# chaitjo/efficient-gnns

Measured on AMD Instinct MI355X. Metric: training epochs/sec, ogbn-arxiv 3-layer GCN student + G-CRD, 1/2/4/8 MI355X, higher is better.
Workload: dtype f32

## Files before the change

### efficient-gnns_amd/_lib.py

```python
from __future__ import annotations

import ctypes as C
import os

import torch

_HERE = os.path.dirname(os.path.abspath(__file__))
LIB_PATH = os.path.join(_HERE, "lib", "libegnn_hip.so")

_p, _i64, _i32, _f32, _sz, _u64 = C.c_void_p, C.c_int64, C.c_int, C.c_float, C.c_size_t, C.c_uint64


class BnAct(C.Structure):
    _fields_ = [("x", _p), ("ld", _i64), ("n", _i64), ("C", _i64),
                ("mean", _p), ("var", _p), ("eps", _f32),
                ("gamma", _p), ("beta", _p),
                ("relu", _i32), ("p", _f32), ("seed", _u64), ("seed_dev", _p),
                ("pick", _p), ("n_pick", _i64)]


class GatLayer(C.Structure):
    _fields_ = [("rowptr", _p), ("col", _p),
                ("colptr", _p), ("t_col", _p), ("perm", _p),
                ("n", _i64), ("nnz", _i64), ("H", _i32), ("C", _i32),
                ("xl", _p), ("ld_xl", _i64),
                ("el", _p), ("er", _p),
                ("attn_l", _p), ("attn_r", _p),
                ("keep", _p), ("mult", _p), ("src_scale", _p), ("dst_scale", _p),
                ("negative_slope", _f32)]


class Spmm(C.Structure):
    _fields_ = [("n_rows", _i64), ("n_src", _i64), ("K", _i64),
                ("rowptr", _p), ("col", _p), ("index_bits", _i32),
                ("val", _p), ("src_scale", _p), ("bias", _p),
                ("X", _p), ("ldx", _i64), ("Y", _p), ("ldy", _i64), ("reduce", _i32),
                ("addend", _p), ("ld_addend", _i64), ("stat_part", _p), ("stat_shift", _p), ("flags", _i32)]


class SignSeg(C.Structure):
    _fields_ = [("B", _i64), ("Cs", _i64), ("H", _i32),
                ("p", _f32), ("seed", _p), ("seed_dev", _p),
                ("slope", _p),
                ("src", _p), ("ld_src", _p), ("n_src", _i64),
                ("batch", _p)]


ADAM_MAX_LAG = 64


class AdamRows(C.Structure):
    _fields_ = [("p", _p), ("m", _p), ("v", _p), ("last", _p),
                ("n_rows", _i64), ("D", _i64), ("ld", _i64),
                ("beta1", _f32), ("beta2", _f32), ("eps", _f32),
                ("one_minus_beta1", _f32), ("one_minus_beta2", _f32),
                ("step", _i32), ("flushed", _i32),
                ("step_size", _f32 * ADAM_MAX_LAG), ("bc2_sqrt", _f32 * ADAM_MAX_LAG),
                ("dup_count", _p)]


SIGNATURES = {
    "egnn_abi_version": (_i32, []),
    "egnn_error_string": (C.c_char_p, [_i32]),
    "egnn_build_info": (_i32, [C.c_char_p, _sz]),
    "egnn_spmm_csr_f32": (_i32, [_p, _p, _p, _i64, _p, _i64, _p, _i64, _p]),
    "egnn_spmm_csr_seg_f32": (_i32, [_p, _p, _i64, _p, _p, _i64, _p, _i64, _p]),
    "egnn_spmm_csr_blk_f32": (_i32, [_p, _i32, _i32, _p, _i64, _p, _p, _i64, _p, _p]),
    "egnn_spmm_blk_stat_rows": (_i64, [_i64, _i32, _i32]),
    "egnn_spmm_blk_window_i32": (_i32, [_p, _p, _i64, _i32, _p, _i64, _p, _p]),
    "egnn_bn_stats_merge_ws_floats": (_sz, [_i64]),
    "egnn_bn_stats_merge_f32": (_i32, [_p, _i64, _i64, _p, _i64, _p, _i64, _p, _i64, _p, _p, _p, _sz, _p]),
    "egnn_spmm_combine_f32": (_i32, [_p, _p, _p, _i64, _p, _i64, _p]),
    "egnn_spmm_csr_max_bwd_f32": (_i32, [_i64, _i64, _p, _i32, _p, _p, _p, _i64, _p, _i64, _p]),
    "egnn_spmm_csr_max_piece_f32": (_i32, [_p, _p, _i32, _p, _p]),
    "egnn_spmm_csr_max_bwd_rows_f32": (_i32, [_i64, _i64, _i64, _p, _p, _i32, _p, _p, _p, _p, _i64, _p, _i64, _p, _i64, _p]),
    "egnn_spmm_algorithmic_bytes": (_i64, [_i64, _i64, _i64, _i64, _i32, _i32]),
    "egnn_csr_from_coo_ws_bytes": (_sz, [_i64, _i64, _i32]),
    "egnn_csr_from_coo_i64": (_i32, [_p, _p, _i64, _i64, _i32, _p, _p, _p, _p, _sz, _p]),
    "egnn_csr_transpose_ws_bytes": (_sz, [_i64, _i64]),
    "egnn_csr_transpose_i64": (_i32, [_p, _p, _i64, _i64, _i64, _p, _p, _p, _p, _sz, _p]),
    "egnn_rowptr_from_sorted_rows_i64": (_i32, [_p, _i64, _i64, _p, _p]),
    "egnn_narrow_i64_to_i32": (_i32, [_p, _i64, _p, _p, _p]),
    "egnn_gcn_norm_count_i64": (_i32, [_p, _p, _i64, _p, _p]),
    "egnn_gcn_norm_fill_i64": (_i32, [_p, _p, _i64, _p, _p, _p, _p]),
    "egnn_gcn_norm_values_i64": (_i32, [_p, _p, _i64, _p, _p, _p]),
    "egnn_gemm_ws_floats": (_sz, [_i32, _i32, _i64, _i64, _i64, _i32]),
    "egnn_gemm_f32": (_i32, [_i32, _i32, _i64, _i64, _i64, _f32, _p, _i64, _p, _i64, _p, _p, _i64, _i32, _p, _sz, _p]),
    "egnn_gemm_ex_f32": (_i32, [_i32, _i32, _i64, _i64, _i64, _f32, _p, _i64, _p, _i64, _p, _p, _i64, _i32, _p, _sz, _i32, _p]),
    "egnn_gemm_add_f32": (_i32, [_i32, _i32, _i64, _i64, _i64, _f32, _p, _i64, _p, _i64, _p, _p, _i64, _p, _i64, _i32, _p, _sz, _p]),
    "egnn_bn_fold_f32": (_i32, [_p, _i64, _i64, _i64, _p, _p, _p, _p, _p, _f32, _p, _i64, _p, _p]),
    "egnn_gemm_rows_f32": (_i32, [_i32, _i32, _i64, _i64, _i64, _f32, _p, _i64, _p, _p, _i64, _p, _p, _p, _i64, _i32, _p, _sz, _p]),
    "egnn_gemm_tn_planes_bytes": (_sz, [_i64, _i64]),
    "egnn_gemm_tn_planes_pack_f32": (_i32, [_p, _i64, _p, _i64, _i64, _p, _sz, _p]),
    "egnn_gemm_tn_planes_ws_floats": (_sz, [_i64, _i64, _i64]),
    "egnn_gemm_tn_planes_f32": (_i32, [_i64, _i64, _i64, _f32, _p, _i64, _p, _p, _i64, _p, _sz, _p]),
    "egnn_gemm_rows_planes_bytes": (_sz, [_i64, _i64]),
    "egnn_gemm_rows_planes_pack_f32": (_i32, [_p, _i64, _p, _i64, _i64, _p, _sz, _p]),
    "egnn_gemm_rows_planes_ws_bytes": (_sz, [_i64, _i64]),
    "egnn_gemm_rows_planes_f32": (_i32, [_i64, _i64, _i64, _f32, _p, _p, _i64, _p, _p, _i64, _p, _sz, _p]),
    "egnn_ce_kd_ws_floats": (_sz, [_i64]),
    "egnn_ce_kd_fwd_f32": (_i32, [_p, _i64, _p, _i64, _p, _p, _i64, _i64, _f32, _p, _p, _p]),
    "egnn_ce_kd_bwd_f32": (_i32, [_p, _i64, _p, _i64, _p, _p, _i64, _i64, _i64, _f32, _p, _p, _p, _p, _i64, _p]),
    "egnn_gather_normalize_rows_f32": (_i32, [_p, _i64, _p, _i64, _i64, _f32, _p, _i64, _p, _p]),
    "egnn_normalize_rows_bwd_f32": (_i32, [_p, _i64, _p, _i64, _p, _p, _i64, _i64, _f32, _p, _i64, _i32, _p]),
    "egnn_nce_ws_floats": (_sz, [_i64]),
    "egnn_nce_fwd_f32": (_i32, [_p, _p, _i64, _i64, _i64, _f32, _i32, _p, _p, _p, _p, _sz, _p]),
    "egnn_nce_saves_exp": (_i32, [_f32, _i32]),
    "egnn_nce_bwd_ws_floats": (_sz, [_i64, _i64, _i64]),
    "egnn_nce_bwd_f32": (_i32, [_p, _p, _i64, _i64, _i64, _f32, _i32, _p, _p, _p, _p, _p, _p, _sz, _p]),
    "egnn_nce_block_fwd_f32": (_i32, [_p, _i64, _p, _i64, _i64, _i64, _i64, _i64, _f32, _f32, _i32, _p, _p, _p, _p, _sz, _p]),
    "egnn_nce_block_bwd_f32": (_i32, [_p, _i64, _p, _i64, _i64, _i64, _i64, _i64, _f32, _f32, _i32, _p, _p, _p, _p, _i64, _p, _i64, _p, _sz, _p]),
    "egnn_gsp_ws_floats": (_sz, [_i64]),
    "egnn_gsp_fwd_f32": (_i32, [_p, _i64, _i64, _p, _i64, _i64, _i64, _i32, _p, _p, _p, _p, _sz, _p]),
    "egnn_rowsum_f32": (_i32, [_p, _i64, _i64, _i64, _p, _p]),
    "egnn_scale_rowcorr_f32": (_i32, [_p, _i64, _p, _i64, _p, _p, _i64, _i64, _p, _i64, _p]),
    "egnn_bce_pair_ws_floats": (_sz, []),
    "egnn_bce_pair_fwd_f32": (_i32, [_p, _p, _p, _i64, _p, _p, _p]),
    "egnn_bce_pair_bwd_f32": (_i32, [_p, _p, _p, _i64, _p, _p, _p, _p]),
    "egnn_edge_sim_f32": (_i32, [_p, _i64, _i64, _p, _p, _i64, _i32, _p, _p, _p]),
    "egnn_edge_sim_coef_f32": (_i32, [_p, _p, _p, _i64, _i32, _p, _p, _p, _p]),
    "egnn_gat_attention_fwd_f32": (_i32, [_p, _p, _p, _p, _i64, _i64, _i32, _f32, _p, _p]),
    "egnn_gat_layer_fwd_f32": (_i32, [_p, _p, _p, _i64, _p]),
    "egnn_gat_layer_bwd_ws_floats": (_sz, [_i64, _i32, _i32]),
    "egnn_gat_layer_bwd_f32": (_i32, [_p, _p, _p, _i64, _i32, _p, _p, _p, _i64, _p, _p, _sz, _p]),
    "egnn_segment_softmax_fwd_f32": (_i32, [_p, _p, _i64, _p, _p]),
    "egnn_segment_softmax_bwd_f32": (_i32, [_p, _p, _p, _i64, _p, _p]),
    "egnn_segment_sum_f32": (_i32, [_p, _p, _i64, _p, _p]),
    "egnn_lsp_loss_ws_floats": (_sz, []),
    "egnn_lsp_loss_fwd_f32": (_i32, [_p, _p, _p, _i64, _i64, _i32, _p, _p, _p, _p, _p]),
    "egnn_lsp_loss_bwd_f32": (_i32, [_p, _p, _p, _i64, _i64, _i32, _p, _p, _p, _p]),
    "egnn_colsum_ws_floats": (_sz, [_i64]),
    "egnn_colsum_f32": (_i32, [_p, _i64, _i64, _i64, _p, _p, _p]),
    "egnn_bn_ws_floats": (_sz, [_i64]),
    "egnn_bn_stats_f32": (_i32, [_p, _i64, _i64, _i64, _p, _p, _p, _sz, _p]),
    "egnn_bn_act_fwd_f32": (_i32, [_p, _p, _i64, _p]),
    "egnn_bn_act_bwd_f32": (_i32, [_p, _p, _i64, _i32, _p, _p, _p, _i64, _p, _p, _sz, _p]),
    "egnn_bn_act_bwd_reduce_f32": (_i32, [_p, _p, _i64, _p, _p, _p, _sz, _p]),
    "egnn_bn_act_bwd_apply_f32": (_i32, [_p, _p, _i64, _p, _p, _f32, _p, _p, _i64, _p, _p, _sz, _p]),
    "egnn_bn_merge_shards_f32": (_i32, [_p, _i32, _i64, _p, _p, _p, _p]),
    "egnn_bn_act_linear_fwd_f32": (_i32, [_p, _p, _i64, _i32, _i64, _p, _i64, _p, _i64, _p]),
    "egnn_skinny_dx_bn_ws_floats": (_sz, [_i64, _i64]),
    "egnn_skinny_dx_bn_bwd_reduce_f32": (_i32, [_p, _i64, _p, _i64, _i32, _i64, _f32, _p, _i64, _p, _i64, _p, _p, _p, _p, _p, _i64, _p, _sz, _p]),
    "egnn_bn_bwd_apply_stored_f32": (_i32, [_p, _p, _p, _f32, _p, _i64, _p, _p, _sz, _p]),
    "egnn_bn_running_update_dev_f32": (_i32, [_p, _p, _i64, _p, _f32, _p, _p, _p, _p]),
    "egnn_bn_running_update_f32": (_i32, [_p, _p, _i64, _i64, _f32, _p, _p, _p, _p]),
    "egnn_split_accuracy_ws_ints": (_sz, []),
    "egnn_split_accuracy_f32": (_i32, [_p, _i64, _i64, _i64, _p, _p, _p, _p, _sz, _p]),
    "egnn_split_counts_f32": (_i32, [_p, _i64, _i64, _i64, _p, _p, _p, _p, _sz, _p]),
    "egnn_rows_add_f32": (_i32, [_p, _i64, _p, _p, _i64, _i64, _i64, _p]),
    "egnn_feature_loss_ws_floats": (_sz, [_i64]),
    "egnn_fitnet_fwd_f32": (_i32, [_p, _i64, _p, _i64, _i64, _i64, _f32, _p, _p, _sz, _p]),
    "egnn_fitnet_bwd_f32": (_i32, [_p, _i64, _p, _i64, _i64, _i64, _f32, _p, _p, _i64, _p, _i64, _p]),
    "egnn_at_fwd_f32": (_i32, [_p, _i64, _i64, _p, _i64, _i64, _i64, _f32, _p, _p, _sz, _p]),
    "egnn_at_bwd_f32": (_i32, [_p, _i64, _i64, _p, _i64, _i64, _i64, _f32, _p, _p, _p, _i64, _p, _i64, _p]),
    "egnn_at_energy_f32": (_i32, [_p, _i64, _i64, _p, _i64, _i64, _i64, _p, _p, _p, _p, _sz, _p]),
    "egnn_at_partial_f32": (_i32, [_p, _p, _i64, _p, _f32, _p, _p, _p, _sz, _p]),
    "egnn_at_bwd_rows_f32": (_i32, [_p, _i64, _i64, _p, _i64, _i64, _i64, _i64, _p, _p, _p, _p, _f32, _p, _p, _i64, _p, _i64, _p]),
    "egnn_saint_induced_geometry": (_i64, [_i32]),
    "egnn_saint_random_walk_i64": (_i32, [_p, _p, _i64, _i64, _i64, _i64, _p, _p, _u64, _p, _p, _p, _p]),
    "egnn_saint_scan_ws_bytes": (_sz, [_i64]),
    "egnn_saint_select_i64": (_i32, [_p, _i64, _p, _p, _i64, _p, _sz, _p]),
    "egnn_saint_induced_count_i64": (_i32, [_p, _p, _p, _i64, _p, _i64, _i64, _i64, _p, _p, _p, _p, _sz, _p]),
    "egnn_saint_induced_fill_i64": (_i32, [_p, _p, _p, _p, _i64, _p, _i64, _i64, _i64, _p, _p, _p, _i64, _p, _p, _p, _p]),
    "egnn_saint_gather_i64": (_i32, [_p, _i64, _p, _p, _p, _p, _p, _p, _p, _p, _p, _i64, _p, _p, _p]),
    "egnn_sign_gather_drop_f32": (_i32, [_p, _p, _i64, _p]),
    "egnn_prelu_drop_fwd_f32": (_i32, [_p, _p, _i64, _p, _i64, _p]),
    "egnn_prelu_drop_ws_floats": (_sz, [_i64, _i64, _i32]),
    "egnn_prelu_drop_bwd_f32": (_i32, [_p, _p, _i64, _p, _i64, _p, _i64, _p, _p, _p, _sz, _p]),
    "egnn_pair_moments_ws_bytes": (_sz, [_i64]),
    "egnn_pair_moments_f32": (_i32, [_p, _i64, _i64, _p, _i64, _i64, _i64, _p, _p, _sz, _p]),
    "egnn_pearson_moments_ws_bytes": (_sz, [_i64]),
    "egnn_pearson_moments_f32": (_i32, [_p, _p, _i64, _p, _p, _sz, _p]),
    "egnn_sqdist_median_ws_bytes": (_sz, [_i64]),
    "egnn_sqdist_median_f32": (_i32, [_p, _i64, _i64, _i64, _p, _p, _sz, _p]),
    "egnn_rbf_cka_ws_bytes": (_sz, [_i64]),
    "egnn_rbf_cka_f32": (_i32, [_p, _i64, _i64, _p, _i64, _i64, _i64, _p, _p, _p, _sz, _p]),
    "egnn_group_input_f32": (_i32, [_p, _p, _i32, _p, _p, _i64, _i64, _p, _i64, _p, _p]),
    "egnn_adam_rows_catchup_f32": (_i32, [_p, _i32, _p, _p, _i64, _p]),
    "egnn_adam_rows_flush_f32": (_i32, [_p, _p]),
    "egnn_adam_rows_step_f32": (_i32, [_p, _i32, _p, _p, _i64, _p, _i64, _p]),
    "egnn_probe_gather_lines_f32":(_i32, [_p, _i64, _i64, _i64, _p, _i64, _i32, _i32, _p, _p]),
}

_lib = None


class HipExtensionError(RuntimeError):
    pass


def load() -> C.CDLL:
    global _lib
    if _lib is not None:
        return _lib
    if not os.path.exists(LIB_PATH):
        raise HipExtensionError(
            f"{LIB_PATH} is missing: build it with `python efficient-gnns_amd/build.py` "
            "(__graft_entry__.build()); there is no CPU fallback")
    lib = C.CDLL(LIB_PATH)
    for name, (res, args) in SIGNATURES.items():
        fn = getattr(lib, name)
        fn.restype, fn.argtypes = res, args
    if lib.egnn_abi_version() != 9:
        raise HipExtensionError("libegnn_hip.so ABI version mismatch")
    _lib = lib
    return lib


EGNN_EALIGN = -4


def check(rc: int, what: str) -> None:
    if rc != 0:
        msg = load().egnn_error_string(rc).decode()
        raise HipExtensionError(f"{what} failed: {msg} ({rc})")


# ... 28 lines not shown
```

### efficient-gnns_amd/criterion.py

```python
from __future__ import annotations

import numpy as np
import torch

from . import ops

__all__ = ["distill", "kd_criterion", "fitnet_criterion", "at_criterion", "gpw_criterion", "lpw_criterion", "nce_criterion",
           "loss_kd_only", "ppi_kd_criterion", "ppi_fitnet_criterion", "ppi_at_criterion", "ppi_gpw_criterion", "ppi_lpw_criterion",
           "ppi_nce_criterion"]


_ROW_SAMPLER = None


def _sample_rows(n: int, max_samples: int, device):
    if _ROW_SAMPLER is not None:
        return _ROW_SAMPLER(n, max_samples, device)
    if max_samples < n:
        pick = np.random.choice(n, max_samples, replace=False)
        return torch.from_numpy(pick).to(device=device, dtype=torch.int64, non_blocking=True)
    return None


def _rows_of(x, idx):
# ... 24 lines not shown
    if rows is not None:
        logits, labels = logits[rows], labels[rows]
    return bce_with_logits_pair(logits, labels, logits.detach())[0]




def kd_criterion(logits, labels, teacher_logits, alpha=0.9, T=4):
    return rows_kd_criterion(logits, labels, teacher_logits, alpha, T, rows=None)


def rows_kd_criterion(logits, labels, teacher_logits, alpha=0.9, T=4, rows=None):
    loss_cls, loss_kd = ops.ce_and_kd(_plain(logits), _plain(labels), _plain(teacher_logits), T, rows)
    loss = loss_kd * (alpha * T * T) + loss_cls * (1 - alpha)
    return loss, loss_cls, loss_kd


def loss_kd_only(logits, labels, teacher_logits, alpha=0.9, T=4):
    return kd_criterion(logits, labels, teacher_logits, alpha, T)[2]


def fitnet_criterion(logits, labels, feat, teacher_feat, beta=1000):
    return rows_fitnet_criterion(logits, labels, feat, teacher_feat, beta, rows=None)


@_plain_args
def rows_fitnet_criterion(logits, labels, feat, teacher_feat, beta=1000, rows=None, *, _cls=None):
    loss_cls = (_cls or _ce_term)(logits, labels, rows)
    loss_aux = ops.fitnet_loss(_plain(feat), _plain(teacher_feat))
    return torch.add(loss_cls, loss_aux, alpha=beta), loss_cls, loss_aux


def at_criterion(logits, labels, feat, teacher_feat, beta=1000):
    return rows_at_criterion(logits, labels, feat, teacher_feat, beta, rows=None)


@_plain_args
def rows_at_criterion(logits, labels, feat, teacher_feat, beta=1000, rows=None, *, _cls=None):
    loss_cls = (_cls or _ce_term)(logits, labels, rows)
    loss_aux = ops.at_loss(_plain(feat), _plain(teacher_feat))
    return torch.add(loss_cls, loss_aux, alpha=beta), loss_cls, loss_aux


def gpw_criterion(logits, labels, feat, teacher_feat, kernel="cosine", beta=1, max_samples=8192):
    return rows_gpw_criterion(logits, labels, feat, teacher_feat, kernel, beta, max_samples, rows=None)


@_plain_args
def rows_gpw_criterion(logits, labels, feat, teacher_feat, kernel="cosine", beta=1, max_samples=8192, rows=None, presampled=False, *, _cls=None):
    from .ops_pairwise import gsp_loss
    if kernel not in ("cosine", "poly", "l2", "rbf"):
        raise NotImplementedError
    loss_cls = (_cls or _ce_term)(logits, labels, rows)
    idx = None if presampled else _sample_rows(feat.shape[0], max_samples, feat.device)
    if hasattr(feat, "_egnn_materialise") or hasattr(teacher_feat, "_egnn_materialise"):
        from .lazy import materialise
        feat, teacher_feat, idx = materialise(feat, idx), materialise(teacher_feat, idx), None
    loss_aux = gsp_loss(feat, teacher_feat, idx, kernel)
    return torch.add(loss_cls, loss_aux, alpha=beta), loss_cls, loss_aux


def lpw_criterion(logits, labels, feat, teacher_feat, edge_index, kernel="cosine", beta=100, criterion="kld"):
    return rows_lpw_criterion(logits, labels, feat, teacher_feat, edge_index, kernel, beta, criterion, rows=None)


@_plain_args
def rows_lpw_criterion(logits, labels, feat, teacher_feat, edge_index, kernel="cosine", beta=100, criterion="kld", rows=None, *, _cls=None):
    from .ops_edge import lsp_loss
    if kernel not in ("cosine", "poly", "l2", "rbf") or criterion not in ("kld", "mse"):
        raise NotImplementedError
    loss_cls = (_cls or _ce_term)(logits, labels, rows)
    loss_aux = lsp_loss(_plain(feat), _plain(teacher_feat), edge_index, kernel, criterion)
    return torch.add(loss_cls, loss_aux, alpha=beta), loss_cls, loss_aux


def nce_criterion(logits, labels, feat, teacher_feat, beta=0.5, nce_T=0.075, max_samples=8192):
    return rows_nce_criterion(logits, labels, feat, teacher_feat, beta, nce_T, max_samples, rows=None)


@_plain_args
def rows_nce_criterion(logits, labels, feat, teacher_feat, beta=0.5, nce_T=0.075, max_samples=8192, rows=None, presampled=False, *, _cls=None):
    loss_cls = (_cls or _ce_term)(logits, labels, rows)
    idx = None if presampled else _sample_rows(feat.shape[0], max_samples, feat.device)
    fhat = ops.gather_normalize(*_rows_of(feat, idx))
    that = ops.gather_normalize(*_rows_of(teacher_feat, idx))
    loss_aux = ops.nce_unit(fhat, that, nce_T)
    return torch.add(loss_cls, loss_aux, alpha=beta), loss_cls, loss_aux


def ppi_fitnet_criterion(logits, labels, feat, teacher_feat, beta=1000):
    return rows_fitnet_criterion(logits, labels, feat, teacher_feat, beta, _cls=_bce_term)


def ppi_at_criterion(logits, labels, feat, teacher_feat, beta=1000):
    return rows_at_criterion(logits, labels, feat, teacher_feat, beta, _cls=_bce_term)


def ppi_gpw_criterion(logits, labels, feat, teacher_feat, kernel="cosine", beta=1, max_samples=8192):
    return rows_gpw_criterion(logits, labels, feat, teacher_feat, kernel, beta, max_samples, _cls=_bce_term)


def ppi_lpw_criterion(logits, labels, feat, teacher_feat, edge_index, kernel="cosine", beta=100, criterion="kld"):
    return rows_lpw_criterion(logits, labels, feat, teacher_feat, edge_index, kernel, beta, criterion, _cls=_bce_term)


def ppi_nce_criterion(logits, labels, feat, teacher_feat, beta=0.5, nce_T=0.075, max_samples=8192):
    return rows_nce_criterion(logits, labels, feat, teacher_feat, beta, nce_T, max_samples, _cls=_bce_term)


def ppi_kd_criterion(logits, labels, teacher_logits, alpha=0.5, T=1):
    from .ops_pairwise import bce_with_logits_pair
    loss_cls, loss_kd = bce_with_logits_pair(_plain(logits), _plain(labels), _plain(teacher_logits))
    return loss_kd * (alpha * T * T) + loss_cls * (1 - alpha), loss_cls, loss_kd


def presample(mode, n, hp, device):
    return _sample_rows(n, hp["max_samples"], device) if mode in ("gpw", "nce") else None


def distill(mode, logits, labels, feat, teacher_feat, hp, *, teacher_logits=None, rows=None, edge_index=None, presampled=False,
            multilabel=False, kd_and_aux=False):
    cls = _bce_term if multilabel else None

    def kd():
        if not multilabel:
            return rows_kd_criterion(logits, labels, teacher_logits, hp["alpha"], hp["kd_T"], rows=rows)
        picked = (logits, labels, teacher_logits) if rows is None else (logits[rows], labels[rows], teacher_logits[rows])
        return ppi_kd_criterion(*picked, hp["alpha"], hp["kd_T"])
    if mode == "kd":
        return kd()
    if mode == "fitnet":
        res = rows_fitnet_criterion(logits, labels, feat, teacher_feat, hp["beta"], rows=rows, _cls=cls)
    elif mode == "at":
        res = rows_at_criterion(logits, labels, feat, teacher_feat, hp["beta"], rows=rows, _cls=cls)
    elif mode == "gpw":
        res = rows_gpw_criterion(logits, labels, feat, teacher_feat, hp["kernel"], hp["beta"], hp["max_samples"], rows=rows,
                                 presampled=presampled, _cls=cls)
    elif mode == "lpw":
        res = rows_lpw_criterion(logits, labels, feat, teacher_feat, edge_index, hp["kernel"], hp["beta"], rows=rows, _cls=cls)
    elif mode in ("nce", "gcd"):
        res = rows_nce_criterion(logits, labels, feat, teacher_feat, hp["beta"], hp["nce_T"], hp["max_samples"], rows=rows,
                                 presampled=presampled, _cls=cls)
    else:
        raise NotImplementedError(mode)
    if not kd_and_aux:
        return res
    loss, loss_cls, _ = kd()
    return loss + hp["beta"] * res[2], loss_cls, res[2]
```

### efficient-gnns_amd/csrc/fused_bn.hip

```cpp
#include "bn_common.h"

namespace {

constexpr int kMaxChunks = 4;
constexpr int kStatBlocks = 512;

using namespace egnn_bn;

__global__ __launch_bounds__(256) void bn_stats_partial_kernel(const float* __restrict__ x, int64_t ld, int64_t n, int64_t C,
                                                               float* __restrict__ part) {
  __shared__ float sh[4][2][kMaxChunks * 256];
  const int lane = egnn_lane();
  const int wave = egnn_wave_id();
  const int chunks = (int)((C + 255) / 256);
  float s1[kMaxChunks][4], s2[kMaxChunks][4], x0[kMaxChunks][4];
#pragma unroll
  for (int j = 0; j < kMaxChunks; ++j)
#pragma unroll
    for (int q = 0; q < 4; ++q) { s1[j][q] = 0.f; s2[j][q] = 0.f; x0[j][q] = 0.f; }
#pragma unroll
  for (int j = 0; j < kMaxChunks; ++j) {
    const int64_t c = j * 256 + lane * 4;
    if (j < chunks && c < C) {
      const float4 v = *reinterpret_cast<const float4*>(x + c);
      x0[j][0] = v.x; x0[j][1] = v.y; x0[j][2] = v.z; x0[j][3] = v.w;
    }
  }
  auto tally = [&](int j, const float4& v) {
    const float d0 = v.x - x0[j][0], d1 = v.y - x0[j][1], d2 = v.z - x0[j][2], d3 = v.w - x0[j][3];
    s1[j][0] += d0; s1[j][1] += d1; s1[j][2] += d2; s1[j][3] += d3;
    s2[j][0] = fmaf(d0, d0, s2[j][0]); s2[j][1] = fmaf(d1, d1, s2[j][1]);
    s2[j][2] = fmaf(d2, d2, s2[j][2]); s2[j][3] = fmaf(d3, d3, s2[j][3]);
  };
  const int64_t stride = (int64_t)gridDim.x * 4;
  int64_t row = blockIdx.x * 4LL + wave;
  if (chunks == 1) {
    const int64_t c = lane * 4;
    if (c < C) {
      for (; row + 3 * stride < n; row += 4 * stride) {
        float4 v[4];
#pragma unroll
        for (int u = 0; u < 4; ++u) v[u] = *reinterpret_cast<const float4*>(x + (row + u * stride) * ld + c);
#pragma unroll
        for (int u = 0; u < 4; ++u) tally(0, v[u]);
      }
    }
  }
  for (; row < n; row += stride) {
#pragma unroll
    for (int j = 0; j < kMaxChunks; ++j) {
      const int64_t c = j * 256 + lane * 4;
      if (j < chunks && c < C) tally(j, *reinterpret_cast<const float4*>(x + row * ld + c));
    }
  }
#pragma unroll
  for (int j = 0; j < kMaxChunks; ++j)
#pragma unroll
    for (int q = 0; q < 4; ++q) {
      sh[wave][0][j * 256 + lane * 4 + q] = s1[j][q];
      sh[wave][1][j * 256 + lane * 4 + q] = s2[j][q];
    }
  __syncthreads();
  for (int64_t c = threadIdx.x; c < C; c += 256) {
    float a = 0.f, b = 0.f;
    for (int w = 0; w < 4; ++w) { a += sh[w][0][c]; b += sh[w][1][c]; }
    part[((int64_t)blockIdx.x * 2) * C + c] = a;
    part[((int64_t)blockIdx.x * 2 + 1) * C + c] = b;
  }
}

constexpr int kMergeCols = 8;
constexpr int kMergeGroups = 256 / kMergeCols;
__device__ __forceinline__ void merge_partials(const float* __restrict__ part, int nblocks, int64_t C, float& a, float& b, bool& owner,
                                               int64_t& c) {
  __shared__ float sh[2][kMergeGroups][kMergeCols];
  const int col = threadIdx.x % kMergeCols, grp = threadIdx.x / kMergeCols;
  c = (int64_t)blockIdx.x * kMergeCols + col;
  float sa = 0.f, sb = 0.f;
  if (c < C)
    for (int i = grp; i < nblocks; i += kMergeGroups) { sa += part[((int64_t)i * 2) * C + c]; sb += part[((int64_t)i * 2 + 1) * C + c]; }
  sh[0][grp][col] = sa;
  sh[1][grp][col] = sb;
  __syncthreads();
  owner = grp == 0 && c < C;
  a = 0.f; b = 0.f;
  if (owner)
    for (int g = 0; g < kMergeGroups; ++g) { a += sh[0][g][col]; b += sh[1][g][col]; }
}

__global__ __launch_bounds__(256) void bn_stats_final_kernel(const float* __restrict__ part, int nblocks, const float* __restrict__ x,
                                                             int64_t n, int64_t C, float* __restrict__ mean, float* __restrict__ var) {
  float a, b; bool owner; int64_t c;
  merge_partials(part, nblocks, C, a, b, owner, c);
  if (!owner) return;
  const float inv = 1.f / (float)n;
  const float m1 = a * inv;
  mean[c] = x[c] + m1;
  var[c] = fmaxf(b * inv - m1 * m1, 0.f);
}

__global__ __launch_bounds__(256) void bn_act_fwd_kernel(const BnParams q, float* __restrict__ y, int64_t ldy) {
  const int lane = egnn_lane();
  const int wave = egnn_wave_id();
  const int chunks = (int)((q.C + 255) / 256);
  for (int j = 0; j < chunks; ++j) {
    const int64_t c = j * 256 + lane * 4;
    if (c >= q.C) continue;
    float mean[4], rstd[4], g[4], b[4];
#pragma unroll
    for (int k = 0; k < 4; ++k) {
      mean[k] = q.mean[c + k];
      rstd[k] = rsqrtf(q.var[c + k] + q.eps);
      g[k] = q.gamma ? q.gamma[c + k] : 1.f;
      b[k] = q.beta ? q.beta[c + k] : 0.f;
    }
    for (int64_t row = blockIdx.x * 4LL + wave; row < q.n; row += (int64_t)gridDim.x * 4) {
      const int64_t src = bn_row(q, row);
      const float4 v = *reinterpret_cast<const float4*>(q.x + src * q.ldx + c);
      const float xv[4] = {v.x, v.y, v.z, v.w};
      float o[4];
#pragma unroll
      for (int k = 0; k < 4; ++k) {
        float xhat, gate;
        bn_elem(q, xv[k], mean[k], rstd[k], g[k], b[k], src, c + k, xhat, gate);
        o[k] = (g[k] * xhat + b[k]) * gate;
      }
      *reinterpret_cast<float4*>(y + row * ldy + c) = make_float4(o[0], o[1], o[2], o[3]);
    }
  }
}

__global__ __launch_bounds__(256) void bn_act_bwd_reduce_kernel(const BnParams q, const float* __restrict__ dy, int64_t ldd,
                                                                float* __restrict__ part) {
  __shared__ float sh[4][2][kMaxChunks * 256];
  const int lane = egnn_lane();
  const int wave = egnn_wave_id();
  const int chunks = (int)((q.C + 255) / 256);
  for (int j = 0; j < chunks; ++j) {
    const int64_t c = j * 256 + lane * 4;
    float sd[4] = {0.f, 0.f, 0.f, 0.f}, sx[4] = {0.f, 0.f, 0.f, 0.f};
    if (c < q.C) {
      float mean[4], rstd[4], g[4], b[4];
#pragma unroll
      for (int k = 0; k < 4; ++k) {
        mean[k] = q.mean[c + k];
        rstd[k] = rsqrtf(q.var[c + k] + q.eps);
        g[k] = q.gamma ? q.gamma[c + k] : 1.f;
        b[k] = q.beta ? q.beta[c + k] : 0.f;
      }
      const int64_t stride = (int64_t)gridDim.x * 4;
      int64_t row = blockIdx.x * 4LL + wave;
      for (; row + 3 * stride < q.n; row += 4 * stride) {
        float4 v[4], gd[4];
        int64_t src[4];
#pragma unroll
        for (int u = 0; u < 4; ++u) {
          src[u] = bn_row(q, row + u * stride);
          v[u] = *reinterpret_cast<const float4*>(q.x + src[u] * q.ldx + c);
          gd[u] = *reinterpret_cast<const float4*>(dy + (row + u * stride) * ldd + c);
        }
#pragma unroll
        for (int u = 0; u < 4; ++u) {
          const float xv[4] = {v[u].x, v[u].y, v[u].z, v[u].w};
          const float gv[4] = {gd[u].x, gd[u].y, gd[u].z, gd[u].w};
#pragma unroll
          for (int k = 0; k < 4; ++k) {
            float xhat, gate;
            bn_elem(q, xv[k], mean[k], rstd[k], g[k], b[k], src[u], c + k, xhat, gate);
            const float d = gv[k] * gate;
            sd[k] += d;
            sx[k] = fmaf(d, xhat, sx[k]);
          }
        }
      }
      for (; row < q.n; row += stride) {
        const int64_t src = bn_row(q, row);
        const float4 v = *reinterpret_cast<const float4*>(q.x + src * q.ldx + c);
        const float4 gd = *reinterpret_cast<const float4*>(dy + row * ldd + c);
        const float xv[4] = {v.x, v.y, v.z, v.w};
        const float gv[4] = {gd.x, gd.y, gd.z, gd.w};
#pragma unroll
// ... 121 lines not shown
    rmean[c] = (1.f - m) * rmean[c] + m * mean[c];
    rvar[c] = (1.f - m) * rvar[c] + (m * unbias) * var[c];
  }
  __syncthreads();
  if (threadIdx.x == 0 && tracked) tracked[0] = t;
}

__global__ __launch_bounds__(256) void bn_running_update_dev_kernel(const float* __restrict__ mean, const float* __restrict__ var, int64_t C,
                                                                    const float* __restrict__ total, float momentum, float* __restrict__ rmean,
                                                                    float* __restrict__ rvar, long long* __restrict__ tracked) {
  const long long t = tracked ? tracked[0] + 1 : 1;
  const float m = momentum < 0.f ? 1.f / (float)t : momentum;
  const float n = total[0];
  const float unbias = n > 1.f ? n / (n - 1.f) : 1.f;
  for (int64_t c = threadIdx.x; c < C; c += 256) {
    rmean[c] = (1.f - m) * rmean[c] + m * mean[c];
    rvar[c] = (1.f - m) * rvar[c] + (m * unbias) * var[c];
  }
  __syncthreads();
  if (threadIdx.x == 0 && tracked) tracked[0] = t;
}

bool shape_ok(const void* p, int64_t ld, int64_t C) { return C > 0 && C % 4 == 0 && C <= kMaxChunks * 256 && ld % 4 == 0 && egnn_aligned16(p); }

int row_blocks(int64_t n) {
  const int64_t want = (n + 3) / 4;
  return (int)(want < 2048 ? (want < 1 ? 1 : want) : 2048);
}

int bn_unpack(const egnn_bn_act_t* b, BnParams& all, BnParams& out) {
  EGNN_CHECK_ARG(b && b->n > 0 && b->x && b->mean && b->var && b->ld >= b->C);
  EGNN_CHECK_ARG(!b->pick || (b->n_pick >= 0 && b->n_pick <= b->n));
  if (!shape_ok(b->x, b->ld, b->C)) return EGNN_EALIGN;
  all = BnParams{b->x, b->ld, b->n, b->C, b->mean, b->var, b->eps, b->gamma, b->beta, b->relu, b->p, (unsigned long long)b->seed,
                 (const unsigned long long*)b->seed_dev, nullptr};
  out = all;
  if (b->pick) { out.n = b->n_pick; out.pick = b->pick; }
  return EGNN_OK;
}

}

namespace {
__global__ void bn_merge_shards_kernel(const float* __restrict__ st, int world, int64_t C, float* __restrict__ mean,
                                       float* __restrict__ var, float* __restrict__ total) {
  const int64_t c = blockIdx.x * 256LL + threadIdx.x;
  if (c >= C) return;
  const int64_t ld = 2 * C + 1;
  float n = 0.f, m = 0.f, m2 = 0.f;
  for (int w = 0; w < world; ++w) {
    const float nb = st[w * ld + 2 * C];
    if (nb <= 0.f) continue;
    const float mb = st[w * ld + c], vb = st[w * ld + C + c];
    const float nt = n + nb, d = mb - m;
    m2 = m2 + vb * nb + d * d * (n * nb / nt);
    m = m + d * (nb / nt);
    n = nt;
  }
  mean[c] = m;
  var[c] = n > 0.f ? m2 / n : 0.f;
  if (c == 0) total[0] = n;
}
}

extern "C" int egnn_bn_merge_shards_f32(const float* stats, int world, int64_t C, float* mean, float* var, float* total,
                                        void* stream) {
  EGNN_CHECK_ARG(world > 0 && C > 0 && stats && mean && var && total);
  hipLaunchKernelGGL(bn_merge_shards_kernel, dim3((unsigned)((C + 255) / 256)), dim3(256), 0, (hipStream_t)stream, stats, world, C, mean,
                     var, total);
  return egnn_launch_status();
}

extern "C" size_t egnn_bn_ws_floats(int64_t C) { return (size_t)kStatBlocks * 2 * (size_t)C; }

extern "C" int egnn_bn_stats_f32(const float* x, int64_t ld, int64_t n, int64_t C, float* mean, float* var, float* ws,
                                 size_t ws_floats, void* stream) {
  EGNN_CHECK_ARG(n > 0 && x && mean && var && ws && ld >= C);
  if (!shape_ok(x, ld, C)) return EGNN_EALIGN;
  if (ws_floats < egnn_bn_ws_floats(C)) return EGNN_EWORKSPACE;
  hipStream_t st = (hipStream_t)stream;
  const int64_t want = (n + 3) / 4;
  const int nb = (int)(want < kStatBlocks ? want : kStatBlocks);
  hipLaunchKernelGGL(bn_stats_partial_kernel, dim3(nb), dim3(256), 0, st, x, ld, n, C, ws);
  hipLaunchKernelGGL(bn_stats_final_kernel, dim3((unsigned)((C + kMergeCols - 1) / kMergeCols)), dim3(256), 0, st, ws, nb, x, n, C, mean, var);
  return egnn_launch_status();
}

extern "C" int egnn_bn_act_fwd_f32(const egnn_bn_act_t* bn, float* y, int64_t ldy, void* stream) {
  BnParams qa, q;
  const int rc = bn_unpack(bn, qa, q);
  if (rc != EGNN_OK) return rc;
  EGNN_CHECK_ARG(q.n > 0 && y && ldy >= bn->C && bn->p >= 0.f && bn->p < 1.f);
  if (!shape_ok(y, ldy, bn->C)) return EGNN_EALIGN;
  hipLaunchKernelGGL(bn_act_fwd_kernel, dim3(row_blocks(q.n)), dim3(256), 0, (hipStream_t)stream, q, y, ldy);
  return egnn_launch_status();
}

extern "C" int egnn_bn_act_bwd_reduce_f32(const egnn_bn_act_t* bn, const float* dy, int64_t ld_dy, float* dgamma, float* dbeta, float* ws,
                                          size_t ws_floats, void* stream) {
  BnParams qa, q;
  const int rc = bn_unpack(bn, qa, q);
  if (rc != EGNN_OK) return rc;
  const int64_t C = bn->C;
  EGNN_CHECK_ARG(q.n > 0 && dy && dgamma && dbeta && ws && ld_dy >= C);
  if (!shape_ok(dy, ld_dy, C)) return EGNN_EALIGN;
  if (ws_floats < egnn_bn_ws_floats(C)) return EGNN_EWORKSPACE;
  hipStream_t st = (hipStream_t)stream;
  const int64_t want = (q.n + 3) / 4;
  const int nb = (int)(want < kStatBlocks ? want : kStatBlocks);
  hipLaunchKernelGGL(bn_act_bwd_reduce_kernel, dim3(nb), dim3(256), 0, st, q, dy, ld_dy, ws);
  hipLaunchKernelGGL(bn_bwd_final_kernel, dim3((unsigned)((C + kMergeCols - 1) / kMergeCols)), dim3(256), 0, st, ws, nb, C, dbeta, dgamma);
  return egnn_launch_status();
}

extern "C" int egnn_bn_act_bwd_apply_f32(const egnn_bn_act_t* bn, const float* dy, int64_t ld_dy, const float* sum_dbeta,
                                         const float* sum_dgamma, float inv_count, const float* local_dbeta, float* dx, int64_t ld_dx,
                                         float* dx_colsum, float* ws, size_t ws_floats, void* stream) {
  BnParams qa, qp;
  const int rc = bn_unpack(bn, qa, qp);
  if (rc != EGNN_OK) return rc;
  const int64_t C = bn->C;
  const bool rows = bn->pick != nullptr;
  EGNN_CHECK_ARG(sum_dbeta && sum_dgamma && dx && ld_dx >= C);
  EGNN_CHECK_ARG(qp.n == 0 || (dy && ld_dy >= C));
  EGNN_CHECK_ARG(!dx_colsum || !rows || qp.n == 0 || local_dbeta);
  if (!shape_ok(dx, ld_dx, C) || (qp.n > 0 && !shape_ok(dy, ld_dy, C))) return EGNN_EALIGN;
  if (dx_colsum && (ws == nullptr || ws_floats < egnn_bn_ws_floats(C))) return EGNN_EWORKSPACE;
  hipStream_t st = (hipStream_t)stream;
  int nb = row_blocks(bn->n);
  if (dx_colsum) {
    if (nb > 2 * kStatBlocks) nb = 2 * kStatBlocks;
    nb = (nb + 1) & ~1;
  }
  if (!rows) {
    if (dx_colsum)
      hipLaunchKernelGGL(bn_act_bwd_apply_kernel<true>, dim3(nb), dim3(256), 0, st, qa, dy, ld_dy, sum_dbeta, sum_dgamma, inv_count, dx, ld_dx, ws);
    else
      hipLaunchKernelGGL(bn_act_bwd_apply_kernel<false>, dim3(nb), dim3(256), 0, st, qa, dy, ld_dy, sum_dbeta, sum_dgamma, inv_count, dx, ld_dx,
                         (float*)nullptr);
  } else {
    if (dx_colsum)
      hipLaunchKernelGGL((bn_act_bwd_apply_kernel<true, 1>), dim3(nb), dim3(256), 0, st, qa, (const float*)nullptr, (int64_t)0, sum_dbeta, sum_dgamma,
                         inv_count, dx, ld_dx, ws);
    else
      hipLaunchKernelGGL((bn_act_bwd_apply_kernel<false, 1>), dim3(nb), dim3(256), 0, st, qa, (const float*)nullptr, (int64_t)0, sum_dbeta, sum_dgamma,
                         inv_count, dx, ld_dx, (float*)nullptr);
    if (qp.n > 0)
      hipLaunchKernelGGL((bn_act_bwd_apply_kernel<false, 2>), dim3(row_blocks(qp.n)), dim3(256), 0, st, qp, dy, ld_dy, sum_dbeta, sum_dgamma, inv_count,
                         dx, ld_dx, (float*)nullptr);
  }
  if (dx_colsum)
    hipLaunchKernelGGL(colsum_final_kernel, dim3((unsigned)((C + kMergeCols - 1) / kMergeCols)), dim3(256), 0, st, ws, nb / 2, C, dx_colsum,
                       rows ? bn->gamma : (const float*)nullptr, rows ? bn->var : (const float*)nullptr, rows ? bn->eps : 0.f,
                       rows && qp.n > 0 ? local_dbeta : (const float*)nullptr);
  return egnn_launch_status();
}

extern "C" int egnn_bn_act_bwd_f32(const egnn_bn_act_t* bn, const float* dy, int64_t ld_dy, int batch_stats, float* dgamma, float* dbeta,
                                   float* dx, int64_t ld_dx, float* dx_colsum, float* ws, size_t ws_floats, void* stream) {
  EGNN_CHECK_ARG(bn && dx && ld_dx >= bn->C);
  if (!shape_ok(dx, ld_dx, bn->C)) return EGNN_EALIGN;
  const int rc = egnn_bn_act_bwd_reduce_f32(bn, dy, ld_dy, dgamma, dbeta, ws, ws_floats, stream);
  if (rc != EGNN_OK) return rc;
  return egnn_bn_act_bwd_apply_f32(bn, dy, ld_dy, dbeta, dgamma, batch_stats ? 1.f / (float)bn->n : 0.f, dbeta, dx, ld_dx, dx_colsum, ws,
                                   ws_floats, stream);
}

// ... 504 lines not shown
```

### efficient-gnns_amd/csrc/nce.hip

```cpp
#include <stdlib.h>

#include "gemm3.h"

using namespace egnn_gemm;

namespace {

#ifndef EGNN_NCE_FWD_WAVES
#define EGNN_NCE_FWD_WAVES 2
#endif
constexpr int kMaxSplit = 8;
constexpr int FB = 128;

__device__ __forceinline__ float nce_shift(float inv_tau) { return inv_tau * 1.0001f; }
inline bool nce_unit_form(float tau, int unit_rows) { return unit_rows && (2.f / tau) <= 80.f; }

__device__ __forceinline__ float exp_bounded(float x) {
  const float kL2eHi = 1.44269502162933349609375f, kL2eLo = 1.925963033500011e-8f;
  const float n = __builtin_rintf(x * kL2eHi);
  float f = fmaf(x, kL2eHi, -n);
  f = fmaf(x, kL2eLo, f);
  return ldexpf(__builtin_amdgcn_exp2f(f), (int)n);
}

// ... 296 lines not shown
                                                      float coef, const float* __restrict__ g, float* __restrict__ C,
                                                      int64_t ldc, int64_t k_per_split, float* __restrict__ ws) {
  constexpr int BN = 128;
  using TS = typename TileSel<SPLIT, BM, BN>::type;
  extern __shared__ __attribute__((aligned(16))) float smem[];
  const int64_t tiles_n = (P + BN - 1) / BN;
  const int64_t tiles = (int64_t)gridDim.x;
  int64_t mt, nt;
  if (tiles_n > 1 && tiles % (8 * tiles_n) == 0) {
    nt = (blockIdx.x >> 3) % tiles_n;
    mt = (blockIdx.x & 7) + 8 * (blockIdx.x / (8 * tiles_n));
  } else {
    mt = blockIdx.x / tiles_n;
    nt = blockIdx.x % tiles_n;
  }
  const int64_t m0 = mt * BM, n0 = nt * BN;
  const int64_t kbeg = (int64_t)blockIdx.y * k_per_split;
  int64_t kend = kbeg + k_per_split;
  if (kend > Kd) kend = Kd;
  f32x16 acc[TS::TM][TS::TN];
  zero_acc(acc);
  IdentityXf id;
  const bool full = SPLIT && (kend - kbeg) % BK == 0;
  auto run = [&](auto fo, const auto& xa, const auto& xb) {
    mainloop_sel<SPLIT, BM, BN, AMAJ, MNMAJOR, VEC4, fo.value>(acc, Z, ldz, m0, M, Bm, ldb, n0, P, kbeg, kend, xa, xb, smem);
  };
  auto both = [&](const auto& xa, const auto& xb) {
    if constexpr (SPLIT) {
      if (full) run(std::true_type{}, xa, xb);
      else run(std::false_type{}, xa, xb);
    } else {
      run(std::false_type{}, xa, xb);
    }
  };
  if constexpr (!EXPZ) {
    NceGradXf xf{lse, AMAJ == MNMAJOR, diag_off};
    both(xf, id);
  } else if constexpr (AMAJ == KMAJOR) {
    both(id, id);
  } else if constexpr (BW) {
    RowWeightXf xw{lse, shift};
    both(id, xw);
  } else {
    both(id, id);
  }
  const int lane = egnn_lane();
  const int wave = egnn_wave_id();
  const int wm = wave >> 1, wn = wave & 1;
  const bool partial = gridDim.y > 1;
  const float scale = coef * (g ? g[0] : 1.f);
  float* out = partial ? ws + (int64_t)blockIdx.y * M * P : C;
  const int64_t ldo = partial ? P : ldc;
#pragma unroll
  for (int tn = 0; tn < TS::TN; ++tn) {
    const int64_t c = n0 + acc_col<BM, BN>(wn, tn, lane);
    if (c >= P) continue;
#pragma unroll
    for (int tm = 0; tm < TS::TM; ++tm)
#pragma unroll
      for (int r = 0; r < 16; ++r) {
        const int64_t row = m0 + acc_row<BM, BN>(wm, tm, r, lane);
        if (row >= M) continue;
        const float v = acc[tm][tn][r];
        out[row * ldo + c] = partial ? v : nce_bwd_finish<AMAJ, EXPZ>(v, row, c, Kd, diag_off, lse, shift, Im, ldi, scale);
      }
  }
}

template <int AMAJ, bool EXPZ>
__global__ __launch_bounds__(256) void nce_bwd_reduce_kernel(const float* __restrict__ ws, int nsplit, int64_t M, int64_t P, int64_t Kd,
                                                             int64_t diag_off, const float* __restrict__ lse, float shift,
                                                             const float* __restrict__ Im, int64_t ldi, float coef,
                                                             const float* __restrict__ g, float* __restrict__ C, int64_t ldc) {
  const int64_t total = M * P;
  const float scale = coef * (g ? g[0] : 1.f);
  for (int64_t t = blockIdx.x * 256LL + threadIdx.x; t < total; t += (int64_t)gridDim.x * 256) {
    float v = 0.f;
    for (int k = 0; k < nsplit; ++k) v += ws[(int64_t)k * total + t];
    const int64_t row = t / P, c = t % P;
    C[row * ldc + c] = nce_bwd_finish<AMAJ, EXPZ>(v, row, c, Kd, diag_off, lse, shift, Im, ldi, scale);
  }
}

__global__ __launch_bounds__(256) void nce_row_weight_kernel(const float* __restrict__ x, int64_t ldx, const float* __restrict__ lse,
                                                             float shift, int64_t n, int64_t P, float* __restrict__ out) {
  const int64_t total = n * P;
  for (int64_t t = blockIdx.x * 256LL + threadIdx.x; t < total; t += (int64_t)gridDim.x * 256) {
    const int64_t i = t / P, c = t % P;
    out[t] = x[i * ldx + c] * expf(shift - lse[i]);
  }
}

inline int nce_bwd_split(int64_t M, int64_t P, int64_t Kd) {
  const int64_t t128 = ((M + 127) / 128) * ((P + 127) / 128);
  int64_t n = (768 + t128 - 1) / t128;
  const int64_t ksteps = (Kd + BK - 1) / BK;
  if (n > ksteps / 8) n = ksteps / 8;
  if (n > kMaxSplit) n = kMaxSplit;
  return n < 1 ? 1 : (int)n;
}

template <int AMODE, int TM, int TN, int BKT, int NB, int OCC>
__global__ __launch_bounds__(256, OCC) void nce3_bwd_kernel(const float* __restrict__ E, int64_t lde, const char* __restrict__ planes, int64_t nks,
                                                            int64_t M, int64_t P, int64_t k_per_split, float* __restrict__ ws) {
  using T = egnn_gemm3::Tile<AMODE, egnn_gemm3::PLANES, TM, TN, BKT, NB>;
  extern __shared__ __attribute__((aligned(16))) float smem[];
  const int64_t tiles_n = P / T::BN;
  int64_t tile = blockIdx.x;
  if (tiles_n > 1 && tiles_n <= 8) {
    const int64_t tiles = gridDim.x, q = tiles >> 3, rem = tiles & 7, xcd = tile & 7, j = tile >> 3;
    tile = (xcd < rem ? xcd * (q + 1) : rem * (q + 1) + (xcd - rem) * q) + j;
  }
  const int64_t m0 = (tile / tiles_n) * T::BM, n0 = (tile % tiles_n) * T::BN;
  const int64_t kbeg = (int64_t)blockIdx.y * k_per_split, kend = kbeg + k_per_split;
  f32x16 acc[TM][TN];
#pragma unroll
  for (int i = 0; i < TM; ++i)
#pragma unroll
    for (int j = 0; j < TN; ++j)
#pragma unroll
      for (int r = 0; r < 16; ++r) acc[i][j][r] = 0.f;
  constexpr int SCHED = AMODE == egnn_gemm3::F32M ? egnn_gemm3::SCHED_IGLP0 : egnn_gemm3::SCHED_HAND;
  egnn_gemm3::mainloop<AMODE, egnn_gemm3::PLANES, TM, TN, BKT, NB, 1, SCHED>(acc, E, lde, m0, planes, nks, n0, kbeg, kend, reinterpret_cast<char*>(smem));
  const int lane = egnn_lane(), wave = egnn_wave_id();
  const int wm = wave >> 1, wn = wave & 1;
  float* out = ws + (int64_t)blockIdx.y * M * P;
#pragma unroll
  for (int tn = 0; tn < TN; ++tn) {
    const int64_t c = n0 + wn * 32 * TN + tn * 32 + (lane & 31);
#pragma unroll
    for (int tm = 0; tm < TM; ++tm)
#pragma unroll
      for (int r = 0; r < 16; ++r) {
        const int64_t row = m0 + wm * 32 * TM + tm * 32 + (r & 3) + 8 * (r >> 2) + 4 * (lane >> 5);
        out[row * P + c] = acc[tm][tn][r];
      }
  }
}

constexpr int kNce3SplitMax = 8;
static inline int nce3_split(int64_t M) {
  return (M / 256) * 4 >= 256 ? 4 : 8;
}

inline size_t nce3_ws_floats(int64_t M, int64_t P, int64_t Kd) {
  return (size_t)kNce3SplitMax * M * P + (egnn_gemm3::planes_bytes(P, Kd, 256, 32) + 1024) / 4;
}

template <int AMAJ>
inline bool nce3_takes(int64_t M, int64_t Kd, int64_t P, int64_t ldz, const float* Z, bool expz, bool vec4, const float* ws) {
  constexpr int BM = AMAJ == KMAJOR ? 128 : 256, BN = AMAJ == KMAJOR ? 128 : 256, BKT = AMAJ == KMAJOR ? 32 : 16;
  return egnn_split_pipe() && expz && vec4 && ws && M % BM == 0 && P % BN == 0 && Kd % (kNce3SplitMax * BKT) == 0 && ldz % 4 == 0 &&
         egnn_aligned16(Z) && Kd / kNce3SplitMax >= 4 * BKT;
}

template <int AMAJ>
int launch_bwd3(const float* Z, int64_t ldz, int64_t M, int64_t Kd, int64_t diag_off, const float* lse, float shift, const float* Bm, int64_t P,
                int64_t ldb, const float* Im, int64_t ldi, float coef, const float* g, float* C, int64_t ldc, float* ws, hipStream_t st) {
  using namespace egnn_gemm3;
  float* partial = ws;
  const int kNce3Split = nce3_split(M);
  char* planes = reinterpret_cast<char*>((reinterpret_cast<uintptr_t>(ws + (size_t)kNce3SplitMax * M * P) + 1023) & ~(uintptr_t)1023);
  const int64_t k_per_split = Kd / kNce3Split;
  int rc;
  if constexpr (AMAJ == KMAJOR) {
    constexpr int TM = 2, TN = 2, BKT = 32, NB = 2;
    pack_planes<64 * TN, BKT>(Bm, ldb, 0, P, Kd, nullptr, nullptr, nullptr, 0.f, planes, st);
    using T = Tile<F32K, PLANES, TM, TN, BKT, NB>;
    const dim3 grid((unsigned)((M / T::BM) * (P / T::BN)), (unsigned)kNce3Split);
    rc = launch_dyn_lds<nce3_bwd_kernel<F32K, TM, TN, BKT, NB, 2>>(grid, dim3(256), (size_t)T::SMEM_BYTES, st, Z, ldz, (const char*)planes, Kd / BKT, M, P,
                                                                   k_per_split, partial);
  } else {
    constexpr int TM = 4, TN = 4, BKT = 16, NB = 3;
    pack_planes<64 * TN, BKT>(Bm, ldb, 0, P, Kd, nullptr, nullptr, lse, shift, planes, st);
    using T = Tile<F32M, PLANES, TM, TN, BKT, NB>;
    const dim3 grid((unsigned)((M / T::BM) * (P / T::BN)), (unsigned)kNce3Split);
    rc = launch_dyn_lds<nce3_bwd_kernel<F32M, TM, TN, BKT, NB, 1>>(grid, dim3(256), (size_t)T::SMEM_BYTES, st, Z, ldz, (const char*)planes, Kd / BKT, M, P,
                                                                   k_per_split, partial);
  }
  if (rc != EGNN_OK) return rc;
  const int64_t rb = (M * P + 255) / 256;
  hipLaunchKernelGGL((nce_bwd_reduce_kernel<AMAJ, true>), dim3((unsigned)(rb < 4096 ? rb : 4096)), dim3(256), 0, st, partial, kNce3Split, M, P, Kd,
                     diag_off, lse, shift, Im, ldi, coef, g, C, ldc);
  return EGNN_OK;
}

template <int AMAJ>
int launch_bwd(const float* Z, int64_t ldz, int64_t M, int64_t Kd, int64_t diag_off, const float* lse, float shift, bool expz,
                const float* Bm, int64_t P, int64_t ldb, const float* Im, int64_t ldi, float coef, const float* g, float* C,
                int64_t ldc, bool vec4, float* ws, hipStream_t st) {
  if (nce3_takes<AMAJ>(M, Kd, P, ldz, Z, expz, vec4, ws)) {
    return launch_bwd3<AMAJ>(Z, ldz, M, Kd, diag_off, lse, shift, Bm, P, ldb, Im, ldi, coef, g, C, ldc, ws, st);
  }
  const int64_t tiles_n = (P + 127) / 128;
  const int64_t t128 = ((M + 127) / 128) * tiles_n;
  constexpr int64_t min_tiles = 600;
  const int nsplit = ws ? nce_bwd_split(M, P, Kd) : 1;
  const bool big = ws || t128 >= min_tiles;
  const int64_t ksteps = (Kd + BK - 1) / BK;
  const int64_t k_per_split = ((ksteps + nsplit - 1) / nsplit) * BK;
  const dim3 grid((unsigned)(big ? t128 : ((M + 63) / 64) * tiles_n), (unsigned)nsplit);
  const bool split = big && egnn_split_pipe();
  constexpr size_t shm_f32 = (size_t)TileShape<128, 128>::SMEM_FLOATS * 4, shm_split = (size_t)TileShapeS<128, 128>::SMEM_BYTES;
  int rc = EGNN_OK;
#define EGNN_NCE_BWD_ARGS(B_, LDB_) Z, ldz, M, Kd, diag_off, lse, shift, B_, P, LDB_, Im, ldi, coef, g, C, ldc, k_per_split, ws
  if (AMAJ == MNMAJOR && ws && expz && vec4 && big) {
    float* wx = ws + (size_t)nsplit * M * P;
    const int64_t blocks = (Kd * P + 255) / 256;
    hipLaunchKernelGGL(nce_row_weight_kernel, dim3((unsigned)(blocks < 4096 ? blocks : 4096)), dim3(256), 0, st, Bm, ldb, lse, shift, Kd, P, wx);
    if (split) rc = launch_dyn_lds<nce_bwd_kernel<128, AMAJ, true, true, false, true>>(grid, dim3(256), shm_split, st, EGNN_NCE_BWD_ARGS(wx, P));
    else rc = launch_dyn_lds<nce_bwd_kernel<128, AMAJ, true, true, false, false>>(grid, dim3(256), shm_f32, st, EGNN_NCE_BWD_ARGS(wx, P));
    if (rc != EGNN_OK) return rc;
    if (nsplit > 1) {
      const int64_t rb = (M * P + 255) / 256;
      hipLaunchKernelGGL((nce_bwd_reduce_kernel<AMAJ, true>), dim3((unsigned)(rb < 4096 ? rb : 4096)), dim3(256), 0, st, ws, nsplit, M, P, Kd,
                         diag_off, lse, shift, Im, ldi, coef, g, C, ldc);
    }
    return EGNN_OK;
  }
#define EGNN_NCE_BWD(BM_, V, E, S_) rc_main = launch_dyn_lds<nce_bwd_kernel<BM_, AMAJ, V, E, true, S_>>(grid, dim3(256), S_ ? shm_split : (size_t)TileShape<BM_, 128>::SMEM_FLOATS * 4, st, EGNN_NCE_BWD_ARGS(Bm, ldb))
  int rc_main = EGNN_OK;
  if (split) {
    if (vec4) { if (expz) EGNN_NCE_BWD(128, true, true, true); else EGNN_NCE_BWD(128, true, false, true); }
    else { if (expz) EGNN_NCE_BWD(128, false, true, true); else EGNN_NCE_BWD(128, false, false, true); }
  } else if (big) {
    if (vec4) { if (expz) EGNN_NCE_BWD(128, true, true, false); else EGNN_NCE_BWD(128, true, false, false); }
    else { if (expz) EGNN_NCE_BWD(128, false, true, false); else EGNN_NCE_BWD(128, false, false, false); }
  } else {
    if (vec4) { if (expz) EGNN_NCE_BWD(64, true, true, false); else EGNN_NCE_BWD(64, true, false, false); }
    else { if (expz) EGNN_NCE_BWD(64, false, true, false); else EGNN_NCE_BWD(64, false, false, false); }
  }
#undef EGNN_NCE_BWD
#undef EGNN_NCE_BWD_ARGS
  if (rc_main != EGNN_OK) return rc_main;
  if (nsplit > 1) {
    const int64_t blocks = (M * P + 255) / 256;
    const dim3 rgrid((unsigned)(blocks < 4096 ? blocks : 4096));
    if (expz) hipLaunchKernelGGL((nce_bwd_reduce_kernel<AMAJ, true>), rgrid, dim3(256), 0, st, ws, nsplit, M, P, Kd, diag_off, lse, shift, Im, ldi, coef, g, C, ldc);
    else hipLaunchKernelGGL((nce_bwd_reduce_kernel<AMAJ, false>), rgrid, dim3(256), 0, st, ws, nsplit, M, P, Kd, diag_off, lse, shift, Im, ldi, coef, g, C, ldc);
  }
  return EGNN_OK;
}

}

extern "C" size_t egnn_nce_ws_floats(int64_t S) { return (size_t)S * (1 + 2 * kMaxSplit) + kFinalBlocks; }

extern "C" size_t egnn_nce_bwd_ws_floats(int64_t Sr, int64_t Sc, int64_t P) {
  if (Sr <= 0 || Sc <= 0 || P <= 0) return 0;
  const size_t a = (size_t)nce_bwd_split(Sr, P, Sc) * Sr * P, b = (size_t)nce_bwd_split(Sc, P, Sr) * Sc * P;
  const size_t staged = (a > b ? a : b) + (size_t)Sr * P;
  const size_t a3 = nce3_ws_floats(Sr, P, Sc), b3 = nce3_ws_floats(Sc, P, Sr);
  const size_t dma = a3 > b3 ? a3 : b3;
  return staged > dma ? staged : dma;
}

extern "C" int egnn_nce_saves_exp(float tau, int unit_rows) { return tau > 0.f && nce_unit_form(tau, unit_rows) ? 1 : 0; }

extern "C" int egnn_nce_block_fwd_f32(const float* fhat, int64_t ld_f, const float* that, int64_t ld_t, int64_t Sr, int64_t Sc,
                                      int64_t diag_off, int64_t P, float tau, float inv_count, int unit_rows, float* Z,
                                      float* lse, float* loss, float* ws, size_t ws_floats, void* stream) {
  EGNN_CHECK_ARG(Sr > 0 && Sc > 0 && P > 0 && ld_f >= P && ld_t >= P && tau > 0.f && fhat && that && lse && loss && ws);
  EGNN_CHECK_ARG(diag_off >= 0 && diag_off + Sr <= Sc);
  if (ws_floats < egnn_nce_ws_floats(Sr)) return EGNN_EWORKSPACE;
  hipStream_t st = (hipStream_t)stream;
  const int64_t rb = (Sr + FB - 1) / FB;
  const int64_t ncb = (Sc + FB - 1) / FB;
  int nsplit = (int)((256 * EGNN_NCE_FWD_WAVES + rb - 1) / rb);
  if (nsplit > kMaxSplit) nsplit = kMaxSplit;
  if (nsplit > ncb) nsplit = (int)ncb;
  if (nsplit < 1) nsplit = 1;
  const int cb_per_split = (int)((ncb + nsplit - 1) / nsplit);
  nsplit = (int)((ncb + cb_per_split - 1) / cb_per_split);
  float* zdiag = ws;
  float* pm = ws + Sr;
  float* ps = pm + Sr * kMaxSplit;
  const bool vec4 = (ld_f % 4 == 0) && (ld_t % 4 == 0) && egnn_aligned16(fhat) && egnn_aligned16(that);
  dim3 grid((unsigned)rb, (unsigned)nsplit);
  const bool fixed = nce_unit_form(tau, unit_rows);
  const bool aligned = Z && vec4 && fixed && Sr % FB == 0 && Sc % FB == 0 && P % BK == 0 && Sc < (1LL << 28);
  const bool split = egnn_split_pipe() && (!aligned || P % (BK * PipelineS<FB, FB, KMAJOR, KMAJOR, true, true, IdentityXf, IdentityXf>::UNROLL) == 0);
  int rc_fwd = EGNN_OK;
#define EGNN_NCE_FWD(V, F, A)                                                                                                              \
  do {                                                                                                                                     \
    if (split) rc_fwd = launch_dyn_lds<nce_fwd_kernel<V, F, A, true>>(grid, dim3(256), (size_t)TileShapeS<FB, FB>::SMEM_BYTES, st, fhat, ld_f, that, ld_t, Sr, \
                                                             Sc, diag_off, P, 1.f / tau, Z, zdiag, pm, ps, nsplit, cb_per_split);           \
    else rc_fwd = launch_dyn_lds<nce_fwd_kernel<V, F, A, false>>(grid, dim3(256), (size_t)TileShape<FB, FB>::SMEM_FLOATS * 4, st, fhat, ld_f, that, ld_t, Sr,  \
                                                        Sc, diag_off, P, 1.f / tau, Z, zdiag, pm, ps, nsplit, cb_per_split);                \
  } while (0)
  if (aligned) EGNN_NCE_FWD(true, true, true);
  else if (vec4) { if (fixed) EGNN_NCE_FWD(true, true, false); else EGNN_NCE_FWD(true, false, false); }
  else { if (fixed) EGNN_NCE_FWD(false, true, false); else EGNN_NCE_FWD(false, false, false); }
#undef EGNN_NCE_FWD
  if (rc_fwd != EGNN_OK) return rc_fwd;
  float* block_part = ps + Sr * kMaxSplit;
  const int fb = (int)((Sr + 255) / 256 < kFinalBlocks ? (Sr + 255) / 256 : kFinalBlocks);
  hipLaunchKernelGGL(nce_finalize_rows_kernel, dim3(fb), dim3(256), 0, st, pm, ps, zdiag, Sr, nsplit, lse, block_part);
  hipLaunchKernelGGL(nce_finalize_sum_kernel, dim3(1), dim3(256), 0, st, block_part, fb, inv_count, loss);
  return egnn_launch_status();
}

extern "C" int egnn_nce_block_bwd_f32(const float* fhat, int64_t ld_f, const float* that, int64_t ld_t, int64_t Sr, int64_t Sc,
                                      int64_t diag_off, int64_t P, float tau, float scale, int unit_rows, const float* Z,
                                      const float* lse, const float* g, float* dfhat, int64_t ld_df, float* dthat, int64_t ld_dt,
                                      float* ws, size_t ws_floats, void* stream) {
  EGNN_CHECK_ARG(Sr > 0 && Sc > 0 && P > 0 && ld_f >= P && ld_t >= P && tau > 0.f && fhat && that && Z && lse);
  if (ws && ws_floats < egnn_nce_bwd_ws_floats(Sr, Sc, P)) return EGNN_EWORKSPACE;
  EGNN_CHECK_ARG(diag_off >= 0 && diag_off + Sr <= Sc);
  EGNN_CHECK_ARG((dfhat == nullptr || ld_df >= P) && (dthat == nullptr || ld_dt >= P));
  hipStream_t st = (hipStream_t)stream;
  const bool vec4 = (ld_f % 4 == 0) && (ld_t % 4 == 0) && (Sc % 4 == 0) && egnn_aligned16(fhat) && egnn_aligned16(that) && egnn_aligned16(Z);
  const bool expz = nce_unit_form(tau, unit_rows);
  const float shift = (1.f / tau) * 1.0001f;
  int rc = EGNN_OK;
  if (dfhat) rc = launch_bwd<KMAJOR>(Z, Sc, Sr, Sc, diag_off, lse, shift, expz, that, P, ld_t, that, ld_t, scale, g, dfhat, ld_df, vec4, ws, st);
  if (rc == EGNN_OK && dthat) rc = launch_bwd<MNMAJOR>(Z, Sc, Sc, Sr, diag_off, lse, shift, expz, fhat, P, ld_f, fhat, ld_f, scale, g, dthat, ld_dt, vec4, ws, st);
  if (rc != EGNN_OK) return rc;
  return egnn_launch_status();
}

extern "C" int egnn_nce_fwd_f32(const float* fhat, const float* that, int64_t S, int64_t P, int64_t ld, float tau, int unit_rows,
                                float* Z, float* lse, float* loss, float* ws, size_t ws_floats, void* stream) {
  return egnn_nce_block_fwd_f32(fhat, ld, that, ld, S, S, 0, P, tau, S > 0 ? 1.f / (float)S : 0.f, unit_rows, Z, lse, loss, ws, ws_floats, stream);
}

extern "C" int egnn_nce_bwd_f32(const float* fhat, const float* that, int64_t S, int64_t P, int64_t ld, float tau, int unit_rows,
                                const float* Z, const float* lse, const float* g, float* dfhat, float* dthat,
                                float* ws, size_t ws_floats, void* stream) {
  EGNN_CHECK_ARG(S > 0 && tau > 0.f);
  return egnn_nce_block_bwd_f32(fhat, ld, that, ld, S, S, 0, P, tau, 1.f / ((float)S * tau), unit_rows, Z, lse, g, dfhat, ld, dthat,
                                ld, ws, ws_floats, stream);
}
```

### efficient-gnns_amd/csrc/spmm_blk.hip

```cpp
#include "spmm_desc.h"

namespace {

typedef unsigned int v4u __attribute__((ext_vector_type(4)));
typedef float v4f __attribute__((ext_vector_type(4)));
typedef __amdgpu_buffer_rsrc_t rsrc_t;

struct BlkArgs {
  int64_t n_rows, K;
  const int32_t* rowptr;
  const int32_t* col;
  const float* val;
  const float* src_scale;
  const float* bias;
  const float* X;
  int64_t ldx;
  float* Y;
  int64_t ldy;
  int mean;
  int seg_max;
  int rows_per_blk;
  const int32_t* blk_ptr;
  int64_t n_blk;
  const int32_t* win;
// ... 269 lines not shown
#pragma unroll
      for (int o = 8; o < 64; o <<= 1) {
        st1[q] += __shfl_xor(st1[q], o);
        st2[q] += __shfl_xor(st2[q], o);
      }
    }
    if (lane < 8 && colok) {
      float* sp = a.stat_part + ((int64_t)(blk * WAVES + wave) * 2) * a.K + col0;
      *reinterpret_cast<float4*>(sp) = make_float4(st1[0], st1[1], st1[2], st1[3]);
      *reinterpret_cast<float4*>(sp + a.K) = make_float4(st2[0], st2[1], st2[2], st2[3]);
    }
  }
}

__global__ __launch_bounds__(256) void spmm_blk_window_kernel(const int32_t* __restrict__ rowptr, const int32_t* __restrict__ col,
                                                             int64_t n_rows, int rows_per_blk, const int32_t* __restrict__ blk_ptr,
                                                             int64_t n_blk, int32_t* __restrict__ win) {
  const int64_t row = blockIdx.x * 256LL + threadIdx.x;
  if (row >= n_rows) return;
  int64_t lo_id, hi_id;
  if (blk_ptr) {
    int64_t lo = 0, hi = n_blk;
    while (hi - lo > 1) {
      const int64_t mid = (lo + hi) >> 1;
      if (blk_ptr[mid] <= row) lo = mid; else hi = mid;
    }
    lo_id = blk_ptr[lo];
    hi_id = blk_ptr[lo + 1];
  } else {
    lo_id = row / rows_per_blk * rows_per_blk;
    hi_id = lo_id + rows_per_blk;
  }
  const int s = rowptr[row], e = rowptr[row + 1];
  auto lower = [&](int64_t key) {
    int l = s, h = e;
    while (l < h) {
      const int m = (l + h) >> 1;
      if (col[m] < key) l = m + 1; else h = m;
    }
    return l;
  };
  win[2 * row] = lower(lo_id);
  win[2 * row + 1] = lower(hi_id);
}

constexpr int kStatSplits = 512;
__global__ __launch_bounds__(256) void bn_stats_fold_kernel(const float* __restrict__ part, int64_t n_blk, int64_t C,
                                                            float* __restrict__ fold) {
  __shared__ float sh[2][8][32];
  const int c = threadIdx.x & 31, g = threadIdx.x >> 5;
  const int64_t col = (int64_t)blockIdx.x * 32 + c;
  const int s = blockIdx.y;
  const int64_t per = (n_blk + kStatSplits - 1) / kStatSplits;
  const int64_t b0 = s * per, b1 = b0 + per < n_blk ? b0 + per : n_blk;
  float sa = 0.f, sb = 0.f;
  if (col < C) {
    int64_t i = b0 + g;
    for (; i + 24 < b1; i += 32) {
      const float a0 = part[(i * 2) * C + col], a1 = part[((i + 8) * 2) * C + col], a2 = part[((i + 16) * 2) * C + col],
                  a3 = part[((i + 24) * 2) * C + col];
      const float c0 = part[(i * 2 + 1) * C + col], c1 = part[((i + 8) * 2 + 1) * C + col], c2 = part[((i + 16) * 2 + 1) * C + col],
                  c3 = part[((i + 24) * 2 + 1) * C + col];
      sa += a0; sa += a1; sa += a2; sa += a3;
      sb += c0; sb += c1; sb += c2; sb += c3;
    }
    for (; i < b1; i += 8) {
      sa += part[(i * 2) * C + col];
      sb += part[(i * 2 + 1) * C + col];
    }
  }
  sh[0][g][c] = sa;
  sh[1][g][c] = sb;
  __syncthreads();
  if (threadIdx.x < 64) {
    const int which = threadIdx.x >> 5;
    float t = 0.f;
    for (int q = 0; q < 8; ++q) t += sh[which][q][c];
    if (col < C) fold[((int64_t)s * 2 + which) * C + col] = t;
  }
}

__global__ __launch_bounds__(256) void bn_stats_merge_kernel(const float* __restrict__ part, int64_t n_part, int64_t C,
                                                             const float* __restrict__ Y, int64_t ldy, const int64_t* __restrict__ extra_rows,
                                                             int64_t n_extra, const float* __restrict__ shift, int64_t n_total,
                                                             float* __restrict__ mean, float* __restrict__ var) {
  __shared__ float sh[2][32][8];
  const int colo = threadIdx.x & 7, grp = threadIdx.x >> 3;
  const int64_t c = (int64_t)blockIdx.x * 8 + colo;
  float sa = 0.f, sb = 0.f;
  if (c < C) {
    const float sft = shift ? shift[c] : 0.f;
    for (int64_t i = grp; i < n_part; i += 32) {
      sa += part[(i * 2) * C + c];
      sb += part[(i * 2 + 1) * C + c];
    }
    for (int64_t i = grp; i < n_extra; i += 32) {
      const float d = Y[extra_rows[i] * ldy + c] - sft;
      sa += d;
      sb = fmaf(d, d, sb);
    }
  }
  sh[0][grp][colo] = sa;
  sh[1][grp][colo] = sb;
  __syncthreads();
  if (grp == 0 && c < C) {
    float a = 0.f, b = 0.f;
    for (int g = 0; g < 32; ++g) { a += sh[0][g][colo]; b += sh[1][g][colo]; }
    const float inv = 1.f / (float)n_total;
    const float m1 = a * inv;
    mean[c] = (shift ? shift[c] : 0.f) + m1;
    var[c] = fmaxf(b * inv - m1 * m1, 0.f);
  }
}

template <bool LDS, bool STATS, int WAVES, int ROWS>
int launch_blk(const BlkArgs& a, unsigned grid, size_t shm, hipStream_t st) {
  if (shm > 65536 && hipFuncSetAttribute((const void*)spmm_blk_kernel<LDS, STATS, WAVES, ROWS>,
                                         hipFuncAttributeMaxDynamicSharedMemorySize, (int)shm) != hipSuccess)
    return EGNN_ELAUNCH;
  hipLaunchKernelGGL((spmm_blk_kernel<LDS, STATS, WAVES, ROWS>), dim3(grid), dim3(WAVES * 64), shm, st, a);
  return egnn_launch_status();
}

}

extern "C" int64_t egnn_spmm_blk_stat_rows(int64_t n_rows, int rows_per_blk, int lds) {
  if (n_rows <= 0 || rows_per_blk <= 0) return 0;
  return (n_rows + rows_per_blk - 1) / rows_per_blk * (lds ? 16 : 4);
}

extern "C" int egnn_spmm_blk_window_i32(const int32_t* rowptr, const int32_t* col, int64_t n_rows, int rows_per_blk,
                                        const int32_t* blk_ptr, int64_t n_blk, int32_t* win, void* stream) {
  EGNN_CHECK_ARG(n_rows >= 0 && rows_per_blk > 0 && (blk_ptr == nullptr || n_blk > 0));
  if (n_rows == 0) return EGNN_OK;
  EGNN_CHECK_ARG(rowptr && win);
  hipLaunchKernelGGL(spmm_blk_window_kernel, dim3((unsigned)((n_rows + 255) / 256)), dim3(256), 0, (hipStream_t)stream, rowptr, col,
                     n_rows, rows_per_blk, blk_ptr, n_blk, win);
  return egnn_launch_status();
}

extern "C" int egnn_spmm_csr_blk_f32(const egnn_spmm_t* op, int seg_max, int rows_per_blk, const int32_t* blk_ptr, int64_t n_blk,
                                     const int32_t* win, const int32_t* hub_seg, int64_t n_hub_seg, float* partial, void* stream) {
  const int rc = spmm_check(op, kSpmmGather | kSpmmEpilogue);
  if (rc != EGNN_OK) return rc;
  EGNN_CHECK_ARG(rows_per_blk > 0 && rows_per_blk % 32 == 0 && seg_max > 0 && n_hub_seg >= 0);
  const int64_t n_rows = op->n_rows, K = op->K;
  if (n_rows == 0 || K == 0) return EGNN_OK;
  EGNN_CHECK_ARG(op->rowptr && op->col && op->X && op->Y && (n_hub_seg == 0 || (hub_seg && partial)));
  if (op->index_bits != 32) return EGNN_EALIGN;
  if (K % 4 != 0 || op->ldx % 4 != 0 || op->ldy % 4 != 0 || !egnn_aligned16(op->X) || !egnn_aligned16(op->Y) ||
      (op->bias && !egnn_aligned16(op->bias)) || (partial && !egnn_aligned16(partial)) ||
      (op->addend && (!egnn_aligned16(op->addend) || op->ld_addend % 4 != 0 || op->ld_addend < K)))
    return EGNN_EALIGN;
  const uint64_t xb = (uint64_t)op->n_src * (uint64_t)op->ldx * 4ull;
  if (xb > 0x7FFFFFFFull) return EGNN_EALIGN;
  if (blk_ptr == nullptr) n_blk = (n_rows + rows_per_blk - 1) / rows_per_blk;
  EGNN_CHECK_ARG(n_blk > 0);
  const bool lds = win != nullptr;
  EGNN_CHECK_ARG(!lds || (op->n_src == n_rows && rows_per_blk <= 512 && rows_per_blk % 128 == 0));
  BlkArgs a{};
  a.n_rows = n_rows; a.K = K; a.rowptr = (const int32_t*)op->rowptr; a.col = (const int32_t*)op->col;
  a.val = op->val; a.src_scale = op->src_scale; a.bias = op->bias;
  a.X = op->X; a.ldx = op->ldx; a.Y = op->Y; a.ldy = op->ldy; a.mean = op->reduce == EGNN_MEAN;
  a.seg_max = seg_max; a.rows_per_blk = rows_per_blk; a.blk_ptr = blk_ptr; a.n_blk = n_blk; a.win = win;
  a.hseg = hub_seg; a.n_hseg = n_hub_seg; a.P = partial;
  a.addend = op->addend; a.ld_add = op->ld_addend; a.stat_part = op->stat_part; a.stat_shift = op->stat_shift;
  a.x_bytes = (uint32_t)xb; a.flags = op->flags;
  a.NS = (int)((K + 31) / 32);
  a.map_mode = (a.NS <= 8 && 8 % a.NS == 0) ? 1 : (a.NS % 8 == 0 ? 2 : 0);
  const int nsub = lds ? 128 : 32;
  const int64_t n_items = (n_hub_seg + nsub - 1) / nsub + n_blk;
  int64_t grid;
  if (a.map_mode == 1) {
    const int r = 8 / a.NS;
    grid = (n_items + r - 1) / r * 8;
  } else {
    grid = n_items * a.NS;
  }
  if (grid > 0x7fffffffLL) return EGNN_EINVAL;
  hipStream_t st = (hipStream_t)stream;
  const bool stats = op->stat_part != nullptr;
  if (!lds) {
    if (rows_per_blk == 32)
      return stats ? launch_blk<false, true, 4, 1>(a, (unsigned)grid, 0, st) : launch_blk<false, false, 4, 1>(a, (unsigned)grid, 0, st);
    return stats ? launch_blk<false, true, 4, 0>(a, (unsigned)grid, 0, st) : launch_blk<false, false, 4, 0>(a, (unsigned)grid, 0, st);
  }
  const size_t shm = (size_t)(rows_per_blk + 1) * 128;
  return stats ? launch_blk<true, true, 16, 4>(a, (unsigned)grid, shm, st) : launch_blk<true, false, 16, 4>(a, (unsigned)grid, shm, st);
}

extern "C" size_t egnn_bn_stats_merge_ws_floats(int64_t C) { return (size_t)kStatSplits * 2 * (size_t)C; }

extern "C" int egnn_bn_stats_merge_f32(const float* part, int64_t n_blk, int64_t C, const float* Y, int64_t ldy,
                                       const int64_t* extra_rows, int64_t n_extra, const float* shift, int64_t n_total, float* mean,
                                       float* var, float* ws, size_t ws_floats, void* stream) {
  EGNN_CHECK_ARG(n_blk >= 0 && C > 0 && n_extra >= 0 && n_total > 0 && mean && var);
  EGNN_CHECK_ARG((n_blk == 0 || part) && (n_extra == 0 || (Y && extra_rows && ldy >= C)));
  hipStream_t st = (hipStream_t)stream;
  int64_t n_part = n_blk;
  if (n_blk > 2 * kStatSplits) {
    if (ws == nullptr || ws_floats < egnn_bn_stats_merge_ws_floats(C)) return EGNN_EWORKSPACE;
    hipLaunchKernelGGL(bn_stats_fold_kernel, dim3((unsigned)((C + 31) / 32), kStatSplits), dim3(256), 0, st, part, n_blk, C, ws);
    part = ws;
    n_part = kStatSplits;
  }
  hipLaunchKernelGGL(bn_stats_merge_kernel, dim3((unsigned)((C + 7) / 8)), dim3(256), 0, st, part, n_part, C, Y, ldy, extra_rows,
                     n_extra, shift, n_total, mean, var);
  return egnn_launch_status();
}
```

### efficient-gnns_amd/models.py

```python
from __future__ import annotations

import contextlib
import math
import os

import torch
import torch.nn.functional as F
from torch import nn

from . import _cache, _lib
from . import criterion as C
from . import ops
from .nn import DGLGATConv, GATConv, GCNConv, RGCNConv, SAGEConv
from .sparse import SparseTensor


_EVAL_BN_FOLD = True
_TRAIN_ROWS = True
_FUSED_TAIL = True


class _Student(nn.Module):
    def __init__(self, make_conv, in_channels, hidden_channels, out_channels, num_layers, dropout):
        super().__init__()
        dims = [in_channels] + [hidden_channels] * (num_layers - 1) + [out_channels]
        self.convs = nn.ModuleList(make_conv(a, b) for a, b in zip(dims[:-1], dims[1:]))
        self.bns = nn.ModuleList(nn.BatchNorm1d(hidden_channels) for _ in range(num_layers - 1))
        self.dropout = dropout
        self.out_feat = None

    def reset_parameters(self):
        for m in list(self.convs) + list(self.bns):
            m.reset_parameters()

    def _layer_form(self, li, x, adj_t):
        conv, bn, last = self.convs[li], self.bns[li], self.convs[-1]
        training, grad, gpu = self.training, torch.is_grad_enabled(), x.is_cuda
        plain_adj, sharded_adj = isinstance(adj_t, SparseTensor), hasattr(adj_t, "gcn_normalized")
        gcn, torch_bn, sync_bn = isinstance(conv, GCNConv), isinstance(bn, nn.BatchNorm1d), hasattr(bn, "fused_act")
        if (_EVAL_BN_FOLD and not training and not grad and gcn and gpu and not conv._uses_memoised_input(x)
                and ((type(bn) is nn.BatchNorm1d and bn.track_running_stats and plain_adj) or (sharded_adj and sync_bn))):
            return "fold", None
        conv_form = "stats" if (gcn and torch_bn and gpu and training and plain_adj) else "plain"
        act = "bn_act" if (torch_bn and gpu) else ("sync" if sync_bn else "torch")
        if (li == len(self.bns) - 1 and _FUSED_TAIL and training and grad and gpu and isinstance(last, GCNConv)
                and last.in_channels >= last.out_channels):
            if plain_adj and not sharded_adj and type(bn) is nn.BatchNorm1d and last.out_channels <= 64 and last.in_channels % 64 == 0:
                act = "tail"
            elif sharded_adj and hasattr(bn, "fused_act_linear"):
                act = "tail_sync"
        return conv_form, act

    def forward(self, x, adj_t):
        for li, (conv, bn) in enumerate(zip(self.convs[:-1], self.bns)):
            conv_form, act = self._layer_form(li, x, adj_t)
            if conv_form == "fold":
                x = self.out_feat = conv(x, adj_t, eval_bn=bn)
                continue
            x = conv(x, adj_t, bn_stats_shift=bn.running_mean, want_bn_stats=True) if conv_form == "stats" else conv(x, adj_t)
            if act in ("tail", "tail_sync"):
                both = (ops.bn_act_linear(x, bn, self.convs[-1].weight, relu=True, p=self.dropout, training=True) if act == "tail"
                        else bn.fused_act_linear(x, self.convs[-1].weight, True, self.dropout, True))
                if both is not None:
                    self.out_feat, xw = both
                    return self.convs[-1](self.out_feat, adj_t, xw=xw)
                act = "bn_act" if act == "tail" else "sync"
            if act == "bn_act":
                x = ops.bn_act(x, bn, relu=True, p=self.dropout, training=self.training)
            elif act == "sync":
                x = bn.fused_act(x, True, self.dropout, self.training)
            else:
                _lib.require_gpu(x)
                x = F.dropout(F.relu(bn(x)), p=self.dropout, training=self.training)
            self.out_feat = x
        if self.training and x.is_cuda:
            x = self.out_feat = ops.grad_tap(x)
        return self.convs[-1](x, adj_t)


class GCN(_Student):
    def __init__(self, in_channels, hidden_channels, out_channels, num_layers, dropout, cached=True):
        super().__init__(lambda a, b: GCNConv(a, b, cached=cached), in_channels, hidden_channels, out_channels,
                         num_layers, dropout)


class SAGE(_Student):
    def __init__(self, in_channels, hidden_channels, out_channels, num_layers, dropout, aggr="mean"):
        super().__init__(lambda a, b: SAGEConv(a, b, aggr=aggr), in_channels, hidden_channels, out_channels,
                         num_layers, dropout)


class ProjectionGCD(nn.Module):
    def __init__(self, hidden_channels, proj_dim):
        super().__init__()
        self.lin = nn.Linear(hidden_channels, proj_dim)
        self.conv = GCNConv(hidden_channels, proj_dim)
        self.bn = nn.BatchNorm1d(proj_dim)

    def forward(self, x, adj_t):
        return F.relu(self.bn(self.lin(x) + self.conv(x, adj_t)))


class ProjectionHead(nn.Sequential):

    def __init__(self, in_dim, proj_dim):
        super().__init__(nn.Linear(in_dim, proj_dim), nn.BatchNorm1d(proj_dim), nn.ReLU())

    def forward(self, x):
        lin, bn = self[0], self[1]
        if hasattr(bn, "fused_act"):
            return bn.fused_act(ops.linear(x, lin.weight, lin.bias), True, 0.0, self.training)
        _lib.require_gpu(x)
        if not isinstance(bn, nn.BatchNorm1d):
            return super().forward(x)
        return ops.bn_act(ops.linear(x, lin.weight, lin.bias), bn, relu=True, p=0.0, training=self.training)

    def forward_rows(self, x, idx, pick=None, const_input=False):
        lin, bn = self[0], self[1]
        y = ops.linear_rows(x, idx, lin.weight, lin.bias, const_input=const_input)
        if hasattr(bn, "fused_act"):
            return bn.fused_act(y, True, 0.0, self.training, pick=pick)
        if not isinstance(bn, nn.BatchNorm1d):
            y = self[2](bn(y))
            return y if pick is None else y[pick]
        return ops.bn_act(y, bn, relu=True, p=0.0, training=self.training, pick=pick)


def make_projection(in_dim, proj_dim):
    return ProjectionHead(in_dim, proj_dim)


_ROW_CACHE = _cache.TensorKeyedCache(capacity=8)
_CACHE_CONST_ROWS = os.environ.get("EGNN_CACHE_CONST_ROWS", "0") == "1"


def _const_rows(t, idx):
    if t.requires_grad or not _CACHE_CONST_ROWS:
        return t[idx]
    return _ROW_CACHE.get((t, idx), (), lambda: t[idx])


_GLOBAL_EDGES = _cache.TensorKeyedCache(capacity=8)
# ... 818 lines not shown
```

### efficient-gnns_amd/nn.py

```python
from __future__ import annotations

import math

import torch
from torch import Tensor, nn

from . import ops
import os

from . import _lib, ops_edge
from .sparse import SparseTensor, _ind2ptr, csr_from_coo, gcn_norm

_MEMOISE_AX = os.environ.get("EGNN_GCN_MEMOISE_AX", "0") == "1"
_SAGE_FUSED = True
_SAGE_NARROW_FIRST = True


def _adj_from_edge_index(edge_index: Tensor, n: int, value: Tensor | None = None) -> SparseTensor:
    src, dst = edge_index[0], edge_index[1]
    perm = torch.argsort(dst, stable=True)
    return SparseTensor(rowptr=_ind2ptr(dst[perm].contiguous(), n), col=src[perm],
                        value=None if value is None else value[perm], sparse_sizes=(n, n))


def _gcn_norm_edge_index(edge_index: Tensor, n: int) -> SparseTensor:
    src, dst = edge_index[0], edge_index[1]
    keep = src != dst
    loops = torch.arange(n, dtype=torch.int64, device=edge_index.device)
    src2, dst2 = torch.cat([src[keep], loops]), torch.cat([dst[keep], loops])
    w = torch.ones(src2.numel(), dtype=torch.float32, device=edge_index.device)
    deg = torch.zeros(n, dtype=torch.float32, device=edge_index.device).index_add_(0, dst2, w)
    dinv = deg.pow(-0.5)
    dinv.masked_fill_(dinv == float("inf"), 0.0)
    val = dinv[src2] * w * dinv[dst2]
    return _adj_from_edge_index(torch.stack([src2, dst2]), n, val)


from ._cache import TensorKeyedCache as _TensorKeyedCache


_GCN_NORM_CACHE = _TensorKeyedCache(capacity=64)


class GCNConv(nn.Module):

    def __init__(self, in_channels: int, out_channels: int, cached: bool = False, bias: bool = True, **_):
        super().__init__()
        self.in_channels, self.out_channels, self.cached = in_channels, out_channels, cached
        self.weight = nn.Parameter(torch.empty(in_channels, out_channels))
        self.bias = nn.Parameter(torch.empty(out_channels)) if bias else None
        self._cached_adj_t = None
        self._cached_ax = None
        self.reset_parameters()

    def reset_parameters(self):
        a = math.sqrt(6.0 / (self.in_channels + self.out_channels))
        with torch.no_grad():
            self.weight.uniform_(-a, a)
            if self.bias is not None:
                self.bias.zero_()
        self._cached_adj_t = None
        self._cached_ax = None

    def forward(self, x: Tensor, edge_index, edge_weight=None, bn_stats_shift: Tensor | None = None, want_bn_stats: bool = False,
                eval_bn=None, xw: Tensor | None = None) -> Tensor:
        if edge_weight is not None:
            raise NotImplementedError("GCNConv with edge_weight is not used by the reference")
        agg_first = self.in_channels < self.out_channels
        if eval_bn is not None:
            sharded = hasattr(edge_index, "gcn_normalized")
            if torch.is_grad_enabled() or eval_bn.training or not (isinstance(edge_index, SparseTensor) or sharded) or not x.is_cuda:
                raise ValueError("eval_bn: inference only (no_grad, BatchNorm in eval mode, SparseTensor / sharded adjacency on the GPU)")
            if sharded:
                w, b = ops.bn_fold(self.weight, self.bias, eval_bn)
                if agg_first:
                    return ops.gemm_raw(edge_index.gcn_normalized().aggregate(x, "sum"), w, False, False, b, relu=True)
                return edge_index.gcn_normalized().aggregate(ops.gemm_raw(x, w), "sum", bias=b, relu=True)
            norm = self._cached_adj_t
            if norm is None:
                norm = gcn_norm(edge_index)
                if self.cached:
                    self._cached_adj_t = norm
            w, b = ops.bn_fold(self.weight, self.bias, eval_bn)
            if agg_first:
                return ops.gemm_raw(ops.spmm_raw(norm, x, "sum")[0], w, False, False, b, relu=True)
            return ops.spmm_raw(norm, ops.gemm_raw(x, w), "sum", bias=b, relu=True)[0]
        if hasattr(edge_index, "gcn_normalized"):
            if agg_first:
                return ops.matmul(edge_index.gcn_normalized().aggregate(x, "sum"), self.weight, self.bias)
            return edge_index.gcn_normalized().aggregate(ops.matmul(x, self.weight) if xw is None else xw, "sum", bias=self.bias)
        norm = self._cached_adj_t
        if norm is None:
            if isinstance(edge_index, SparseTensor):
                norm = gcn_norm(edge_index)
            else:
                n_nodes = x.shape[0]
                norm = _GCN_NORM_CACHE.get((edge_index,), (n_nodes,), lambda: _gcn_norm_edge_index(edge_index, n_nodes))
            if self.cached:
                self._cached_adj_t = norm
        if (self.cached and _MEMOISE_AX and not x.requires_grad and self.in_channels <= self.out_channels
                and isinstance(edge_index, SparseTensor)):
            key = (x.data_ptr(), x._version, tuple(x.shape), id(norm))
            if self._cached_ax is None or self._cached_ax[0] != key:
                with torch.no_grad():
                    self._cached_ax = (key, ops.spmm_raw(norm, x, "sum")[0], x)
            out = ops.matmul(self._cached_ax[1], self.weight)
            return ops.add_bias(out, self.bias)
        if agg_first:
            return ops.matmul(ops.spmm(norm, x, "sum"), self.weight, self.bias)
        return ops.spmm(norm, ops.matmul(x, self.weight) if xw is None else xw, "sum", bias=self.bias,
                        bn_stats_shift=bn_stats_shift, want_bn_stats=want_bn_stats)

    def _uses_memoised_input(self, x: Tensor) -> bool:
        return bool(self.cached and _MEMOISE_AX and not x.requires_grad and self.in_channels <= self.out_channels)

    def __repr__(self):
        return f"GCNConv({self.in_channels}, {self.out_channels})"


class SAGEConv(nn.Module):

    def __init__(self, in_channels: int, out_channels: int, aggr: str = "mean", **_):
        super().__init__()
        if aggr == "add":
            aggr = "sum"
        if aggr not in ("mean", "sum", "max"):
            raise ValueError(f"unsupported aggregation '{aggr}'")
        self.in_channels, self.out_channels, self.aggr = in_channels, out_channels, aggr
        self.lin_l = nn.Linear(in_channels, out_channels, bias=True)
        self.lin_r = nn.Linear(in_channels, out_channels, bias=False)

    def reset_parameters(self):
        self.lin_l.reset_parameters()
        self.lin_r.reset_parameters()

    def forward(self, x: Tensor, edge_index) -> Tensor:
        if hasattr(edge_index, "aggregate"):
            if _SAGE_FUSED and hasattr(edge_index, "sage_layer"):
                out = edge_index.sage_layer(x, self.lin_l, self.lin_r, self.aggr, _SAGE_NARROW_FIRST and self.out_channels < self.in_channels)
                if out is not None:
                    return out
            agg = edge_index.aggregate(x, self.aggr, valueless=True)
            return ops.linear_add(agg, self.lin_l.weight, self.lin_l.bias, ops.linear(x, self.lin_r.weight, None))
        adj = edge_index if isinstance(edge_index, SparseTensor) else _adj_from_edge_index(edge_index, x.shape[0])
        if (_SAGE_FUSED and self.aggr in ("mean", "sum") and x.is_cuda and x.dim() == 2 and self.lin_r.bias is None
                and adj.nnz() > 0 and adj.sparse_size(0) == adj.sparse_size(1)):
            narrow = _SAGE_NARROW_FIRST and self.out_channels < self.in_channels
            return ops.sage_layer(x, adj.set_value(None), self.lin_l, self.lin_r, self.aggr, narrow)
        if _SAGE_NARROW_FIRST and self.out_channels < self.in_channels and self.aggr in ("mean", "sum") and x.is_cuda:
            return ops.spmm(adj.set_value(None), ops.linear(x, self.lin_l.weight, None), self.aggr, bias=self.lin_l.bias) \
                + ops.linear(x, self.lin_r.weight, None)
        agg = ops.spmm(adj.set_value(None), x, self.aggr)
        return ops.linear(agg, self.lin_l.weight, self.lin_l.bias) + ops.linear(x, self.lin_r.weight, None)

    def __repr__(self):
        return f"SAGEConv({self.in_channels}, {self.out_channels}, aggr={self.aggr})"


_GAT_STRUCT_CACHE = _TensorKeyedCache(capacity=64)


class GATConv(nn.Module):

    def __init__(self, in_channels: int, out_channels: int, heads: int = 1, concat: bool = True, negative_slope: float = 0.2,
                 dropout: float = 0.0, add_self_loops: bool = True, bias: bool = True, **_):
        super().__init__()
        self.in_channels, self.out_channels, self.heads, self.concat = in_channels, out_channels, heads, concat
        self.negative_slope, self.dropout, self.add_self_loops = negative_slope, dropout, add_self_loops
        self.lin_l = nn.Linear(in_channels, heads * out_channels, bias=False)
        self.lin_r = self.lin_l
        self.att_l = nn.Parameter(torch.empty(1, heads, out_channels))
        self.att_r = nn.Parameter(torch.empty(1, heads, out_channels))
        self.bias = nn.Parameter(torch.empty(heads * out_channels if concat else out_channels)) if bias else None
        self.reset_parameters()

    def reset_parameters(self):
        with torch.no_grad():
            for t in (self.lin_l.weight, self.att_l, self.att_r):
                a = math.sqrt(6.0 / (t.size(-2) + t.size(-1)))
                t.uniform_(-a, a)
            if self.bias is not None:
                self.bias.zero_()

    def _structure(self, adj, n: int) -> SparseTensor:
        keys = (adj._col, adj._rowptr) if isinstance(adj, SparseTensor) else (adj,)
        return _GAT_STRUCT_CACHE.get(keys, (n, self.add_self_loops), lambda: self._build_structure(adj, n))

    def _build_structure(self, adj, n: int) -> SparseTensor:
        if isinstance(adj, SparseTensor):
            src, dst = adj._col, adj._row()
        else:
            src, dst = adj[0], adj[1]
        if self.add_self_loops:
            keep = src != dst
# ... 200 lines not shown
```

### efficient-gnns_amd/ops.py

```python
from __future__ import annotations

import ctypes
import os

import torch
from torch import Tensor

from . import _cache, _lib

_REDUCE = {"sum": 0, "add": 0, "mean": 1, "max": 2}
_OVERLAP_HEAVY_ROWS = True
_SIDE_STREAMS: dict = {}


def _side_stream(device) -> "torch.cuda.Stream":
    key = torch.device(device).index
    if key not in _SIDE_STREAMS:
        _SIDE_STREAMS[key] = torch.cuda.Stream(device=device)
    return _SIDE_STREAMS[key]



def _rowmajor(x: Tensor) -> Tensor:
    if x.dtype != torch.float32:
        raise TypeError(f"expected float32, got {x.dtype}")
    if x.dim() != 2:
        raise ValueError("expected a 2-D tensor")
    if x.stride(1) != 1 or x.stride(0) < x.shape[1]:
        x = x.contiguous()
    return x


_SPMM_SCHEDULE = "blocks"


class HipStatsUnavailable(RuntimeError):
    """spmm_raw(want_stats=True) on a shape / schedule whose kernel has no statistics epilogue (callers fall back to the
    separate egnn_bn_stats_f32 pass)."""


def _spmm_desc(adj, rowptr, col, bits, x, y, red, src_scale, bias) -> ctypes.Structure:
    n_rows, n_src = adj.sparse_sizes()
    return _lib.Spmm(n_rows, n_src, x.shape[1], _lib.ptr(rowptr), _lib.ptr(col), bits, _lib.ptr(adj._value), _lib.ptr(src_scale),
                     _lib.ptr(bias), _lib.ptr(x), x.stride(0), _lib.ptr(y), y.stride(0), red)


def spmm_raw(adj, x: Tensor, reduce: str = "sum", src_scale: Tensor | None = None, use_plan: bool = True,
             bias: Tensor | None = None, out: Tensor | None = None, stat_shift: Tensor | None = None, want_stats: bool = False,
             addend: Tensor | None = None, relu: bool = False):
    fused = []
    res = _spmm_raw(adj, x, reduce, src_scale, use_plan, bias, out, stat_shift, want_stats, addend, relu, fused)
    if relu and not fused:
        res[0].clamp_(min=0)
    return res


def _spmm_raw(adj, x: Tensor, reduce: str = "sum", src_scale: Tensor | None = None, use_plan: bool = True,
              bias: Tensor | None = None, out: Tensor | None = None, stat_shift: Tensor | None = None, want_stats: bool = False,
              addend: Tensor | None = None, relu: bool = False, relu_fused: list | None = None):
    _lib.require_gpu(x, adj._col)
    x = _rowmajor(x)
    n_rows, n_src = adj.sparse_sizes()
    if x.shape[0] != n_src:
        raise ValueError(f"matmul: adjacency has {n_src} columns, x has {x.shape[0]} rows")
    K = x.shape[1]
    red = _REDUCE[reduce]
    if out is not None:
        if tuple(out.shape) != (n_rows, K) or out.stride(1) != 1 or out.dtype != torch.float32 or out.device != x.device:
            raise ValueError("spmm_raw: `out` must be a float32 [n_rows, K] view with unit column stride on x's device")
        y = out
    else:
        y = torch.empty(n_rows, K, dtype=torch.float32, device=x.device)
    arg = torch.empty(n_rows, K, dtype=torch.int64, device=x.device) if red == 2 else None
    if addend is not None:
        if red == 2 or tuple(addend.shape) != (n_rows, K) or addend.dtype != torch.float32:
            raise ValueError("spmm_raw: `addend` is a float32 [n_rows, K] matrix (sum / mean only)")
        addend = _rowmajor(addend)
    if adj.nnz() == 0:
        y.zero_()
        if bias is not None:
            y.add_(bias)
        if addend is not None:
            y.add_(addend)
        if arg is not None:
            arg.fill_(-1)
        if want_stats:
            raise HipStatsUnavailable()
        return y, arg
    rowptr, col, bits = adj._index_arrays()
    lib = _lib.load()
    op = _spmm_desc(adj, rowptr, col, bits, x, y, red, src_scale, bias)
    op_ref = ctypes.byref(op)
    float4_ok = (use_plan and red != 2 and K % 4 == 0 and x.stride(0) % 4 == 0 and x.data_ptr() % 16 == 0
                 and y.stride(0) % 4 == 0 and y.data_ptr() % 16 == 0 and (bias is None or bias.data_ptr() % 16 == 0))
    add_fused = addend is not None and addend.stride(0) % 4 == 0 and addend.data_ptr() % 16 == 0
    if (float4_ok and _SPMM_SCHEDULE == "blocks" and bits == 32 and K >= 64 and n_src * x.stride(0) * 4 < 2 ** 31 and n_rows > 0
            and (addend is None or add_fused)):
        from .sparse import BLK_ROWS, SEG_MAX
        hseg, crow, cptr, slots = adj._blk_plan()
        partial = adj._scratch("partial", (max(slots, 1), K))
        loc = adj._struct.get("locality")
        use_lds = loc is not None and n_rows == n_src and K % 32 == 0
        rows_blk = loc[0] if use_lds else BLK_ROWS
        n_blk = (n_rows + rows_blk - 1) // rows_blk
        flags = 4 | (8 if (relu and not want_stats) else 0)
        n_stat = lib.egnn_spmm_blk_stat_rows(n_rows, rows_blk, int(use_lds)) if want_stats else 0
        n_hub = crow.numel()
        stat_part = adj._scratch("stat", (n_stat + n_hub, 2, K)) if want_stats else None
        if stat_shift is not None:
            stat_shift = stat_shift.detach().contiguous()
        op.addend, op.ld_addend = _lib.ptr(addend), 0 if addend is None else addend.stride(0)
        op.stat_part, op.stat_shift, op.flags = _lib.ptr(stat_part), _lib.ptr(stat_shift) if want_stats else None, flags
        rc = lib.egnn_spmm_csr_blk_f32(op_ref, SEG_MAX, rows_blk, None, 0, _lib.ptr(loc[1]) if use_lds else None, _lib.ptr(hseg),
                                       hseg.shape[0], _lib.ptr(partial), _lib.stream())
        if rc == 0:
            if n_hub > 0:
                _lib.check(lib.egnn_spmm_combine_f32(op_ref, _lib.ptr(crow), _lib.ptr(cptr), n_hub, _lib.ptr(partial), n_stat, _lib.stream()),
                           "egnn_spmm_combine_f32")
            if not want_stats:
                if flags & 8 and relu_fused is not None:
                    relu_fused.append(True)
                return y, None
            mean = torch.empty(K, dtype=torch.float32, device=x.device)
            var = torch.empty(K, dtype=torch.float32, device=x.device)
            nws = lib.egnn_bn_stats_merge_ws_floats(K)
            ws = adj._scratch("statfold", (nws,))
            _lib.check(lib.egnn_bn_stats_merge_f32(_lib.ptr(stat_part), n_stat + n_hub, K, None, 0, None, 0,
                                                   _lib.ptr(stat_shift), n_rows, _lib.ptr(mean), _lib.ptr(var), _lib.ptr(ws), nws,
                                                   _lib.stream()), "egnn_bn_stats_merge_f32")
            return y, None, (mean, var)
        if rc != -4:
            _lib.check(rc, "egnn_spmm_csr_blk_f32")
        op.addend = op.stat_part = op.stat_shift = None
        op.ld_addend = op.flags = 0
    if want_stats:
        raise HipStatsUnavailable()
    if float4_ok and _SPMM_SCHEDULE in ("blocks", "segments"):
        seg, crow, cptr, slots = adj._seg_plan()
        partial = adj._scratch("partial", (max(slots, 1), K))
        rc = lib.egnn_spmm_csr_seg_f32(op_ref, _lib.ptr(seg), seg.shape[0], _lib.ptr(crow), _lib.ptr(cptr), crow.numel(), _lib.ptr(partial),
                                       slots, _lib.stream())
        if rc == 0:
            if addend is not None:
                y.add_(addend)
            return y, None
        if rc != -4:
            _lib.check(rc, "egnn_spmm_csr_seg_f32")
    short, mid, long_ = adj._row_plan() if use_plan else (None, None, None)

    def lst(t):
        return (None, 0) if t is None or t.numel() == 0 else (_lib.ptr(t), t.numel())

    def launch(s, m, l, stream):
        return lib.egnn_spmm_csr_f32(op_ref, _lib.ptr(arg), *lst(s), *lst(m), *lst(l), stream)

    heavy = use_plan and short is not None and short.numel() > 0 and (mid.numel() + long_.numel()) > 0
    if heavy and _OVERLAP_HEAVY_ROWS:
        main = torch.cuda.current_stream()
        side = _side_stream(x.device)
        fork = torch.cuda.Event()
        fork.record(main)
        side.wait_event(fork)
        rc = launch(None, mid, long_, side.cuda_stream)
        _lib.check(rc, "egnn_spmm_csr_f32")
        rc = launch(short, None, None, main.cuda_stream)
        join = torch.cuda.Event()
        join.record(side)
        main.wait_event(join)
        for t in (x, y, arg, adj._value, src_scale, bias):
            if t is not None:
                t.record_stream(side)
    else:
        rc = launch(short, mid, long_, _lib.stream())
    _lib.check(rc, "egnn_spmm_csr_f32")
    if addend is not None:
        y.add_(addend)
    return y, arg


class _SpMM(torch.autograd.Function):
    @staticmethod
    def forward(ctx, x, adj, reduce, bias=None, stat_shift=None, want_stats=False):
        b = None if bias is None else bias.detach().contiguous()
        stats = None
        if want_stats:
            try:
                y, arg, stats = spmm_raw(adj, x, reduce, bias=b, stat_shift=stat_shift, want_stats=True)
            except HipStatsUnavailable:
                y, arg = spmm_raw(adj, x, reduce, bias=b)
        else:
            y, arg = spmm_raw(adj, x, reduce, bias=b)
        ctx.adj, ctx.reduce, ctx.has_bias = adj, reduce, bias is not None
        ctx.tap_box = getattr(x, "_egnn_tap", None)
        if arg is not None:
            ctx.save_for_backward(arg)
        if stats is None:
            return y, None, None
        ctx.mark_non_differentiable(*stats)
        return y, stats[0], stats[1]

    @staticmethod
    def backward(ctx, gy, _gm=None, _gv=None):
        adj, reduce = ctx.adj, ctx.reduce
        gy = _rowmajor(gy)
        if reduce in ("sum", "add"):
            gx, _ = spmm_raw(adj.t(), gy, "sum")
        elif reduce == "mean":
            gx, _ = spmm_raw(adj.t(), gy, "sum", src_scale=adj._inv_rowcount())
        else:
            (arg,) = ctx.saved_tensors
            n_rows, n_src = adj.sparse_sizes()
            K = gy.shape[1]
            gx = torch.zeros(n_src, K, dtype=torch.float32, device=gy.device)
            if adj.nnz() == 0:
                return gx, None, None, (colsum(gy) if ctx.has_bias and ctx.needs_input_grad[3] else None), None, None
            _, col, bits = adj._index_arrays()
            rc = _lib.load().egnn_spmm_csr_max_bwd_f32(n_rows, K, _lib.ptr(col), bits, _lib.ptr(adj._value), _lib.ptr(arg),
                                                       _lib.ptr(gy), gy.stride(0), _lib.ptr(gx), gx.stride(0), _lib.stream())
            _lib.check(rc, "egnn_spmm_csr_max_bwd_f32")
        gb = colsum(gy) if ctx.has_bias and ctx.needs_input_grad[3] else None
        return _fresh(gx, ctx.tap_box), None, None, gb, None, None


def _fresh(g, tap_box):
    if g is not None and tap_box is not None:
        g._egnn_fresh_for = tap_box
    return g


def colsum(g: Tensor) -> Tensor:
    tag = getattr(g, "_egnn_colsum", None)
    if tag is not None and tag[1] == g._version and tag[0].shape[0] == g.shape[1]:
        return tag[0]
    _lib.require_gpu(g)
    if g.dim() != 2 or g.dtype != torch.float32 or g.shape[0] == 0:
        return g.sum(0)
    g = _rowmajor(g)
    n, C = g.shape
    lib = _lib.load()
    out = torch.empty(C, dtype=torch.float32, device=g.device)
    ws = torch.empty(lib.egnn_colsum_ws_floats(C), dtype=torch.float32, device=g.device)
    _lib.check(lib.egnn_colsum_f32(_lib.ptr(g), g.stride(0), n, C, _lib.ptr(out), _lib.ptr(ws), _lib.stream()), "egnn_colsum_f32")
    return out


class _AddBias(torch.autograd.Function):

    @staticmethod
    def forward(ctx, x, bias):
        return x + bias

    @staticmethod
    def backward(ctx, g):
        return g, (colsum(g) if ctx.needs_input_grad[1] else None)


def add_bias(x: Tensor, bias: Tensor | None) -> Tensor:
    if bias is None:
        return x
    _lib.require_gpu(x)
    return _AddBias.apply(x, bias)


def spmm(adj, x: Tensor, reduce: str = "sum", bias: Tensor | None = None, bn_stats_shift: Tensor | None = None,
         want_bn_stats: bool = False, addend: Tensor | None = None) -> Tensor:
    if reduce not in _REDUCE:
        raise ValueError(f"unknown reduce '{reduce}'")
    if addend is not None:
        if torch.is_grad_enabled() and (x.requires_grad or addend.requires_grad):
            raise NotImplementedError("spmm(addend=...) is a forward-only form")
        return spmm_raw(adj, x, reduce, bias=bias, addend=addend)[0]
    if bias is not None and (reduce == "max" or (x.shape[1] % 4 == 0 and bias.data_ptr() % 16 != 0)):
        return _SpMM.apply(x, adj, reduce, None)[0] + bias
    y, mean, var = _SpMM.apply(x, adj, reduce, bias, bn_stats_shift, bool(want_bn_stats) and reduce != "max")
    if mean is not None:
        y._egnn_bn_stats = (mean, var, y._version)
    return y


def spmm_max_piece(adj, x: Tensor, entry_id: Tensor | None = None, merge: bool = False, y: Tensor | None = None,
                   argmax: Tensor | None = None, src_scale: Tensor | None = None):
    _lib.require_gpu(x, adj._col)
    x = _rowmajor(x)
    n_rows, n_src = adj.sparse_sizes()
    if x.shape[0] != n_src:
        raise ValueError(f"spmm_max_piece: adjacency has {n_src} columns, x has {x.shape[0]} rows")
    K = x.shape[1]
    if merge:
        if (y is None or argmax is None or tuple(y.shape) != (n_rows, K) or tuple(argmax.shape) != (n_rows, K) or y.dtype != torch.float32
                or argmax.dtype != torch.int64 or y.stride(1) != 1 or not argmax.is_contiguous()):
            raise ValueError("spmm_max_piece(merge=True) needs the float32 [n_rows, K] / contiguous int64 [n_rows, K] state of the earlier pieces")
    else:
        y = torch.empty(n_rows, K, dtype=torch.float32, device=x.device)
        argmax = torch.empty(n_rows, K, dtype=torch.int64, device=x.device)
    if n_rows == 0 or K == 0:
        return y, argmax
    if adj.nnz() == 0:
        if not merge:
            y.zero_()
            argmax.fill_(-1)
        return y, argmax
    if entry_id is not None and (entry_id.dtype != torch.int64 or entry_id.numel() != adj.nnz() or not entry_id.is_contiguous()):
        raise ValueError("spmm_max_piece: `entry_id` is a contiguous int64 [nnz] vector")
    rowptr, col, bits = adj._index_arrays()
    op = _spmm_desc(adj, rowptr, col, bits, x, y, _REDUCE["max"], src_scale, None)
    rc = _lib.load().egnn_spmm_csr_max_piece_f32(ctypes.byref(op), _lib.ptr(entry_id), int(bool(merge)), _lib.ptr(argmax), _lib.stream())
    _lib.check(rc, "egnn_spmm_csr_max_piece_f32")
    return y, argmax


def spmm_max_bwd_rows(t_adj, t_eid: Tensor, val: Tensor | None, argmax: Tensor, gy: Tensor, addend: Tensor | None = None) -> Tensor:
    _lib.require_gpu(gy, t_adj._col)
    gy = _rowmajor(gy)
    n_src, n_rows = t_adj.sparse_sizes()
    K = gy.shape[1]
    if gy.shape[0] != n_rows or tuple(argmax.shape) != (n_rows, K) or argmax.dtype != torch.int64 or not argmax.is_contiguous():
        raise ValueError("spmm_max_bwd_rows: dY is [n_rows, K] and argmax a contiguous int64 [n_rows, K]")
    if addend is not None:
        if tuple(addend.shape) != (n_src, K):
            raise ValueError("spmm_max_bwd_rows: `addend` is a float32 [n_src, K] matrix")
        addend = _rowmajor(addend)
    gx = torch.empty(n_src, K, dtype=torch.float32, device=gy.device)
    if n_src == 0 or K == 0:
        return gx
    if t_adj.nnz() == 0:
        return gx.zero_() if addend is None else gx.copy_(addend)
    if t_eid.dtype != torch.int64 or t_eid.numel() != t_adj.nnz() or not t_eid.is_contiguous():
        raise ValueError("spmm_max_bwd_rows: `t_eid` is a contiguous int64 [nnz] vector")
    rowptr, col, bits = t_adj._index_arrays()
    rc = _lib.load().egnn_spmm_csr_max_bwd_rows_f32(n_src, n_rows, K, _lib.ptr(rowptr), _lib.ptr(col), bits, _lib.ptr(t_eid), _lib.ptr(val),
                                                    _lib.ptr(argmax), _lib.ptr(gy), gy.stride(0), _lib.ptr(addend),
                                                    0 if addend is None else addend.stride(0), _lib.ptr(gx), gx.stride(0), _lib.stream())
    _lib.check(rc, "egnn_spmm_csr_max_bwd_rows_f32")
    return gx


class _TakeRows(torch.autograd.Function):

    @staticmethod
    def forward(ctx, x, idx):
        ctx.save_for_backward(idx)
        ctx.n = x.shape[0]
        return x.index_select(0, idx)

    @staticmethod
    def backward(ctx, g):
        (idx,) = ctx.saved_tensors
        gx = torch.zeros(ctx.n, *g.shape[1:], dtype=g.dtype, device=g.device)
        gx.index_copy_(0, idx, g)
        return gx, None


def take_rows(x: Tensor, idx: Tensor) -> Tensor:
    return _TakeRows.apply(x, idx)


def gemm_backend() -> str:
    return "hip"

# ... 546 lines not shown
    es, et = torch.empty(n, dtype=torch.float32, device=dev), torch.empty(n, dtype=torch.float32, device=dev)
    sumsq = torch.empty(2, dtype=torch.float32, device=dev)
    nws = lib.egnn_feature_loss_ws_floats(n)
    ws = torch.empty(nws, dtype=torch.float32, device=dev)
    _lib.check(lib.egnn_at_energy_f32(_lib.ptr(f), f.stride(0), f.shape[1], _lib.ptr(t), t.stride(0), t.shape[1], n, _lib.ptr(es), _lib.ptr(et),
                                      _lib.ptr(sumsq), _lib.ptr(ws), nws, _lib.stream()), "egnn_at_energy_f32")
    return es, et, sumsq


def at_partial(es: Tensor, et: Tensor, sumsq_global: Tensor, eps: float = 1e-12):
    _lib.require_gpu(es, et, sumsq_global)
    n, dev = es.shape[0], sumsq_global.device
    sums = torch.empty(3, dtype=torch.float32, device=dev)
    scal = torch.empty(4, dtype=torch.float32, device=dev)
    if n == 0:
        return scal, sums.zero_()
    lib = _lib.load()
    nws = lib.egnn_feature_loss_ws_floats(n)
    ws = torch.empty(nws, dtype=torch.float32, device=dev)
    _lib.check(lib.egnn_at_partial_f32(_lib.ptr(es), _lib.ptr(et), n, _lib.ptr(sumsq_global), float(eps), _lib.ptr(scal), _lib.ptr(sums),
                                       _lib.ptr(ws), nws, _lib.stream()), "egnn_at_partial_f32")
    return scal, sums


def at_rows_bwd(f: Tensor, t: Tensor, n_global: int, es: Tensor, et: Tensor, scal: Tensor, sums_global: Tensor, g: Tensor,
                eps: float = 1e-12, need_df: bool = True, need_dt: bool = True):
    _lib.require_gpu(f, t)
    f, t = _rowmajor(f), _rowmajor(t)
    n = f.shape[0]
    df = torch.empty_like(f) if need_df else None
    dt = torch.empty_like(t) if need_dt else None
    if n == 0:
        return df, dt
    g = g.contiguous().to(torch.float32).reshape(1)
    _lib.check(_lib.load().egnn_at_bwd_rows_f32(_lib.ptr(f), f.stride(0), f.shape[1], _lib.ptr(t), t.stride(0), t.shape[1], n, int(n_global),
                                                _lib.ptr(es), _lib.ptr(et), _lib.ptr(scal), _lib.ptr(sums_global), float(eps), _lib.ptr(g),
                                                _lib.ptr(df), 0 if df is None else df.stride(0), _lib.ptr(dt),
                                                0 if dt is None else dt.stride(0), _lib.stream()), "egnn_at_bwd_rows_f32")
    return df, dt


class _NCE(torch.autograd.Function):
    @staticmethod
    def forward(ctx, fhat, that, tau):
        _lib.require_gpu(fhat, that)
        fhat, that = fhat.contiguous(), that.contiguous()
        S, P = fhat.shape
        if that.shape != fhat.shape:
            raise ValueError("nce: student and teacher features must have the same shape")
        lib = _lib.load()
        dev = fhat.device
        Z = torch.empty(S, S, dtype=torch.float32, device=dev)
        lse = torch.empty(S, dtype=torch.float32, device=dev)
        loss = torch.empty(1, dtype=torch.float32, device=dev)
        nws = lib.egnn_nce_ws_floats(S)
        ws = torch.empty(nws, dtype=torch.float32, device=dev)
        rc = lib.egnn_nce_fwd_f32(_lib.ptr(fhat), _lib.ptr(that), S, P, fhat.stride(0), float(tau), 1, _lib.ptr(Z), _lib.ptr(lse),
                                  _lib.ptr(loss), _lib.ptr(ws), nws, _lib.stream())
        _lib.check(rc, "egnn_nce_fwd_f32")
        ctx.save_for_backward(fhat, that, Z, lse)
        ctx.tau = float(tau)
        return loss[0]

    @staticmethod
    def backward(ctx, g):
        fhat, that, Z, lse = ctx.saved_tensors
        S, P = fhat.shape
        g = g.contiguous().to(torch.float32)
        df = torch.empty_like(fhat) if ctx.needs_input_grad[0] else None
        dt = torch.empty_like(that) if ctx.needs_input_grad[1] else None
        lib = _lib.load()
        nws = lib.egnn_nce_bwd_ws_floats(S, S, P)
        ws = torch.empty(nws, dtype=torch.float32, device=fhat.device)
        rc = lib.egnn_nce_bwd_f32(_lib.ptr(fhat), _lib.ptr(that), S, P, fhat.stride(0), ctx.tau, 1, _lib.ptr(Z), _lib.ptr(lse),
                                  _lib.ptr(g), _lib.ptr(df), _lib.ptr(dt), _lib.ptr(ws), nws, _lib.stream())
        _lib.check(rc, "egnn_nce_bwd_f32")
        return df, dt, None


def nce_unit(fhat: Tensor, that: Tensor, tau: float) -> Tensor:
    return _NCE.apply(fhat, that, tau)


def nce_block_fwd(fhat: Tensor, t_all: Tensor, diag_off: int, tau: float, inv_count: float, unit_rows: bool = True):
    _lib.require_gpu(fhat, t_all)
    Sr, P = fhat.shape
    Sc = t_all.shape[0]
    lib, dev = _lib.load(), fhat.device
    Z = torch.empty(Sr, Sc, dtype=torch.float32, device=dev)
    lse = torch.empty(Sr, dtype=torch.float32, device=dev)
    loss = torch.empty(1, dtype=torch.float32, device=dev)
    nws = lib.egnn_nce_ws_floats(Sr)
    ws = torch.empty(nws, dtype=torch.float32, device=dev)
    rc = lib.egnn_nce_block_fwd_f32(_lib.ptr(fhat), fhat.stride(0), _lib.ptr(t_all), t_all.stride(0), Sr, Sc, diag_off, P, float(tau),
                                    float(inv_count), int(unit_rows), _lib.ptr(Z), _lib.ptr(lse), _lib.ptr(loss), _lib.ptr(ws), nws, _lib.stream())
    _lib.check(rc, "egnn_nce_block_fwd_f32")
    return Z, lse, loss


def nce_block_bwd(fhat: Tensor, t_all: Tensor, diag_off: int, scale: float, Z: Tensor, lse: Tensor, g: Tensor, tau: float,
                  unit_rows: bool = True):
    Sr, P = fhat.shape
    Sc = t_all.shape[0]
    df, dt = torch.empty_like(fhat), torch.empty_like(t_all)
    nws = _lib.load().egnn_nce_bwd_ws_floats(Sr, Sc, P)
    ws = torch.empty(nws, dtype=torch.float32, device=fhat.device)
    rc = _lib.load().egnn_nce_block_bwd_f32(_lib.ptr(fhat), fhat.stride(0), _lib.ptr(t_all), t_all.stride(0), Sr, Sc, diag_off, P,
                                            float(tau), float(scale), int(unit_rows), _lib.ptr(Z), _lib.ptr(lse), _lib.ptr(g), _lib.ptr(df), df.stride(0),
                                            _lib.ptr(dt), dt.stride(0), _lib.ptr(ws), nws, _lib.stream())
    _lib.check(rc, "egnn_nce_block_bwd_f32")
    return df, dt


_DROPOUT_SEED_DEV: Tensor | None = None


def _draw_dropout_seed() -> int:
    return int(torch.empty((), dtype=torch.int64).random_()) & 0x7FFFFFFFFFFFFFFF


def _bn_shape_ok(x: Tensor) -> bool:
    C = x.shape[1]
    return x.is_cuda and C % 4 == 0 and C <= 1024 and x.stride(0) % 4 == 0 and x.data_ptr() % 16 == 0


_NO_PICKED_ROW = ctypes.c_int64(-1)


def _bn_desc(x, gamma, beta, mean, var, eps, relu, p, seed, seed_dev, pick=None) -> ctypes.Structure:
    n, C = x.shape
    pick_ptr = None if pick is None else (pick.data_ptr() or ctypes.addressof(_NO_PICKED_ROW))
    return _lib.BnAct(_lib.ptr(x), x.stride(0), n, C, _lib.ptr(mean), _lib.ptr(var), float(eps), _lib.ptr(gamma), _lib.ptr(beta),
                      int(relu), float(p), int(seed), _lib.ptr(seed_dev), pick_ptr, 0 if pick is None else pick.numel())


def _sync_sums(sums: Tensor, sync) -> Tensor:
    import torch.distributed as dist
    total, group = sync
    if dist.get_world_size(group) > 1:
        sums = sums.clone()
        dist.all_reduce(sums, group=group)
    return sums / total


def _bn_act_fwd(x, gamma, beta, mean, var, eps, relu, p, seed, seed_dev, pick=None) -> Tensor:
    n, C = x.shape
    y = torch.empty(n if pick is None else pick.numel(), C, dtype=torch.float32, device=x.device)
    if y.shape[0] == 0:
        return y
    bn = _bn_desc(x, gamma, beta, mean, var, eps, relu, p, seed, seed_dev, pick)
    _lib.check(_lib.load().egnn_bn_act_fwd_f32(ctypes.byref(bn), _lib.ptr(y), y.stride(0), _lib.stream()), "egnn_bn_act_fwd_f32")
    return y


class _BnAct(torch.autograd.Function):

    @staticmethod
    def forward(ctx, x, gamma, beta, mean, var, eps, relu, p, seed, batch_stats, pick=None, sync=None):
        if not x.is_cuda:
            raise RuntimeError(f"bn_act: the HIP kernels need a GPU tensor, got one on {x.device}")
        x = _rowmajor(x)
        n = x.shape[0]
        if pick is not None and (pick.dtype != torch.int64 or pick.dim() != 1 or not pick.is_contiguous() or pick.numel() > n
                                 or (sync is None and pick.numel() == 0)):
            raise ValueError("bn_act: `pick` must be a non-empty contiguous 1-D int64 tensor of unique row ids" if sync is None else
                             "sync_bn_act: `pick` must be a contiguous 1-D int64 tensor of unique row ids")
        seed_dev = _DROPOUT_SEED_DEV if p > 0 else None
        y = _bn_act_fwd(x, gamma, beta, mean, var, eps, relu, p, seed, seed_dev, pick)
        ctx.save_for_backward(x, gamma, beta, mean, var, *([] if pick is None else [pick]))
        ctx.cfg = (float(eps), int(relu), float(p), int(seed), int(batch_stats))
        ctx.seed_dev, ctx.sync = seed_dev, sync
        return y

    @staticmethod
    def backward(ctx, gy):
        x, gamma, beta, mean, var = ctx.saved_tensors[:5]
        pick = ctx.saved_tensors[5] if len(ctx.saved_tensors) > 5 else None
        eps, relu, p, seed, batch_stats = ctx.cfg
        gy = _rowmajor(gy)
        n, C = x.shape
        lib, dev = _lib.load(), x.device
        bn = ctypes.byref(_bn_desc(x, gamma, beta, mean, var, eps, relu, p, seed, ctx.seed_dev, pick))
        sums = torch.empty(2 * C, dtype=torch.float32, device=dev)
        dx = torch.empty_like(x)
        nws = lib.egnn_bn_ws_floats(C)
        ws = torch.empty(nws, dtype=torch.float32, device=dev) if n > 0 else None
        cs = torch.empty(C, dtype=torch.float32, device=dev) if (batch_stats and n > 0) else None
        if ctx.sync is None:
            _lib.check(lib.egnn_bn_act_bwd_f32(bn, _lib.ptr(gy), gy.stride(0), batch_stats, _lib.ptr(sums[C:]), _lib.ptr(sums), _lib.ptr(dx),
                                               dx.stride(0), _lib.ptr(cs), _lib.ptr(ws), nws, _lib.stream()), "egnn_bn_act_bwd_f32")
        else:
            if (n if pick is None else pick.numel()) > 0:
                _lib.check(lib.egnn_bn_act_bwd_reduce_f32(bn, _lib.ptr(gy), gy.stride(0), _lib.ptr(sums[C:]), _lib.ptr(sums), _lib.ptr(ws),
                                                          nws, _lib.stream()), "egnn_bn_act_bwd_reduce_f32")
            else:
                sums.zero_()
            scaled = _sync_sums(sums, ctx.sync)
            if n > 0:
                _lib.check(lib.egnn_bn_act_bwd_apply_f32(bn, _lib.ptr(gy), gy.stride(0), _lib.ptr(scaled), _lib.ptr(scaled[C:]), 1.0,
                                                         _lib.ptr(sums), _lib.ptr(dx), dx.stride(0), _lib.ptr(cs), _lib.ptr(ws), nws,
                                                         _lib.stream()), "egnn_bn_act_bwd_apply_f32")
        if cs is not None:
            dx._egnn_colsum = (cs, dx._version)
        return dx, sums[C:], sums[:C], None, None, None, None, None, None, None, None, None


def _bn_prepare(x: Tensor, bn, p: float, training: bool):
    x_in = x
    if not _bn_shape_ok(_rowmajor(x)) or not bn.track_running_stats or bn.weight is None:
        return None
    x = _rowmajor(x)
    n, C = x.shape
    use_batch = training
    if use_batch:
        lib, dev = _lib.load(), x.device
        pre = getattr(x_in, "_egnn_bn_stats", None)
        if pre is not None and pre[0].shape[0] == C and pre[2] == x_in._version:
            mean, var = pre[0], pre[1]
        else:
            mean = torch.empty(C, dtype=torch.float32, device=dev)
            var = torch.empty(C, dtype=torch.float32, device=dev)
            nws = lib.egnn_bn_ws_floats(C)
            ws = torch.empty(nws, dtype=torch.float32, device=dev)
            _lib.check(lib.egnn_bn_stats_f32(_lib.ptr(x), x.stride(0), n, C, _lib.ptr(mean), _lib.ptr(var), _lib.ptr(ws), nws, _lib.stream()),
                       "egnn_bn_stats_f32")
        with torch.no_grad():
            rm, rv, nbt = bn.running_mean, bn.running_var, bn.num_batches_tracked
            if rm.dtype == torch.float32 and rv.dtype == torch.float32 and nbt.dtype == torch.int64 and rm.is_contiguous() and rv.is_contiguous():
                _lib.check(lib.egnn_bn_running_update_f32(_lib.ptr(mean), _lib.ptr(var), C, n, -1.0 if bn.momentum is None else float(bn.momentum),
                                                          _lib.ptr(rm), _lib.ptr(rv), _lib.ptr(nbt), _lib.stream()), "egnn_bn_running_update_f32")
            else:
                bn.num_batches_tracked += 1
                m = bn.momentum if bn.momentum is not None else 1.0 / float(bn.num_batches_tracked)
                bn.running_mean.mul_(1 - m).add_(mean, alpha=m)
                bn.running_var.mul_(1 - m).add_(var, alpha=m * n / max(n - 1, 1))
    else:
        mean, var = bn.running_mean, bn.running_var
    drop = p if (training and p > 0) else 0.0
    seed = _draw_dropout_seed() if drop > 0 else 0
    return x, mean, var, use_batch, drop, seed


def bn_act(x: Tensor, bn: "torch.nn.BatchNorm1d", relu: bool = True, p: float = 0.0, training: bool | None = None,
           pick: Tensor | None = None) -> Tensor:
    training = bn.training if training is None else training
    prep = _bn_prepare(x, bn, p, training)
    if prep is None:
        y = bn(x)
        y = torch.relu(y) if relu else y
        y = torch.nn.functional.dropout(y, p, training) if p > 0 else y
        return y if pick is None else y[pick]
    x, mean, var, use_batch, drop, seed = prep
    return _BnAct.apply(x, bn.weight, bn.bias, mean, var, bn.eps, relu, drop, seed, use_batch, pick)


_INV_ROWS = _cache.TensorKeyedCache(capacity=16)


def _inverse_rows(idx: Tensor, n: int) -> Tensor:
    def build():
        inv = torch.full((n,), -1, dtype=torch.int32, device=idx.device)
        inv[idx] = torch.arange(idx.numel(), dtype=torch.int32, device=idx.device)
        return inv
    return _INV_ROWS.get((idx,), (n,), build)


def _bn_act_linear_fwd(x, w, gamma, beta, mean, var, eps, relu, p, seed, seed_dev):
    n, C = x.shape
    if n > 0 and w.stride(0) % 4 == 0 and w.data_ptr() % 16 == 0:
        h = torch.empty(n, C, dtype=torch.float32, device=x.device)
        xw = torch.empty(n, w.shape[1], dtype=torch.float32, device=x.device)
        bn = _bn_desc(x, gamma, beta, mean, var, eps, relu, p, seed, seed_dev)
        rc = _lib.load().egnn_bn_act_linear_fwd_f32(ctypes.byref(bn), _lib.ptr(w), w.stride(0), 0, w.shape[1], _lib.ptr(h), h.stride(0),
                                                    _lib.ptr(xw), xw.stride(0), _lib.stream())
        if rc != _lib.EGNN_EALIGN:
            _lib.check(rc, "egnn_bn_act_linear_fwd_f32")
            return h, xw
    h = _bn_act_fwd(x, gamma, beta, mean, var, eps, relu, p, seed, seed_dev)
    return h, (gemm_raw(h, w, False, False) if n > 0 else torch.empty(0, w.shape[1], dtype=torch.float32, device=x.device))


class _BnActLinear(torch.autograd.Function):

    @staticmethod
    def forward(ctx, x, gamma, beta, mean, var, eps, relu, p, seed, batch_stats, w, box, sync=None):
        x = _rowmajor(x)
        w = _rowmajor(w)
        seed_dev = _DROPOUT_SEED_DEV if p > 0 else None
        h, xw = _bn_act_linear_fwd(x, w, gamma, beta, mean, var, eps, relu, p, seed, seed_dev)
        ctx.save_for_backward(x, gamma, beta, mean, var, h, w)
        ctx.cfg = (float(eps), int(relu), float(p), int(seed), int(batch_stats))
        ctx.seed_dev, ctx.box, ctx.w_index, ctx.sync = seed_dev, box, 10, sync
        ctx.set_materialize_grads(False)
        return h, xw

    @staticmethod
    def backward(ctx, g_h, g_xw):
        x, gamma, beta, mean, var, h, w = ctx.saved_tensors
        eps, relu, p, seed, batch_stats = ctx.cfg
        dx, dgamma, dbeta, gw = _tail_backward(ctx, g_h, g_xw, x, gamma, beta, mean, var, h, w, eps, relu, p, seed, batch_stats, ctx.sync)
        return dx, dgamma, dbeta, None, None, None, None, None, None, None, gw, None, None


def _tail_backward(ctx, g_h, g_xw, x, gamma, beta, mean, var, h, w, eps, relu, p, seed, batch_stats, sync):
    pend = []
    if ctx.box is not None:
        pend, ctx.box.pending = ctx.box.pending, []
        pend = [(i, r) for i, r in pend if r.shape[0] > 0]
    n, C = x.shape
    Ks = w.shape[1]
    lib, dev = _lib.load(), x.device
# ... 414 lines not shown
```

### include/egnn_hip.h

```cpp
#ifndef EGNN_HIP_H
#define EGNN_HIP_H

#include <stddef.h>
#include <stdint.h>

#ifdef __cplusplus
extern "C" {
#endif

#define EGNN_OK 0
#define EGNN_EINVAL (-1)
#define EGNN_ELAUNCH (-2)
#define EGNN_EWORKSPACE (-3)
#define EGNN_EALIGN (-4)

#define EGNN_ABI_VERSION 9
int egnn_abi_version(void);
const char* egnn_error_string(int code);
int egnn_build_info(char* buf, size_t buf_bytes);

#define EGNN_SUM 0
#define EGNN_MEAN 1
#define EGNN_MAX 2

typedef struct egnn_spmm {
  int64_t n_rows; int64_t n_src; int64_t K;
  const void* rowptr; const void* col; int index_bits;
  const float* val; const float* src_scale; const float* bias;
  const float* X; int64_t ldx;
  float* Y; int64_t ldy;
  int reduce;
  const float* addend; int64_t ld_addend;
  float* stat_part; const float* stat_shift;
  int flags;
} egnn_spmm_t;

int egnn_spmm_csr_f32(const egnn_spmm_t* op, int64_t* argmax, const int64_t* short_rows, int64_t n_short,
                      const int64_t* mid_rows, int64_t n_mid, const int64_t* long_rows, int64_t n_long, void* stream);

int egnn_spmm_csr_seg_f32(const egnn_spmm_t* op, const int64_t* seg, int64_t n_seg, const int64_t* comb_rows,
                          const int64_t* comb_ptr, int64_t n_comb, float* partial, int64_t partial_slots, void* stream);

int egnn_spmm_csr_blk_f32(const egnn_spmm_t* op, int seg_max, int rows_per_blk, const int32_t* blk_ptr, int64_t n_blk,
                          const int32_t* win, const int32_t* hub_seg, int64_t n_hub_seg, float* partial, void* stream);
int64_t egnn_spmm_blk_stat_rows(int64_t n_rows, int rows_per_blk, int lds);
int egnn_spmm_blk_window_i32(const int32_t* rowptr, const int32_t* col, int64_t n_rows, int rows_per_blk,
                             const int32_t* blk_ptr, int64_t n_blk, int32_t* win, void* stream);
size_t egnn_bn_stats_merge_ws_floats(int64_t C);
int egnn_bn_stats_merge_f32(const float* stat_part, int64_t n_blk, int64_t C, const float* Y, int64_t ldy,
                            const int64_t* extra_rows, int64_t n_extra, const float* stat_shift, int64_t n_total,
                            float* mean, float* var, float* ws, size_t ws_floats, void* stream);

int egnn_spmm_combine_f32(const egnn_spmm_t* op, const int64_t* comb_rows, const int64_t* comb_ptr, int64_t n_comb,
                          const float* partial, int64_t stat_base, void* stream);

int egnn_spmm_csr_max_bwd_f32(int64_t n_rows, int64_t K, const void* col, int index_bits, const float* val,
                              const int64_t* argmax, const float* dY, int64_t ldy, float* dX, int64_t ldx,
                              void* stream);

int egnn_spmm_csr_max_piece_f32(const struct egnn_spmm* op, const int64_t* entry_id, int merge, int64_t* argmax, void* stream);

int egnn_spmm_csr_max_bwd_rows_f32(int64_t n_src, int64_t n_rows, int64_t K, const void* t_rowptr, const void* t_row, int index_bits,
                                   const int64_t* t_eid, const float* val, const int64_t* argmax, const float* dY, int64_t ldy,
                                   const float* addend, int64_t ld_addend, float* dX, int64_t ldx, void* stream);

int64_t egnn_spmm_algorithmic_bytes(int64_t n_rows, int64_t n_src, int64_t K, int64_t nnz, int index_bits,
                                    int has_val);

size_t egnn_csr_from_coo_ws_bytes(int64_t E, int64_t N, int symmetric);
int egnn_csr_from_coo_i64(const int64_t* row, const int64_t* col, int64_t E, int64_t N, int symmetric,
                          int64_t* rowptr, int64_t* col_out, int64_t* nnz_out, void* ws, size_t ws_bytes, void* stream);

size_t egnn_csr_transpose_ws_bytes(int64_t nnz, int64_t n_cols);
int egnn_csr_transpose_i64(const int64_t* rowptr, const int64_t* col, int64_t n_rows, int64_t n_cols, int64_t nnz,
                           int64_t* colptr, int64_t* row_out, int64_t* perm, void* ws, size_t ws_bytes, void* stream);

int egnn_rowptr_from_sorted_rows_i64(const int64_t* row, int64_t nnz, int64_t n_rows, int64_t* rowptr, void* stream);

int egnn_narrow_i64_to_i32(const int64_t* src, int64_t n, int32_t* dst, int32_t* overflow, void* stream);

int egnn_gcn_norm_count_i64(const int64_t* rowptr, const int64_t* col, int64_t n, int64_t* out_count, void* stream);
int egnn_gcn_norm_fill_i64(const int64_t* rowptr, const int64_t* col, int64_t n, const int64_t* rowptr_out,
                           int64_t* col_out, float* dinv, void* stream);
int egnn_gcn_norm_values_i64(const int64_t* rowptr_out, const int64_t* col_out, int64_t n, const float* dinv,
                             float* val_out, void* stream);

size_t egnn_gemm_ws_floats(int trans_a, int trans_b, int64_t M, int64_t N, int64_t K, int split_k);
int egnn_gemm_f32(int trans_a, int trans_b, int64_t M, int64_t N, int64_t K, float alpha,
                  const float* A, int64_t lda, const float* B, int64_t ldb,
                  const float* bias, float* C, int64_t ldc,
                  int split_k, float* ws, size_t ws_bytes, void* stream);

int egnn_gemm_ex_f32(int trans_a, int trans_b, int64_t M, int64_t N, int64_t K, float alpha, const float* A, int64_t lda,
                     const float* B, int64_t ldb, const float* bias, float* C, int64_t ldc, int split_k, float* ws,
                     size_t ws_bytes, int flags, void* stream);
int egnn_gemm_add_f32(int trans_a, int trans_b, int64_t M, int64_t N, int64_t K, float alpha, const float* A, int64_t lda,
                      const float* B, int64_t ldb, const float* bias, const float* addend, int64_t ld_addend, float* C, int64_t ldc,
                      int split_k, float* ws, size_t ws_bytes, void* stream);
int egnn_gemm_rows_f32(int trans_a, int trans_b, int64_t M, int64_t N, int64_t K, float alpha,
                       const float* A, int64_t lda, const int64_t* a_rows, const float* B, int64_t ldb, const int64_t* b_rows,
                       const float* bias, float* C, int64_t ldc,
                       int split_k, float* ws, size_t ws_bytes, void* stream);

size_t egnn_gemm_tn_planes_bytes(int64_t N, int64_t K);
int egnn_gemm_tn_planes_pack_f32(const float* B, int64_t ldb, const int64_t* b_rows, int64_t N, int64_t K, void* planes,
                                 size_t planes_bytes, void* stream);
size_t egnn_gemm_tn_planes_ws_floats(int64_t M, int64_t N, int64_t K);
int egnn_gemm_tn_planes_f32(int64_t M, int64_t N, int64_t K, float alpha, const float* A, int64_t lda, const void* planes, float* C,
                            int64_t ldc, float* ws, size_t ws_floats, void* stream);

size_t egnn_gemm_rows_planes_bytes(int64_t M, int64_t K);
int egnn_gemm_rows_planes_pack_f32(const float* A, int64_t lda, const int64_t* a_rows, int64_t M, int64_t K, void* planes,
                                   size_t planes_bytes, void* stream);
size_t egnn_gemm_rows_planes_ws_bytes(int64_t N, int64_t K);
int egnn_gemm_rows_planes_f32(int64_t M, int64_t N, int64_t K, float alpha, const void* planes_a, const float* B, int64_t ldb,
                              const float* bias, float* C, int64_t ldc, void* ws, size_t ws_bytes, void* stream);


size_t egnn_ce_kd_ws_floats(int64_t n);
int egnn_ce_kd_fwd_f32(const float* logits, int64_t ld_logits, const float* teacher, int64_t ld_teacher,
                       const int64_t* labels, const int64_t* rows, int64_t n, int64_t C, float T,
                       float* out3, float* partials, void* stream);
int egnn_ce_kd_bwd_f32(const float* logits, int64_t ld_logits, const float* teacher, int64_t ld_teacher,
                       const int64_t* labels, const int64_t* rows, int64_t n_total_rows, int64_t n, int64_t C, float T,
                       const float* out3, const float* g_cls, const float* g_kd, float* dlogits, int64_t ld_dlogits,
                       void* stream);

int egnn_gather_normalize_rows_f32(const float* x, int64_t ldx, const int64_t* idx, int64_t n, int64_t D, float eps,
                                   float* out, int64_t ldo, float* inv_norm, void* stream);
int egnn_normalize_rows_bwd_f32(const float* xhat, int64_t ldh, const float* dout, int64_t ldd, const float* inv_norm,
                                const int64_t* idx, int64_t n, int64_t D, float eps,
                                float* dx, int64_t ldx, int accumulate, void* stream);

size_t egnn_nce_ws_floats(int64_t S);
size_t egnn_nce_bwd_ws_floats(int64_t Sr, int64_t Sc, int64_t P);
int egnn_nce_saves_exp(float tau, int unit_rows);
int egnn_nce_fwd_f32(const float* fhat, const float* that, int64_t S, int64_t P, int64_t ld, float tau, int unit_rows,
                     float* Z, float* lse, float* loss, float* ws, size_t ws_floats, void* stream);
int egnn_nce_bwd_f32(const float* fhat, const float* that, int64_t S, int64_t P, int64_t ld, float tau, int unit_rows,
                     const float* Z, const float* lse, const float* g,
                     float* dfhat, float* dthat, float* ws, size_t ws_floats, void* stream);

int egnn_nce_block_fwd_f32(const float* fhat, int64_t ld_f, const float* that, int64_t ld_t, int64_t Sr, int64_t Sc,
                           int64_t diag_off, int64_t P, float tau, float inv_count, int unit_rows, float* Z, float* lse,
                           float* loss, float* ws, size_t ws_floats, void* stream);
int egnn_nce_block_bwd_f32(const float* fhat, int64_t ld_f, const float* that, int64_t ld_t, int64_t Sr, int64_t Sc,
                           int64_t diag_off, int64_t P, float tau, float scale, int unit_rows, const float* Z,
                           const float* lse, const float* g, float* dfhat, int64_t ld_df, float* dthat, int64_t ld_dt,
                           float* ws, size_t ws_floats, void* stream);

#define EGNN_K_COSINE 0
#define EGNN_K_POLY 1
#define EGNN_K_L2 2
#define EGNN_K_RBF 3
size_t egnn_gsp_ws_floats(int64_t S);
int egnn_gsp_fwd_f32(const float* xs, int64_t ld_s, int64_t Ps, const float* xt, int64_t ld_t, int64_t Pt, int64_t S,
                     int kernel, float* Ws, float* Wt, float* loss, float* ws, size_t ws_floats, void* stream);
int egnn_rowsum_f32(const float* W, int64_t ld, int64_t n, int64_t m, float* out, void* stream);
int egnn_scale_rowcorr_f32(const float* WX, int64_t ldw, const float* X, int64_t ldx, const float* r, const float* g,
                           int64_t n, int64_t P, float* out, int64_t ldo, void* stream);

size_t egnn_bce_pair_ws_floats(void);
int egnn_bce_pair_fwd_f32(const float* logits, const float* labels, const float* teacher, int64_t total, float* out2,
                          float* ws, void* stream);
int egnn_bce_pair_bwd_f32(const float* logits, const float* labels, const float* teacher, int64_t total,
                          const float* g_cls, const float* g_kd, float* dlogits, void* stream);

int egnn_edge_sim_f32(const float* F, int64_t ld, int64_t D, const int64_t* idx_a, const int64_t* idx_b, int64_t E,
                      int kernel, float* sim, float* aux3, void* stream);
int egnn_edge_sim_coef_f32(const float* g, const float* sim, const float* aux3, int64_t E, int kernel,
                           float* alpha, float* beta_a, float* beta_b, void* stream);
int egnn_segment_softmax_fwd_f32(const int64_t* seg_ptr, const float* x, int64_t n_seg, float* p, void* stream);
int egnn_segment_softmax_bwd_f32(const int64_t* seg_ptr, const float* p, const float* gp, int64_t n_seg, float* gx, void* stream);
int egnn_segment_sum_f32(const int64_t* seg_ptr, const float* x, int64_t n_seg, float* out, void* stream);

size_t egnn_lsp_loss_ws_floats(void);
int egnn_lsp_loss_fwd_f32(const int64_t* seg_ptr, const float* sim_s, const float* sim_t, int64_t n_seg, int64_t E,
                          int criterion, float* p_s, float* p_t, float* loss, float* ws, void* stream);
int egnn_lsp_loss_bwd_f32(const int64_t* seg_ptr, const float* p_s, const float* p_t, int64_t n_seg, int64_t E,
                          int criterion, const float* g, float* gsim_s, float* gsim_t, void* stream);

size_t egnn_colsum_ws_floats(int64_t C);
int egnn_colsum_f32(const float* x, int64_t ld, int64_t n, int64_t C, float* out, float* ws, void* stream);

int egnn_gat_attention_fwd_f32(const int64_t* rowptr, const int64_t* col, const float* alpha_src, const float* alpha_dst,
                               int64_t n_rows, int64_t nnz, int H, float negative_slope, float* att, void* stream);

typedef struct egnn_gat_layer {
  const int64_t* rowptr; const int64_t* col;
  const int64_t* colptr; const int64_t* t_col; const int64_t* perm;
  int64_t n; int64_t nnz; int H; int C;
  const float* xl; int64_t ld_xl;
  const float* el; const float* er;
  const float* attn_l; const float* attn_r;
  const uint8_t* keep; const float* mult; const float* src_scale; const float* dst_scale;
  float negative_slope;
} egnn_gat_layer_t;
int egnn_gat_layer_fwd_f32(const egnn_gat_layer_t* layer, float* att, float* out, int64_t ld_out, void* stream);
size_t egnn_gat_layer_bwd_ws_floats(int64_t n, int H, int C);
int egnn_gat_layer_bwd_f32(const egnn_gat_layer_t* layer, const float* att, const float* go, int64_t ld_go, int mean_heads, float* d_raw,
                           float* d_er, float* dxl, int64_t ld_dxl, float* d_attn, float* ws, size_t ws_floats, void* stream);

typedef struct egnn_bn_act {
  const float* x; int64_t ld; int64_t n; int64_t C;
  const float* mean; const float* var; float eps;
  const float* gamma; const float* beta;
  int relu; float p; uint64_t seed; const uint64_t* seed_dev;
  const int64_t* pick; int64_t n_pick;
} egnn_bn_act_t;

size_t egnn_bn_ws_floats(int64_t C);
int egnn_bn_stats_f32(const float* x, int64_t ld, int64_t n, int64_t C, float* mean, float* var, float* ws, size_t ws_floats,
                      void* stream);
int egnn_bn_act_fwd_f32(const egnn_bn_act_t* bn, float* y, int64_t ldy, void* stream);
int egnn_bn_act_bwd_f32(const egnn_bn_act_t* bn, const float* dy, int64_t ld_dy, int batch_stats, float* dgamma, float* dbeta,
                        float* dx, int64_t ld_dx, float* dx_colsum, float* ws, size_t ws_floats, void* stream);
int egnn_bn_act_bwd_reduce_f32(const egnn_bn_act_t* bn, const float* dy, int64_t ld_dy, float* dgamma, float* dbeta, float* ws,
                               size_t ws_floats, void* stream);
int egnn_bn_act_bwd_apply_f32(const egnn_bn_act_t* bn, const float* dy, int64_t ld_dy, const float* sum_dbeta, const float* sum_dgamma,
                              float inv_count, const float* local_dbeta, float* dx, int64_t ld_dx, float* dx_colsum, float* ws,
                              size_t ws_floats, void* stream);

int egnn_bn_merge_shards_f32(const float* stats, int world, int64_t C, float* mean, float* var, float* total, void* stream);

int egnn_bn_act_linear_fwd_f32(const egnn_bn_act_t* bn, const float* W, int64_t ldw, int w_kmajor, int64_t Ks, float* h, int64_t ldh,
                               float* xw, int64_t ld_xw, void* stream);
size_t egnn_skinny_dx_bn_ws_floats(int64_t M, int64_t C);
int egnn_skinny_dx_bn_bwd_reduce_f32(const float* G, int64_t ldg, const float* W, int64_t ldw, int w_kmajor, int64_t Ks, float alpha,
                                     const float* addend, int64_t ld_addend, const float* add_rows, int64_t ld_add_rows,
                                     const int32_t* add_inv, const egnn_bn_act_t* bn, float* dgamma, float* dbeta, float* dx,
                                     int64_t ld_dx, float* ws, size_t ws_floats, void* stream);
int egnn_bn_bwd_apply_stored_f32(const egnn_bn_act_t* bn, const float* sum_dbeta, const float* sum_dgamma, float inv_count, float* dx,
                                 int64_t ld_dx, float* dx_colsum, float* ws, size_t ws_floats, void* stream);

int egnn_bn_running_update_f32(const float* mean, const float* var, int64_t C, int64_t n, float momentum, float* running_mean,
                               float* running_var, int64_t* num_batches_tracked, void* stream);
int egnn_bn_running_update_dev_f32(const float* mean, const float* var, int64_t C, const float* total_rows, float momentum,
                                   float* running_mean, float* running_var, int64_t* num_batches_tracked, void* stream);

int egnn_bn_fold_f32(const float* W, int64_t ldw, int64_t rows, int64_t C, const float* bias, const float* mean, const float* var,
                     const float* gamma, const float* beta, float eps, float* W_out, int64_t ld_out, float* bias_out, void* stream);

size_t egnn_split_accuracy_ws_ints(void);
int egnn_split_accuracy_f32(const float* logits, int64_t ld, int64_t n, int64_t C, const int64_t* y, const int8_t* split_id,
                            double* acc3, int32_t* ws, size_t ws_ints, void* stream);
int egnn_split_counts_f32(const float* logits, int64_t ld, int64_t n, int64_t C, const int64_t* y, const int8_t* split_id,
                          double* out6, int32_t* ws, size_t ws_ints, void* stream);

int egnn_rows_add_f32(float* dst, int64_t ld_dst, const int64_t* idx, const float* src, int64_t ld_src, int64_t n, int64_t C,
                      void* stream);

size_t egnn_feature_loss_ws_floats(int64_t n);
int egnn_fitnet_fwd_f32(const float* f, int64_t ldf, const float* t, int64_t ldt, int64_t n, int64_t D, float eps, float* loss,
                        float* ws, size_t ws_floats, void* stream);
int egnn_fitnet_bwd_f32(const float* f, int64_t ldf, const float* t, int64_t ldt, int64_t n, int64_t D, float eps, const float* g,
                        float* df, int64_t lddf, float* dt, int64_t lddt, void* stream);

int egnn_at_fwd_f32(const float* f, int64_t ldf, int64_t Df, const float* t, int64_t ldt, int64_t Dt, int64_t n, float eps, float* loss,
                    float* ws, size_t ws_floats, void* stream);
int egnn_at_bwd_f32(const float* f, int64_t ldf, int64_t Df, const float* t, int64_t ldt, int64_t Dt, int64_t n, float eps, const float* ws,
                    const float* g, float* df, int64_t lddf, float* dt, int64_t lddt, void* stream);

int egnn_at_energy_f32(const float* f, int64_t ldf, int64_t Df, const float* t, int64_t ldt, int64_t Dt, int64_t n, float* es, float* et,
                       float* sumsq, float* ws, size_t ws_floats, void* stream);
int egnn_at_partial_f32(const float* es, const float* et, int64_t n, const float* sumsq_global, float eps, float* scal, float* sums,
                        float* ws, size_t ws_floats, void* stream);
int egnn_at_bwd_rows_f32(const float* f, int64_t ldf, int64_t Df, const float* t, int64_t ldt, int64_t Dt, int64_t n, int64_t n_global,
                         const float* es, const float* et, const float* scal, const float* sums_global, float eps, const float* g,
                         float* df, int64_t lddf, float* dt, int64_t lddt, void* stream);

int64_t egnn_saint_induced_geometry(int which);
int egnn_saint_random_walk_i64(const int64_t* rowptr, const int64_t* col, int64_t N, int64_t nnz, int64_t B, int64_t L,
                               const int64_t* start, const float* rand, uint64_t seed, const uint64_t* seed_dev, int64_t* walks,
                               uint8_t* flag, void* stream);
size_t egnn_saint_scan_ws_bytes(int64_t items);
int egnn_saint_select_i64(const uint8_t* flag, int64_t N, int64_t* relabel, int64_t* node_idx, int64_t node_cap, void* ws,
                          size_t ws_bytes, void* stream);
int egnn_saint_induced_count_i64(const int64_t* rowptr, const int64_t* col, const int64_t* row_map, int64_t n_map,
                                 const int64_t* n_map_dev, int64_t groups, int64_t group_stride, int64_t N, const uint8_t* flag,
                                 int64_t* counts, int64_t* out_ptr, void* ws, size_t ws_bytes, void* stream);
int egnn_saint_induced_fill_i64(const int64_t* rowptr, const int64_t* col, const int64_t* val, const int64_t* row_map, int64_t n_map,
                                const int64_t* n_map_dev, int64_t groups, int64_t group_stride, int64_t N, const uint8_t* flag,
                                const int64_t* relabel, const int64_t* out_ptr, int64_t out_cap, int64_t* out_row, int64_t* out_col,
                                int64_t* out_val, void* stream);
int egnn_saint_gather_i64(const int64_t* node_idx, int64_t n_sub, const int64_t* node_type, const int64_t* local_idx, const int64_t* y,
                          const uint8_t* train_mask, int64_t* o_node_type, int64_t* o_local_idx, int64_t* o_y, uint8_t* o_train_mask,
                          const int64_t* edge_idx, int64_t e_sub, const int64_t* edge_attr, int64_t* o_edge_attr, void* stream);

typedef struct egnn_sign_seg {
  int64_t B; int64_t Cs; int H;
  float p; const uint64_t* seed; const uint64_t* seed_dev;
  const float* const* slope;
  const float* const* src; const int64_t* ld_src; int64_t n_src;
  const int64_t* batch;
} egnn_sign_seg_t;
int egnn_sign_gather_drop_f32(const egnn_sign_seg_t* seg, float* out, int64_t ld_out, void* stream);
// ... 46 lines not shown
```

Measured before the change: 159.5.

## Fuse row normalization into NCE and BN running-stat update into stats kernels

Adds a fused NCE path that takes raw gathered features and folds the L2-normalization backward into the NCE gradient split-reduce kernel, so normalized gradients are written straight to the input rows. Separately, the BatchNorm statistics final kernel now also updates running mean, variance and the batch counter, removing the separate running-update launch. Both changes are meant to cut kernel launches and intermediate tensor round-trips in the G-CRD training step. They add new code paths with fallbacks when the fused reduce does not apply (P>256, or no split reduce), and a guard against in-place modification after a producer has already updated the stats.

```diff
diff --git a/efficient-gnns_amd/_lib.py b/efficient-gnns_amd/_lib.py
--- a/efficient-gnns_amd/_lib.py
+++ b/efficient-gnns_amd/_lib.py
@@ -70,6 +70,7 @@
     "egnn_spmm_blk_window_i32": (_i32, [_p, _p, _i64, _i32, _p, _i64, _p, _p]),
     "egnn_bn_stats_merge_ws_floats": (_sz, [_i64]),
     "egnn_bn_stats_merge_f32": (_i32, [_p, _i64, _i64, _p, _i64, _p, _i64, _p, _i64, _p, _p, _p, _sz, _p]),
+    "egnn_bn_stats_merge_update_f32": (_i32, [_p, _i64, _i64, _p, _i64, _p, _i64, _p, _i64, _p, _p, _p, _sz, _f32, _p, _p, _p, _p]),
     "egnn_spmm_combine_f32": (_i32, [_p, _p, _p, _i64, _p, _i64, _p]),
     "egnn_spmm_csr_max_bwd_f32": (_i32, [_i64, _i64, _p, _i32, _p, _p, _p, _i64, _p, _i64, _p]),
     "egnn_spmm_csr_max_piece_f32": (_i32, [_p, _p, _i32, _p, _p]),
@@ -108,6 +109,7 @@
     "egnn_nce_saves_exp": (_i32, [_f32, _i32]),
     "egnn_nce_bwd_ws_floats": (_sz, [_i64, _i64, _i64]),
     "egnn_nce_bwd_f32": (_i32, [_p, _p, _i64, _i64, _i64, _f32, _i32, _p, _p, _p, _p, _p, _p, _sz, _p]),
+    "egnn_nce_bwd_norm_f32": (_i32, [_p, _p, _i64, _i64, _i64, _f32, _p, _p, _p, _f32, _p, _p, _p, _i64, _p, _p, _p, _i64, _p, _p, _p, _sz, _p]),
     "egnn_nce_block_fwd_f32": (_i32, [_p, _i64, _p, _i64, _i64, _i64, _i64, _i64, _f32, _f32, _i32, _p, _p, _p, _p, _sz, _p]),
     "egnn_nce_block_bwd_f32": (_i32, [_p, _i64, _p, _i64, _i64, _i64, _i64, _i64, _f32, _f32, _i32, _p, _p, _p, _p, _i64, _p, _i64, _p, _sz, _p]),
     "egnn_gsp_ws_floats": (_sz, [_i64]),
@@ -133,6 +135,7 @@
     "egnn_colsum_f32": (_i32, [_p, _i64, _i64, _i64, _p, _p, _p]),
     "egnn_bn_ws_floats": (_sz, [_i64]),
     "egnn_bn_stats_f32": (_i32, [_p, _i64, _i64, _i64, _p, _p, _p, _sz, _p]),
+    "egnn_bn_stats_update_f32": (_i32, [_p, _i64, _i64, _i64, _p, _p, _p, _sz, _f32, _p, _p, _p, _p]),
     "egnn_bn_act_fwd_f32": (_i32, [_p, _p, _i64, _p]),
     "egnn_bn_act_bwd_f32": (_i32, [_p, _p, _i64, _i32, _p, _p, _p, _i64, _p, _p, _sz, _p]),
     "egnn_bn_act_bwd_reduce_f32": (_i32, [_p, _p, _i64, _p, _p, _p, _sz, _p]),
diff --git a/efficient-gnns_amd/criterion.py b/efficient-gnns_amd/criterion.py
--- a/efficient-gnns_amd/criterion.py
+++ b/efficient-gnns_amd/criterion.py
@@ -130,9 +130,7 @@
 def rows_nce_criterion(logits, labels, feat, teacher_feat, beta=0.5, nce_T=0.075, max_samples=8192, rows=None, presampled=False, *, _cls=None):
     loss_cls = (_cls or _ce_term)(logits, labels, rows)
     idx = None if presampled else _sample_rows(feat.shape[0], max_samples, feat.device)
-    fhat = ops.gather_normalize(*_rows_of(feat, idx))
-    that = ops.gather_normalize(*_rows_of(teacher_feat, idx))
-    loss_aux = ops.nce_unit(fhat, that, nce_T)
+    loss_aux = ops.nce_normalized(*_rows_of(feat, idx), *_rows_of(teacher_feat, idx), nce_T)
     return torch.add(loss_cls, loss_aux, alpha=beta), loss_cls, loss_aux
 
 
diff --git a/efficient-gnns_amd/csrc/fused_bn.hip b/efficient-gnns_amd/csrc/fused_bn.hip
--- a/efficient-gnns_amd/csrc/fused_bn.hip
+++ b/efficient-gnns_amd/csrc/fused_bn.hip
@@ -89,14 +89,23 @@
 }
 
 __global__ __launch_bounds__(256) void bn_stats_final_kernel(const float* __restrict__ part, int nblocks, const float* __restrict__ x,
-                                                             int64_t n, int64_t C, float* __restrict__ mean, float* __restrict__ var) {
+                                                             int64_t n, int64_t C, float* __restrict__ mean, float* __restrict__ var,
+                                                             float unbias, float m, float* __restrict__ rmean, float* __restrict__ rvar,
+                                                             long long* __restrict__ tracked) {
   float a, b; bool owner; int64_t c;
   merge_partials(part, nblocks, C, a, b, owner, c);
   if (!owner) return;
   const float inv = 1.f / (float)n;
   const float m1 = a * inv;
-  mean[c] = x[c] + m1;
-  var[c] = fmaxf(b * inv - m1 * m1, 0.f);
+  const float mu = x[c] + m1;
+  const float v = fmaxf(b * inv - m1 * m1, 0.f);
+  mean[c] = mu;
+  var[c] = v;
+  if (rmean) {
+    rmean[c] = (1.f - m) * rmean[c] + m * mu;
+    rvar[c] = (1.f - m) * rvar[c] + (m * unbias) * v;
+    if (c == 0 && tracked) tracked[0] = tracked[0] + 1;
+  }
 }
 
 __global__ __launch_bounds__(256) void bn_act_fwd_kernel(const BnParams q, float* __restrict__ y, int64_t ldy) {
@@ -384,7 +393,28 @@
   const int64_t want = (n + 3) / 4;
   const int nb = (int)(want < kStatBlocks ? want : kStatBlocks);
   hipLaunchKernelGGL(bn_stats_partial_kernel, dim3(nb), dim3(256), 0, st, x, ld, n, C, ws);
-  hipLaunchKernelGGL(bn_stats_final_kernel, dim3((unsigned)((C + kMergeCols - 1) / kMergeCols)), dim3(256), 0, st, ws, nb, x, n, C, mean, var);
+  hipLaunchKernelGGL(bn_stats_final_kernel, dim3((unsigned)((C + kMergeCols - 1) / kMergeCols)), dim3(256), 0, st, ws, nb, x, n, C, mean, var,
+                     1.f, 0.f, (float*)nullptr, (float*)nullptr, (long long*)nullptr);
+  return egnn_launch_status();
+}
+
+extern "C" int egnn_bn_stats_update_f32(const float* x, int64_t ld, int64_t n, int64_t C, float* mean, float* var, float* ws,
+                                        size_t ws_floats, float momentum, float* running_mean, float* running_var,
+                                        int64_t* num_batches_tracked, void* stream) {
+  EGNN_CHECK_ARG(n > 0 && x && mean && var && ws && ld >= C && running_mean && running_var);
+  if (momentum < 0.f) {
+    const int rc = egnn_bn_stats_f32(x, ld, n, C, mean, var, ws, ws_floats, stream);
+    return rc != EGNN_OK ? rc : egnn_bn_running_update_f32(mean, var, C, n, momentum, running_mean, running_var, num_batches_tracked, stream);
+  }
+  if (!shape_ok(x, ld, C)) return EGNN_EALIGN;
+  if (ws_floats < egnn_bn_ws_floats(C)) return EGNN_EWORKSPACE;
+  hipStream_t st = (hipStream_t)stream;
+  const int64_t want = (n + 3) / 4;
+  const int nb = (int)(want < kStatBlocks ? want : kStatBlocks);
+  const float unbias = n > 1 ? (float)n / (float)(n - 1) : 1.f;
+  hipLaunchKernelGGL(bn_stats_partial_kernel, dim3(nb), dim3(256), 0, st, x, ld, n, C, ws);
+  hipLaunchKernelGGL(bn_stats_final_kernel, dim3((unsigned)((C + kMergeCols - 1) / kMergeCols)), dim3(256), 0, st, ws, nb, x, n, C, mean, var,
+                     unbias, momentum, running_mean, running_var, (long long*)num_batches_tracked);
   return egnn_launch_status();
 }
 
diff --git a/efficient-gnns_amd/csrc/nce.hip b/efficient-gnns_amd/csrc/nce.hip
--- a/efficient-gnns_amd/csrc/nce.hip
+++ b/efficient-gnns_amd/csrc/nce.hip
@@ -402,6 +402,70 @@
   }
 }
 
+struct NormTail {
+  const float* xhat; int64_t ldh;
+  const float* inv_norm;
+  const int64_t* idx;
+  float eps;
+  float* dx; int64_t ldx;
+};
+constexpr int kTailCols = 256;
+
+template <int AMAJ, bool EXPZ>
+__global__ __launch_bounds__(256) void nce_bwd_reduce_norm_kernel(const float* __restrict__ ws, int nsplit, int64_t M, int64_t P, int64_t Kd,
+                                                                  int64_t diag_off, const float* __restrict__ lse, float shift,
+                                                                  const float* __restrict__ Im, int64_t ldi, float coef,
+                                                                  const float* __restrict__ g, const NormTail nt) {
+  const int lane = egnn_lane();
+  const int64_t total = M * P;
+  const float scale = coef * (g ? g[0] : 1.f);
+  for (int64_t row = blockIdx.x * 4LL + egnn_wave_id(); row < M; row += (int64_t)gridDim.x * 4) {
+    float gv[kTailCols / 64];
+#pragma unroll
+    for (int j = 0; j < kTailCols / 64; ++j) {
+      const int64_t c = lane + 64 * j;
+      gv[j] = 0.f;
+      if (c < P) {
+        float v = 0.f;
+        for (int k = 0; k < nsplit; ++k) v += ws[(int64_t)k * total + row * P + c];
+        gv[j] = nce_bwd_finish<AMAJ, EXPZ>(v, row, c, Kd, diag_off, lse, shift, Im, ldi, scale);
+      }
+    }
+    const float* hp = nt.xhat + row * nt.ldh;
+    const float inv = nt.inv_norm[row];
+    float dot = 0.f;
+#pragma unroll
+    for (int j = 0; j < kTailCols / 64; ++j) {
+      const int64_t c = lane + 64 * j;
+      if (c < P) dot = fmaf(gv[j], hp[c], dot);
+    }
+    dot = egnn_wave_sum(dot);
+    if (inv >= 1.f / nt.eps) dot = 0.f;
+    float* xp = nt.dx + (nt.idx ? nt.idx[row] : row) * nt.ldx;
+#pragma unroll
+    for (int j = 0; j < kTailCols / 64; ++j) {
+      const int64_t c = lane + 64 * j;
+      if (c < P) xp[c] = inv * (gv[j] - hp[c] * dot);
+    }
+  }
+}
+
+template <int AMAJ, bool EXPZ>
+void launch_bwd_reduce(const float* ws, int nsplit, int64_t M, int64_t P, int64_t Kd, int64_t diag_off, const float* lse, float shift,
+                       const float* Im, int64_t ldi, float coef, const float* g, float* C, int64_t ldc, const NormTail* nt, bool* tail_done,
+                       hipStream_t st) {
+  if (nt && nt->dx && P <= kTailCols) {
+    const int64_t rb = (M + 3) / 4;
+    hipLaunchKernelGGL((nce_bwd_reduce_norm_kernel<AMAJ, EXPZ>), dim3((unsigned)(rb < 16384 ? rb : 16384)), dim3(256), 0, st, ws, nsplit, M, P,
+                       Kd, diag_off, lse, shift, Im, ldi, coef, g, *nt);
+    *tail_done = true;
+    return;
+  }
+  const int64_t rb = (M * P + 255) / 256;
+  hipLaunchKernelGGL((nce_bwd_reduce_kernel<AMAJ, EXPZ>), dim3((unsigned)(rb < 4096 ? rb : 4096)), dim3(256), 0, st, ws, nsplit, M, P, Kd,
+                     diag_off, lse, shift, Im, ldi, coef, g, C, ldc);
+}
+
 __global__ __launch_bounds__(256) void nce_row_weight_kernel(const float* __restrict__ x, int64_t ldx, const float* __restrict__ lse,
                                                              float shift, int64_t n, int64_t P, float* __restrict__ out) {
   const int64_t total = n * P;
@@ -476,7 +540,8 @@
 
 template <int AMAJ>
 int launch_bwd3(const float* Z, int64_t ldz, int64_t M, int64_t Kd, int64_t diag_off, const float* lse, float shift, const float* Bm, int64_t P,
-                int64_t ldb, const float* Im, int64_t ldi, float coef, const float* g, float* C, int64_t ldc, float* ws, hipStream_t st) {
+                int64_t ldb, const float* Im, int64_t ldi, float coef, const float* g, float* C, int64_t ldc, float* ws, hipStream_t st,
+                const NormTail* nt = nullptr, bool* tail_done = nullptr) {
   using namespace egnn_gemm3;
   float* partial = ws;
   const int kNce3Split = nce3_split(M);
@@ -499,18 +564,16 @@
                                                                    k_per_split, partial);
   }
   if (rc != EGNN_OK) return rc;
-  const int64_t rb = (M * P + 255) / 256;
-  hipLaunchKernelGGL((nce_bwd_reduce_kernel<AMAJ, true>), dim3((unsigned)(rb < 4096 ? rb : 4096)), dim3(256), 0, st, partial, kNce3Split, M, P, Kd,
-                     diag_off, lse, shift, Im, ldi, coef, g, C, ldc);
+  launch_bwd_reduce<AMAJ, true>(partial, kNce3Split, M, P, Kd, diag_off, lse, shift, Im, ldi, coef, g, C, ldc, nt, tail_done, st);
   return EGNN_OK;
 }
 
 template <int AMAJ>
 int launch_bwd(const float* Z, int64_t ldz, int64_t M, int64_t Kd, int64_t diag_off, const float* lse, float shift, bool expz,
                 const float* Bm, int64_t P, int64_t ldb, const float* Im, int64_t ldi, float coef, const float* g, float* C,
-                int64_t ldc, bool vec4, float* ws, hipStream_t st) {
+                int64_t ldc, bool vec4, float* ws, hipStream_t st, const NormTail* nt = nullptr, bool* tail_done = nullptr) {
   if (nce3_takes<AMAJ>(M, Kd, P, ldz, Z, expz, vec4, ws)) {
-    return launch_bwd3<AMAJ>(Z, ldz, M, Kd, diag_off, lse, shift, Bm, P, ldb, Im, ldi, coef, g, C, ldc, ws, st);
+    return launch_bwd3<AMAJ>(Z, ldz, M, Kd, diag_off, lse, shift, Bm, P, ldb, Im, ldi, coef, g, C, ldc, ws, st, nt, tail_done);
   }
   const int64_t tiles_n = (P + 127) / 128;
   const int64_t t128 = ((M + 127) / 128) * tiles_n;
@@ -531,11 +594,7 @@
     if (split) rc = launch_dyn_lds<nce_bwd_kernel<128, AMAJ, true, true, false, true>>(grid, dim3(256), shm_split, st, EGNN_NCE_BWD_ARGS(wx, P));
     else rc = launch_dyn_lds<nce_bwd_kernel<128, AMAJ, true, true, false, false>>(grid, dim3(256), shm_f32, st, EGNN_NCE_BWD_ARGS(wx, P));
     if (rc != EGNN_OK) return rc;
-    if (nsplit > 1) {
-      const int64_t rb = (M * P + 255) / 256;
-      hipLaunchKernelGGL((nce_bwd_reduce_kernel<AMAJ, true>), dim3((unsigned)(rb < 4096 ? rb : 4096)), dim3(256), 0, st, ws, nsplit, M, P, Kd,
-                         diag_off, lse, shift, Im, ldi, coef, g, C, ldc);
-    }
+    if (nsplit > 1) launch_bwd_reduce<AMAJ, true>(ws, nsplit, M, P, Kd, diag_off, lse, shift, Im, ldi, coef, g, C, ldc, nt, tail_done, st);
     return EGNN_OK;
   }
 #define EGNN_NCE_BWD(BM_, V, E, S_) rc_main = launch_dyn_lds<nce_bwd_kernel<BM_, AMAJ, V, E, true, S_>>(grid, dim3(256), S_ ? shm_split : (size_t)TileShape<BM_, 128>::SMEM_FLOATS * 4, st, EGNN_NCE_BWD_ARGS(Bm, ldb))
@@ -554,10 +613,8 @@
 #undef EGNN_NCE_BWD_ARGS
   if (rc_main != EGNN_OK) return rc_main;
   if (nsplit > 1) {
-    const int64_t blocks = (M * P + 255) / 256;
-    const dim3 rgrid((unsigned)(blocks < 4096 ? blocks : 4096));
-    if (expz) hipLaunchKernelGGL((nce_bwd_reduce_kernel<AMAJ, true>), rgrid, dim3(256), 0, st, ws, nsplit, M, P, Kd, diag_off, lse, shift, Im, ldi, coef, g, C, ldc);
-    else hipLaunchKernelGGL((nce_bwd_reduce_kernel<AMAJ, false>), rgrid, dim3(256), 0, st, ws, nsplit, M, P, Kd, diag_off, lse, shift, Im, ldi, coef, g, C, ldc);
+    if (expz) launch_bwd_reduce<AMAJ, true>(ws, nsplit, M, P, Kd, diag_off, lse, shift, Im, ldi, coef, g, C, ldc, nt, tail_done, st);
+    else launch_bwd_reduce<AMAJ, false>(ws, nsplit, M, P, Kd, diag_off, lse, shift, Im, ldi, coef, g, C, ldc, nt, tail_done, st);
   }
   return EGNN_OK;
 }
@@ -620,10 +677,10 @@
   return egnn_launch_status();
 }
 
-extern "C" int egnn_nce_block_bwd_f32(const float* fhat, int64_t ld_f, const float* that, int64_t ld_t, int64_t Sr, int64_t Sc,
-                                      int64_t diag_off, int64_t P, float tau, float scale, int unit_rows, const float* Z,
-                                      const float* lse, const float* g, float* dfhat, int64_t ld_df, float* dthat, int64_t ld_dt,
-                                      float* ws, size_t ws_floats, void* stream) {
+static int nce_block_bwd(const float* fhat, int64_t ld_f, const float* that, int64_t ld_t, int64_t Sr, int64_t Sc,
+                         int64_t diag_off, int64_t P, float tau, float scale, int unit_rows, const float* Z,
+                         const float* lse, const float* g, float* dfhat, int64_t ld_df, float* dthat, int64_t ld_dt,
+                         float* ws, size_t ws_floats, void* stream, const NormTail* ntf, const NormTail* ntt) {
   EGNN_CHECK_ARG(Sr > 0 && Sc > 0 && P > 0 && ld_f >= P && ld_t >= P && tau > 0.f && fhat && that && Z && lse);
   if (ws && ws_floats < egnn_nce_bwd_ws_floats(Sr, Sc, P)) return EGNN_EWORKSPACE;
   EGNN_CHECK_ARG(diag_off >= 0 && diag_off + Sr <= Sc);
@@ -633,10 +690,34 @@
   const bool expz = nce_unit_form(tau, unit_rows);
   const float shift = (1.f / tau) * 1.0001f;
   int rc = EGNN_OK;
-  if (dfhat) rc = launch_bwd<KMAJOR>(Z, Sc, Sr, Sc, diag_off, lse, shift, expz, that, P, ld_t, that, ld_t, scale, g, dfhat, ld_df, vec4, ws, st);
-  if (rc == EGNN_OK && dthat) rc = launch_bwd<MNMAJOR>(Z, Sc, Sc, Sr, diag_off, lse, shift, expz, fhat, P, ld_f, fhat, ld_f, scale, g, dthat, ld_dt, vec4, ws, st);
+  bool done_f = false, done_t = false;
+  if (dfhat) rc = launch_bwd<KMAJOR>(Z, Sc, Sr, Sc, diag_off, lse, shift, expz, that, P, ld_t, that, ld_t, scale, g, dfhat, ld_df, vec4, ws, st, ntf, &done_f);
+  if (rc == EGNN_OK && dfhat && ntf && !done_f)
+    rc = egnn_normalize_rows_bwd_f32(ntf->xhat, ntf->ldh, dfhat, ld_df, ntf->inv_norm, ntf->idx, Sr, P, ntf->eps, ntf->dx, ntf->ldx, 0, stream);
+  if (rc == EGNN_OK && dthat) rc = launch_bwd<MNMAJOR>(Z, Sc, Sc, Sr, diag_off, lse, shift, expz, fhat, P, ld_f, fhat, ld_f, scale, g, dthat, ld_dt, vec4, ws, st, ntt, &done_t);
+  if (rc == EGNN_OK && dthat && ntt && !done_t)
+    rc = egnn_normalize_rows_bwd_f32(ntt->xhat, ntt->ldh, dthat, ld_dt, ntt->inv_norm, ntt->idx, Sc, P, ntt->eps, ntt->dx, ntt->ldx, 0, stream);
   if (rc != EGNN_OK) return rc;
   return egnn_launch_status();
+}
+
+extern "C" int egnn_nce_block_bwd_f32(const float* fhat, int64_t ld_f, const float* that, int64_t ld_t, int64_t Sr, int64_t Sc,
+                                      int64_t diag_off, int64_t P, float tau, float scale, int unit_rows, const float* Z,
+                                      const float* lse, const float* g, float* dfhat, int64_t ld_df, float* dthat, int64_t ld_dt,
+                                      float* ws, size_t ws_floats, void* stream) {
+  return nce_block_bwd(fhat, ld_f, that, ld_t, Sr, Sc, diag_off, P, tau, scale, unit_rows, Z, lse, g, dfhat, ld_df, dthat, ld_dt, ws, ws_floats,
+                       stream, nullptr, nullptr);
+}
+
+extern "C" int egnn_nce_bwd_norm_f32(const float* fhat, const float* that, int64_t S, int64_t P, int64_t ld, float tau, const float* Z,
+                                     const float* lse, const float* g, float eps, const float* inv_norm_f, const int64_t* idx_f,
+                                     float* dx_f, int64_t ld_dx_f, const float* inv_norm_t, const int64_t* idx_t, float* dx_t,
+                                     int64_t ld_dx_t, float* dfhat, float* dthat, float* ws, size_t ws_floats, void* stream) {
+  EGNN_CHECK_ARG(S > 0 && tau > 0.f && eps > 0.f);
+  EGNN_CHECK_ARG((!dx_f || (inv_norm_f && dfhat && ld_dx_f >= P)) && (!dx_t || (inv_norm_t && dthat && ld_dx_t >= P)));
+  const NormTail ntf{fhat, ld, inv_norm_f, idx_f, eps, dx_f, ld_dx_f}, ntt{that, ld, inv_norm_t, idx_t, eps, dx_t, ld_dx_t};
+  return nce_block_bwd(fhat, ld, that, ld, S, S, 0, P, tau, 1.f / ((float)S * tau), 1, Z, lse, g, dx_f ? dfhat : nullptr, ld,
+                       dx_t ? dthat : nullptr, ld, ws, ws_floats, stream, &ntf, &ntt);
 }
 
 extern "C" int egnn_nce_fwd_f32(const float* fhat, const float* that, int64_t S, int64_t P, int64_t ld, float tau, int unit_rows,
diff --git a/efficient-gnns_amd/csrc/spmm_blk.hip b/efficient-gnns_amd/csrc/spmm_blk.hip
--- a/efficient-gnns_amd/csrc/spmm_blk.hip
+++ b/efficient-gnns_amd/csrc/spmm_blk.hip
@@ -375,8 +375,9 @@
 
 __global__ __launch_bounds__(256) void bn_stats_merge_kernel(const float* __restrict__ part, int64_t n_part, int64_t C,
                                                              const float* __restrict__ Y, int64_t ldy, const int64_t* __restrict__ extra_rows,
-                                                             int64_t n_extra, const float* __restrict__ shift, int64_t n_total,
-                                                             float* __restrict__ mean, float* __restrict__ var) {
+                                                             int64_t n_extra, const float* shift, int64_t n_total,
+                                                             float* __restrict__ mean, float* __restrict__ var, float unbias, float m,
+                                                             float* rmean, float* rvar, long long* __restrict__ tracked) {
   __shared__ float sh[2][32][8];
   const int colo = threadIdx.x & 7, grp = threadIdx.x >> 3;
   const int64_t c = (int64_t)blockIdx.x * 8 + colo;
@@ -401,8 +402,15 @@
     for (int g = 0; g < 32; ++g) { a += sh[0][g][colo]; b += sh[1][g][colo]; }
     const float inv = 1.f / (float)n_total;
     const float m1 = a * inv;
-    mean[c] = (shift ? shift[c] : 0.f) + m1;
-    var[c] = fmaxf(b * inv - m1 * m1, 0.f);
+    const float mu = (shift ? shift[c] : 0.f) + m1;
+    const float v = fmaxf(b * inv - m1 * m1, 0.f);
+    mean[c] = mu;
+    var[c] = v;
+    if (rmean) {
+      rmean[c] = (1.f - m) * rmean[c] + m * mu;
+      rvar[c] = (1.f - m) * rvar[c] + (m * unbias) * v;
+      if (c == 0 && tracked) tracked[0] = tracked[0] + 1;
+    }
   }
 }
 
@@ -484,9 +492,9 @@
 
 extern "C" size_t egnn_bn_stats_merge_ws_floats(int64_t C) { return (size_t)kStatSplits * 2 * (size_t)C; }
 
-extern "C" int egnn_bn_stats_merge_f32(const float* part, int64_t n_blk, int64_t C, const float* Y, int64_t ldy,
-                                       const int64_t* extra_rows, int64_t n_extra, const float* shift, int64_t n_total, float* mean,
-                                       float* var, float* ws, size_t ws_floats, void* stream) {
+static int bn_stats_merge(const float* part, int64_t n_blk, int64_t C, const float* Y, int64_t ldy, const int64_t* extra_rows,
+                          int64_t n_extra, const float* shift, int64_t n_total, float* mean, float* var, float* ws, size_t ws_floats,
+                          float momentum, float* rmean, float* rvar, int64_t* tracked, void* stream) {
   EGNN_CHECK_ARG(n_blk >= 0 && C > 0 && n_extra >= 0 && n_total > 0 && mean && var);
   EGNN_CHECK_ARG((n_blk == 0 || part) && (n_extra == 0 || (Y && extra_rows && ldy >= C)));
   hipStream_t st = (hipStream_t)stream;
@@ -498,6 +506,27 @@
     n_part = kStatSplits;
   }
   hipLaunchKernelGGL(bn_stats_merge_kernel, dim3((unsigned)((C + 7) / 8)), dim3(256), 0, st, part, n_part, C, Y, ldy, extra_rows,
-                     n_extra, shift, n_total, mean, var);
+                     n_extra, shift, n_total, mean, var, n_total > 1 ? (float)n_total / (float)(n_total - 1) : 1.f, momentum, rmean, rvar,
+                     (long long*)tracked);
   return egnn_launch_status();
 }
+
+extern "C" int egnn_bn_stats_merge_f32(const float* part, int64_t n_blk, int64_t C, const float* Y, int64_t ldy,
+                                       const int64_t* extra_rows, int64_t n_extra, const float* shift, int64_t n_total, float* mean,
+                                       float* var, float* ws, size_t ws_floats, void* stream) {
+  return bn_stats_merge(part, n_blk, C, Y, ldy, extra_rows, n_extra, shift, n_total, mean, var, ws, ws_floats, 0.f, nullptr, nullptr, nullptr,
+                        stream);
+}
+
+extern "C" int egnn_bn_stats_merge_update_f32(const float* part, int64_t n_blk, int64_t C, const float* Y, int64_t ldy,
+                                              const int64_t* extra_rows, int64_t n_extra, const float* shift, int64_t n_total, float* mean,
+                                              float* var, float* ws, size_t ws_floats, float momentum, float* running_mean,
+                                              float* running_var, int64_t* num_batches_tracked, void* stream) {
+  EGNN_CHECK_ARG(running_mean && running_var);
+  if (momentum < 0.f) {
+    const int rc = egnn_bn_stats_merge_f32(part, n_blk, C, Y, ldy, extra_rows, n_extra, shift, n_total, mean, var, ws, ws_floats, stream);
+    return rc != EGNN_OK ? rc : egnn_bn_running_update_f32(mean, var, C, n_total, momentum, running_mean, running_var, num_batches_tracked, stream);
+  }
+  return bn_stats_merge(part, n_blk, C, Y, ldy, extra_rows, n_extra, shift, n_total, mean, var, ws, ws_floats, momentum, running_mean,
+                        running_var, num_batches_tracked, stream);
+}
diff --git a/efficient-gnns_amd/models.py b/efficient-gnns_amd/models.py
--- a/efficient-gnns_amd/models.py
+++ b/efficient-gnns_amd/models.py
@@ -57,7 +57,8 @@
             if conv_form == "fold":
                 x = self.out_feat = conv(x, adj_t, eval_bn=bn)
                 continue
-            x = conv(x, adj_t, bn_stats_shift=bn.running_mean, want_bn_stats=True) if conv_form == "stats" else conv(x, adj_t)
+            x = (conv(x, adj_t, bn_stats_shift=bn.running_mean, want_bn_stats=True, bn_running=bn) if conv_form == "stats"
+                 else conv(x, adj_t))
             if act in ("tail", "tail_sync"):
                 both = (ops.bn_act_linear(x, bn, self.convs[-1].weight, relu=True, p=self.dropout, training=True) if act == "tail"
                         else bn.fused_act_linear(x, self.convs[-1].weight, True, self.dropout, True))
diff --git a/efficient-gnns_amd/nn.py b/efficient-gnns_amd/nn.py
--- a/efficient-gnns_amd/nn.py
+++ b/efficient-gnns_amd/nn.py
@@ -63,7 +63,7 @@
         self._cached_ax = None
 
     def forward(self, x: Tensor, edge_index, edge_weight=None, bn_stats_shift: Tensor | None = None, want_bn_stats: bool = False,
-                eval_bn=None, xw: Tensor | None = None) -> Tensor:
+                eval_bn=None, xw: Tensor | None = None, bn_running=None) -> Tensor:
         if edge_weight is not None:
             raise NotImplementedError("GCNConv with edge_weight is not used by the reference")
         agg_first = self.in_channels < self.out_channels
@@ -109,7 +109,7 @@
         if agg_first:
             return ops.matmul(ops.spmm(norm, x, "sum"), self.weight, self.bias)
         return ops.spmm(norm, ops.matmul(x, self.weight) if xw is None else xw, "sum", bias=self.bias,
-                        bn_stats_shift=bn_stats_shift, want_bn_stats=want_bn_stats)
+                        bn_stats_shift=bn_stats_shift, want_bn_stats=want_bn_stats, bn_running=bn_running)
 
     def _uses_memoised_input(self, x: Tensor) -> bool:
         return bool(self.cached and _MEMOISE_AX and not x.requires_grad and self.in_channels <= self.out_channels)
diff --git a/efficient-gnns_amd/ops.py b/efficient-gnns_amd/ops.py
--- a/efficient-gnns_amd/ops.py
+++ b/efficient-gnns_amd/ops.py
@@ -11,6 +11,7 @@
 _REDUCE = {"sum": 0, "add": 0, "mean": 1, "max": 2}
 _OVERLAP_HEAVY_ROWS = True
 _SIDE_STREAMS: dict = {}
+_UNFUSED_NODES = os.environ.get("EGNN_UNFUSED_NODES", "0") == "1"
 
 
 def _side_stream(device) -> "torch.cuda.Stream":
@@ -47,9 +48,9 @@
 
 def spmm_raw(adj, x: Tensor, reduce: str = "sum", src_scale: Tensor | None = None, use_plan: bool = True,
              bias: Tensor | None = None, out: Tensor | None = None, stat_shift: Tensor | None = None, want_stats: bool = False,
-             addend: Tensor | None = None, relu: bool = False):
+             addend: Tensor | None = None, relu: bool = False, bn_running=None):
     fused = []
-    res = _spmm_raw(adj, x, reduce, src_scale, use_plan, bias, out, stat_shift, want_stats, addend, relu, fused)
+    res = _spmm_raw(adj, x, reduce, src_scale, use_plan, bias, out, stat_shift, want_stats, addend, relu, fused, bn_running)
     if relu and not fused:
         res[0].clamp_(min=0)
     return res
@@ -57,7 +58,7 @@
 
 def _spmm_raw(adj, x: Tensor, reduce: str = "sum", src_scale: Tensor | None = None, use_plan: bool = True,
               bias: Tensor | None = None, out: Tensor | None = None, stat_shift: Tensor | None = None, want_stats: bool = False,
-              addend: Tensor | None = None, relu: bool = False, relu_fused: list | None = None):
+              addend: Tensor | None = None, relu: bool = False, relu_fused: list | None = None, bn_running=None):
     _lib.require_gpu(x, adj._col)
     x = _rowmajor(x)
     n_rows, n_src = adj.sparse_sizes()
@@ -125,9 +126,16 @@
             var = torch.empty(K, dtype=torch.float32, device=x.device)
             nws = lib.egnn_bn_stats_merge_ws_floats(K)
             ws = adj._scratch("statfold", (nws,))
-            _lib.check(lib.egnn_bn_stats_merge_f32(_lib.ptr(stat_part), n_stat + n_hub, K, None, 0, None, 0,
-                                                   _lib.ptr(stat_shift), n_rows, _lib.ptr(mean), _lib.ptr(var), _lib.ptr(ws), nws,
-                                                   _lib.stream()), "egnn_bn_stats_merge_f32")
+            if bn_running is not None:
+                with torch.no_grad():
+                    _lib.check(lib.egnn_bn_stats_merge_update_f32(
+                        _lib.ptr(stat_part), n_stat + n_hub, K, None, 0, None, 0, _lib.ptr(stat_shift), n_rows, _lib.ptr(mean), _lib.ptr(var),
+                        _lib.ptr(ws), nws, float(bn_running.momentum), _lib.ptr(bn_running.running_mean), _lib.ptr(bn_running.running_var),
+                        _lib.ptr(bn_running.num_batches_tracked), _lib.stream()), "egnn_bn_stats_merge_update_f32")
+            else:
+                _lib.check(lib.egnn_bn_stats_merge_f32(_lib.ptr(stat_part), n_stat + n_hub, K, None, 0, None, 0,
+                                                       _lib.ptr(stat_shift), n_rows, _lib.ptr(mean), _lib.ptr(var), _lib.ptr(ws), nws,
+                                                       _lib.stream()), "egnn_bn_stats_merge_f32")
             return y, None, (mean, var)
         if rc != -4:
             _lib.check(rc, "egnn_spmm_csr_blk_f32")
@@ -180,12 +188,12 @@
 
 class _SpMM(torch.autograd.Function):
     @staticmethod
-    def forward(ctx, x, adj, reduce, bias=None, stat_shift=None, want_stats=False):
+    def forward(ctx, x, adj, reduce, bias=None, stat_shift=None, want_stats=False, bn_running=None):
         b = None if bias is None else bias.detach().contiguous()
         stats = None
         if want_stats:
             try:
-                y, arg, stats = spmm_raw(adj, x, reduce, bias=b, stat_shift=stat_shift, want_stats=True)
+                y, arg, stats = spmm_raw(adj, x, reduce, bias=b, stat_shift=stat_shift, want_stats=True, bn_running=bn_running)
             except HipStatsUnavailable:
                 y, arg = spmm_raw(adj, x, reduce, bias=b)
         else:
@@ -213,13 +221,13 @@
             K = gy.shape[1]
             gx = torch.zeros(n_src, K, dtype=torch.float32, device=gy.device)
             if adj.nnz() == 0:
-                return gx, None, None, (colsum(gy) if ctx.has_bias and ctx.needs_input_grad[3] else None), None, None
+                return gx, None, None, (colsum(gy) if ctx.has_bias and ctx.needs_input_grad[3] else None), None, None, None
             _, col, bits = adj._index_arrays()
             rc = _lib.load().egnn_spmm_csr_max_bwd_f32(n_rows, K, _lib.ptr(col), bits, _lib.ptr(adj._value), _lib.ptr(arg),
                                                        _lib.ptr(gy), gy.stride(0), _lib.ptr(gx), gx.stride(0), _lib.stream())
             _lib.check(rc, "egnn_spmm_csr_max_bwd_f32")
         gb = colsum(gy) if ctx.has_bias and ctx.needs_input_grad[3] else None
-        return _fresh(gx, ctx.tap_box), None, None, gb, None, None
+        return _fresh(gx, ctx.tap_box), None, None, gb, None, None, None
 
 
 def _fresh(g, tap_box):
@@ -263,7 +271,7 @@
 
 
 def spmm(adj, x: Tensor, reduce: str = "sum", bias: Tensor | None = None, bn_stats_shift: Tensor | None = None,
-         want_bn_stats: bool = False, addend: Tensor | None = None) -> Tensor:
+         want_bn_stats: bool = False, addend: Tensor | None = None, bn_running=None) -> Tensor:
     if reduce not in _REDUCE:
         raise ValueError(f"unknown reduce '{reduce}'")
     if addend is not None:
@@ -272,9 +280,12 @@
         return spmm_raw(adj, x, reduce, bias=bias, addend=addend)[0]
     if bias is not None and (reduce == "max" or (x.shape[1] % 4 == 0 and bias.data_ptr() % 16 != 0)):
         return _SpMM.apply(x, adj, reduce, None)[0] + bias
-    y, mean, var = _SpMM.apply(x, adj, reduce, bias, bn_stats_shift, bool(want_bn_stats) and reduce != "max")
+    want = bool(want_bn_stats) and reduce != "max"
+    fuse = (want and bn_running is not None and bn_running.training and bn_running.track_running_stats and bn_running.weight is not None
+            and x.shape[1] <= 1024 and _bn_running_fusable(bn_running))
+    y, mean, var = _SpMM.apply(x, adj, reduce, bias, bn_stats_shift, want, bn_running if fuse else None)
     if mean is not None:
-        y._egnn_bn_stats = (mean, var, y._version)
+        y._egnn_bn_stats = (mean, var, y._version, bn_running if fuse else None)
     return y
 
 
@@ -987,6 +998,67 @@
     return _NCE.apply(fhat, that, tau)
 
 
+class _NCENormalized(torch.autograd.Function):
+
+    @staticmethod
+    def forward(ctx, f, idx_f, t, idx_t, tau, eps):
+        _lib.require_gpu(f, idx_f, t, idx_t)
+        f, t = _rowmajor(f), _rowmajor(t)
+        S = f.shape[0] if idx_f is None else idx_f.numel()
+        P = f.shape[1]
+        if (t.shape[0] if idx_t is None else idx_t.numel()) != S or t.shape[1] != P:
+            raise ValueError("nce: student and teacher features must have the same shape")
+        lib, dev = _lib.load(), f.device
+        hats, invs = [], []
+        for x, idx in ((f, idx_f), (t, idx_t)):
+            out = torch.empty(S, P, dtype=torch.float32, device=dev)
+            inv = torch.empty(S, dtype=torch.float32, device=dev)
+            _lib.check(lib.egnn_gather_normalize_rows_f32(_lib.ptr(x), x.stride(0), _lib.ptr(idx), S, P, float(eps), _lib.ptr(out),
+                                                          out.stride(0), _lib.ptr(inv), _lib.stream()), "egnn_gather_normalize_rows_f32")
+            hats.append(out)
+            invs.append(inv)
+        Z = torch.empty(S, S, dtype=torch.float32, device=dev)
+        lse = torch.empty(S, dtype=torch.float32, device=dev)
+        loss = torch.empty(1, dtype=torch.float32, device=dev)
+        nws = lib.egnn_nce_ws_floats(S)
+        ws = torch.empty(nws, dtype=torch.float32, device=dev)
+        _lib.check(lib.egnn_nce_fwd_f32(_lib.ptr(hats[0]), _lib.ptr(hats[1]), S, P, P, float(tau), 1, _lib.ptr(Z), _lib.ptr(lse),
+                                        _lib.ptr(loss), _lib.ptr(ws), nws, _lib.stream()), "egnn_nce_fwd_f32")
+        ctx.save_for_backward(hats[0], hats[1], invs[0], invs[1], Z, lse, *[i for i in (idx_f, idx_t) if i is not None])
+        ctx.tau, ctx.eps, ctx.has_idx, ctx.n_in = float(tau), float(eps), (idx_f is not None, idx_t is not None), (f.shape[0], t.shape[0])
+        return loss[0]
+
+    @staticmethod
+    def backward(ctx, g):
+        fhat, that, inv_f, inv_t, Z, lse, *rest = ctx.saved_tensors
+        idx_f = rest.pop(0) if ctx.has_idx[0] else None
+        idx_t = rest.pop(0) if ctx.has_idx[1] else None
+        S, P = fhat.shape
+        dev = fhat.device
+        g = g.contiguous().to(torch.float32)
+
+        def grad_buffers(need, idx, n_in):
+            if not need:
+                return None, None
+            dx = torch.zeros(n_in, P, dtype=torch.float32, device=dev) if idx is not None else torch.empty(S, P, dtype=torch.float32, device=dev)
+            return dx, torch.empty(S, P, dtype=torch.float32, device=dev)
+        dxf, df = grad_buffers(ctx.needs_input_grad[0], idx_f, ctx.n_in[0])
+        dxt, dt = grad_buffers(ctx.needs_input_grad[2], idx_t, ctx.n_in[1])
+        lib = _lib.load()
+        nws = lib.egnn_nce_bwd_ws_floats(S, S, P)
+        ws = torch.empty(nws, dtype=torch.float32, device=dev)
+        _lib.check(lib.egnn_nce_bwd_norm_f32(_lib.ptr(fhat), _lib.ptr(that), S, P, P, ctx.tau, _lib.ptr(Z), _lib.ptr(lse), _lib.ptr(g), ctx.eps,
+                                             _lib.ptr(inv_f), _lib.ptr(idx_f), _lib.ptr(dxf), P, _lib.ptr(inv_t), _lib.ptr(idx_t), _lib.ptr(dxt), P,
+                                             _lib.ptr(df), _lib.ptr(dt), _lib.ptr(ws), nws, _lib.stream()), "egnn_nce_bwd_norm_f32")
+        return dxf, None, dxt, None, None, None
+
+
+def nce_normalized(f: Tensor, idx_f: Tensor | None, t: Tensor, idx_t: Tensor | None, tau: float, eps: float = 1e-12) -> Tensor:
+    if _UNFUSED_NODES or not (f.is_cuda and t.is_cuda):
+        return nce_unit(gather_normalize(f, idx_f, eps), gather_normalize(t, idx_t, eps), tau)
+    return _NCENormalized.apply(f, idx_f, t, idx_t, tau, eps)
+
+
 def nce_block_fwd(fhat: Tensor, t_all: Tensor, diag_off: int, tau: float, inv_count: float, unit_rows: bool = True):
     _lib.require_gpu(fhat, t_all)
     Sr, P = fhat.shape
@@ -1110,6 +1182,12 @@
         return dx, sums[C:], sums[:C], None, None, None, None, None, None, None, None, None
 
 
+def _bn_running_fusable(bn) -> bool:
+    rm, rv, nbt = bn.running_mean, bn.running_var, bn.num_batches_tracked
+    return (not _UNFUSED_NODES and bn.momentum is not None and rm is not None and rm.dtype == torch.float32 and rv.dtype == torch.float32
+            and nbt.dtype == torch.int64 and rm.is_contiguous() and rv.is_contiguous())
+
+
 def _bn_prepare(x: Tensor, bn, p: float, training: bool):
     x_in = x
     if not _bn_shape_ok(_rowmajor(x)) or not bn.track_running_stats or bn.weight is None:
@@ -1120,18 +1198,31 @@
     if use_batch:
         lib, dev = _lib.load(), x.device
         pre = getattr(x_in, "_egnn_bn_stats", None)
+        updated = False
+        if pre is not None and pre[3] is bn and (pre[0].shape[0] != C or pre[2] != x_in._version):
+            raise RuntimeError("bn_act: this tensor's producer already updated the BatchNorm's running statistics (ops.spmm bn_running=), "
+                               "but the tensor was changed in place since")
         if pre is not None and pre[0].shape[0] == C and pre[2] == x_in._version:
-            mean, var = pre[0], pre[1]
+            mean, var, updated = pre[0], pre[1], pre[3] is bn
         else:
             mean = torch.empty(C, dtype=torch.float32, device=dev)
             var = torch.empty(C, dtype=torch.float32, device=dev)
             nws = lib.egnn_bn_ws_floats(C)
             ws = torch.empty(nws, dtype=torch.float32, device=dev)
-            _lib.check(lib.egnn_bn_stats_f32(_lib.ptr(x), x.stride(0), n, C, _lib.ptr(mean), _lib.ptr(var), _lib.ptr(ws), nws, _lib.stream()),
-                       "egnn_bn_stats_f32")
+            if _bn_running_fusable(bn):
+                with torch.no_grad():
+                    _lib.check(lib.egnn_bn_stats_update_f32(_lib.ptr(x), x.stride(0), n, C, _lib.ptr(mean), _lib.ptr(var), _lib.ptr(ws), nws,
+                                                            float(bn.momentum), _lib.ptr(bn.running_mean), _lib.ptr(bn.running_var),
+                                                            _lib.ptr(bn.num_batches_tracked), _lib.stream()), "egnn_bn_stats_update_f32")
+                updated = True
+            else:
+                _lib.check(lib.egnn_bn_stats_f32(_lib.ptr(x), x.stride(0), n, C, _lib.ptr(mean), _lib.ptr(var), _lib.ptr(ws), nws,
+                                                 _lib.stream()), "egnn_bn_stats_f32")
         with torch.no_grad():
             rm, rv, nbt = bn.running_mean, bn.running_var, bn.num_batches_tracked
-            if rm.dtype == torch.float32 and rv.dtype == torch.float32 and nbt.dtype == torch.int64 and rm.is_contiguous() and rv.is_contiguous():
+            if updated:
+                pass
+            elif rm.dtype == torch.float32 and rv.dtype == torch.float32 and nbt.dtype == torch.int64 and rm.is_contiguous() and rv.is_contiguous():
                 _lib.check(lib.egnn_bn_running_update_f32(_lib.ptr(mean), _lib.ptr(var), C, n, -1.0 if bn.momentum is None else float(bn.momentum),
                                                           _lib.ptr(rm), _lib.ptr(rv), _lib.ptr(nbt), _lib.stream()), "egnn_bn_running_update_f32")
             else:
diff --git a/include/egnn_hip.h b/include/egnn_hip.h
--- a/include/egnn_hip.h
+++ b/include/egnn_hip.h
@@ -50,6 +50,10 @@
 int egnn_bn_stats_merge_f32(const float* stat_part, int64_t n_blk, int64_t C, const float* Y, int64_t ldy,
                             const int64_t* extra_rows, int64_t n_extra, const float* stat_shift, int64_t n_total,
                             float* mean, float* var, float* ws, size_t ws_floats, void* stream);
+int egnn_bn_stats_merge_update_f32(const float* stat_part, int64_t n_blk, int64_t C, const float* Y, int64_t ldy,
+                                   const int64_t* extra_rows, int64_t n_extra, const float* stat_shift, int64_t n_total,
+                                   float* mean, float* var, float* ws, size_t ws_floats, float momentum, float* running_mean,
+                                   float* running_var, int64_t* num_batches_tracked, void* stream);
 
 int egnn_spmm_combine_f32(const egnn_spmm_t* op, const int64_t* comb_rows, const int64_t* comb_ptr, int64_t n_comb,
                           const float* partial, int64_t stat_base, void* stream);
@@ -140,6 +144,10 @@
 int egnn_nce_bwd_f32(const float* fhat, const float* that, int64_t S, int64_t P, int64_t ld, float tau, int unit_rows,
                      const float* Z, const float* lse, const float* g,
                      float* dfhat, float* dthat, float* ws, size_t ws_floats, void* stream);
+int egnn_nce_bwd_norm_f32(const float* fhat, const float* that, int64_t S, int64_t P, int64_t ld, float tau, const float* Z,
+                          const float* lse, const float* g, float eps, const float* inv_norm_f, const int64_t* idx_f, float* dx_f,
+                          int64_t ld_dx_f, const float* inv_norm_t, const int64_t* idx_t, float* dx_t, int64_t ld_dx_t,
+                          float* dfhat, float* dthat, float* ws, size_t ws_floats, void* stream);
 
 int egnn_nce_block_fwd_f32(const float* fhat, int64_t ld_f, const float* that, int64_t ld_t, int64_t Sr, int64_t Sc,
                            int64_t diag_off, int64_t P, float tau, float inv_count, int unit_rows, float* Z, float* lse,
@@ -212,6 +220,8 @@
 size_t egnn_bn_ws_floats(int64_t C);
 int egnn_bn_stats_f32(const float* x, int64_t ld, int64_t n, int64_t C, float* mean, float* var, float* ws, size_t ws_floats,
                       void* stream);
+int egnn_bn_stats_update_f32(const float* x, int64_t ld, int64_t n, int64_t C, float* mean, float* var, float* ws, size_t ws_floats,
+                             float momentum, float* running_mean, float* running_var, int64_t* num_batches_tracked, void* stream);
 int egnn_bn_act_fwd_f32(const egnn_bn_act_t* bn, float* y, int64_t ldy, void* stream);
 int egnn_bn_act_bwd_f32(const egnn_bn_act_t* bn, const float* dy, int64_t ld_dy, int batch_stats, float* dgamma, float* dbeta,
                         float* dx, int64_t ld_dx, float* dx_colsum, float* ws, size_t ws_floats, void* stream);
```

After: 160.0 (median of 6 runs). About the same (+0.3%).
